# pierrepaleo/PDWT

Hardware: AMD Instinct MI355X
Metric: Mpixels/s fwd+inv DWT (4096² db4 L3) (higher is better)
Workload: dtype f32; 1 GPU; 4096x4096 float32, db4, 3 levels, separable DWT fwd+inv (BASELINE.json configs[1]); levels=3, parallelism=batch-split x1 (no data-path collective)

## Files before the change

pdwt_amd/csrc/casc_dev.hpp:

```cpp
#pragma once
#include "common.hpp"

#ifndef PDWT_CASC_DIAG
#define PDWT_CASC_DIAG 0
#endif
#define CASC_DIAG_ST(row) ((PDWT_CASC_DIAG & 1) ? ((row) & 31) : (row))
#define CASC_DIAG_LD(row) ((PDWT_CASC_DIAG & 2) ? ((row) & 31) : (row))

namespace pdwt {

template <int HLEN>
struct CascGeom {
    static constexpr int C = HLEN / 2 - 1;
    static constexpr int NB1 = C > 0 ? (C + 3) / 4 : 0;
    static constexpr int NB2 = C > 0 ? (C + 1) / 2 : 0;
    static constexpr int NBT = NB1 + NB2;
    static constexpr int WIN1 = 4 * (2 * NB1 + 1);
    static constexpr int WIN2 = 2 * (2 * NB2 + 1);
    static constexpr int MAXVL = 64 - 2 * NBT;
};

struct CascMap {
    int cpx;
    int strips;
    int gy;
    int flags;
    const void* tbl;
};
__host__ __device__ inline int casc_chunk_start(int g, int strip, int units, int gy, int strips, int cpx, int d)
{
    if (g >= gy) return units;
    int b = (int)(((long long)g * units) / gy);
    if (d != 0) {
        int bal = 0;
        for (int q = 0; q < g; q++) bal += (((q * strips + strip) / cpx) & 1) ? -1 : 1;
        b += d * bal;
    }
    return b;
}

struct CascBands {
    float *H1, *V1, *D1, *A2, *H2, *V2, *D2;
};
struct CascBatchF {
    const float* in;
    CascBands b;
};

template <int HLEN>
struct CascInvGeom {
    static constexpr int H2 = HLEN / 2;
    static constexpr int C = H2 / 2;
    static constexpr int SHIFT = (H2 & 1) ? 0 : 1;
    static constexpr int NB1 = C > 0 ? (C + 1) / 2 : 0;
    static constexpr int NB2 = C;
    static constexpr int NBT = NB1 + NB2;
    static constexpr int WIN1 = 2 * (2 * NB1 + 1);
    static constexpr int WIN2 = 2 * NB2 + 1;
    static constexpr int MAXVL = 64 - 2 * NBT;
    static constexpr int BASE = (C - SHIFT) & 1;
    static constexpr int VM_SB = H2 * (4 + 2 * (3 + 2));
};
struct CascInvBands {
    const float *A2, *H2, *V2, *D2, *H1, *V1, *D1;
};
struct CascInv3B {
    const float *A3, *H3, *V3, *D3;
};
struct CascBatchI {
    CascInvBands b;
    CascInv3B b3;
    float* out;
};


constexpr size_t kCascTraceOff = 1u << 20;
#ifdef PDWT_CASC_TRACE
#define CASC_TRACE_DECL unsigned long long casc_tr_[8] = {0, 0, 0, 0, 0, 0, 0, 0}
#define CASC_TRACE(i) casc_tr_[i] = wall_clock64()
#define CASC_TRACE_STORE(trash, wave_id, aux)                                                             \
    do {                                                                                                   \
        if ((threadIdx.x & 63) == 0) {                                                                     \
            unsigned long long* p_ = reinterpret_cast<unsigned long long*>((trash) + kCascTraceOff) + (size_t)(wave_id) * 8; \
            for (int i_ = 0; i_ < 7; i_++) p_[i_] = casc_tr_[i_];                                          \
            p_[7] = (unsigned long long)(aux);                                                             \
        }                                                                                                  \
    } while (0)
#else
#define CASC_TRACE_DECL
#define CASC_TRACE(i)
#define CASC_TRACE_STORE(trash, wave_id, aux)
#endif

int inv2d_casc3_f32(const float* A2, const float* H2, const float* V2, const float* D2, const float* H1, const float* V1, const float* D1,
                    const float* A3, const float* H3, const float* V3, const float* D3, float* out, float* trash, int nr, int nc, int hlen,
                    const Taps2<float>& f, const CascBatchI* d_tbl = nullptr, int nimg = 1);

int inv2d_cascw_f32(const float* A2, const float* H2, const float* V2, const float* D2, const float* H1, const float* V1, const float* D1,
                    const float* A3, const float* H3, const float* V3, const float* D3, float* out, float* trash, int nr, int nc, int hlen,
                    const Taps2<float>& f);

}
```

pdwt_amd/csrc/common.hpp:

```cpp
#pragma once
#include <atomic>
#include <hip/hip_runtime.h>
#include <hip/hip_ext.h>
#include <stddef.h>
#include <stdint.h>

#include "../../include/pdwt_hip.h"

namespace pdwt {

void set_last_error(hipError_t e, const char* what, const char* file, int line);

#define PDWT_HIP_TRY(expr)                                              \
    do {                                                                \
        hipError_t _e = (expr);                                         \
        if (_e != hipSuccess) {                                         \
            ::pdwt::set_last_error(_e, #expr, __FILE__, __LINE__);      \
            return PDWT_EHIP;                                           \
        }                                                               \
    } while (0)

hipStream_t stream();

enum KernelId {
    K_FWD2D_FUSED = 0,
    K_INV2D_FUSED,
    K_ANA_ROWS,
    K_ANA_COLS,
    K_SYN_COLS,
    K_SYN_ROWS,
    K_SWT_ANA_ROWS,
    K_SWT_ANA_COLS,
    K_SWT_SYN_COLS,
    K_SWT_SYN_ROWS,
    K_HAAR2D_FWD,
    K_HAAR2D_INV,
    K_HAAR1D_FWD,
    K_HAAR1D_INV,
    K_SOFT_THRESH,
    K_ABS_SUM,
    K_ABS_SUM_FINAL,
    K_FWD2D_CASC,
    K_INV2D_CASC,
    K_FWD2D_STREAM,
    K_INV2D_STREAM,
    K_FWD2D_SMALL,
    K_INV2D_SMALL,
    K_FWD2D_F64,
    K_INV2D_F64,
    K_THRESH_SUM,
    K_COUNT
};

struct KTimer {
    int id;
    hipEvent_t e0 = nullptr, e1 = nullptr;
    bool ext = false;
    explicit KTimer(int kernel_id, bool attach_to_launch = false);
    ~KTimer();
};
#define PDWT_LAUNCH_KT(kt, kernel, grid, block, lds, ...)                                                                  \
    do {                                                                                                                   \
        if ((kt).e0 && (kt).e1) hipExtLaunchKernelGGL(kernel, grid, block, lds, pdwt::stream(), (kt).e0, (kt).e1, 0, __VA_ARGS__); \
        else hipLaunchKernelGGL(kernel, grid, block, lds, pdwt::stream(), __VA_ARGS__);                                    \
    } while (0)

template <auto Kernel>
inline int lds_opt_in()
{
    static std::atomic<unsigned long long> done{0};
    int dev = 0;
    PDWT_HIP_TRY(hipGetDevice(&dev));
    const unsigned long long bit = 1ull << (dev & 63);
    if (!(done.load(std::memory_order_relaxed) & bit)) {
        PDWT_HIP_TRY(hipFuncSetAttribute((const void*)Kernel, hipFuncAttributeMaxDynamicSharedMemorySize, 160 * 1024));
        done.fetch_or(bit, std::memory_order_relaxed);
    }
    return PDWT_OK;
}

int lds_opt_in_ptr(const void* kernel);

unsigned long long* clock_probe_slot(int slot);
inline int clock_probe_size_class(int rows) { int c = 0; while ((rows << c) < 16384 && c < 7) c++; return c; }
constexpr int kClockProbeAllBlocks = 16384;
unsigned long long* clock_probe_all(int* all);
__device__ __forceinline__ void clock_probe_stamp(unsigned long long* probe, int second, int all = 0)
{
    if (probe && (all || (blockIdx.x == 0 && blockIdx.y == 0))) {
        unsigned long long* const p = probe + (all ? 4 * (size_t)blockIdx.x : (size_t)0);
        const unsigned long long c = clock64(), t = wall_clock64();
        if (threadIdx.x == 0) {
            p[2 * second] = c;
            p[2 * second + 1] = t;
        }
    }
}

enum KnobId {
    KN_FORCE_TWOPASS = 0,
    KN_TILED_COLS,
    KN_CASC,
    KN_CASC_WAVES,
    KN_CASC_NV,
    KN_CASC_MIN,
    KN_CASC_IWAVES,
    KN_CASC_IPFD,
    KN_CASC_WG,
    KN_CASC_IWG,
    KN_CASC_L3,
    KN_CASC_SPEC,
    KN_CASC_XCDW,
    KN_DWT1D_LDS_KB,
    KN_STREAM,
    KN_STREAM_R,
    KN_STREAM_WAVES,
    KN_STREAM_NARROW,
    KN_SMALL,
    KN_ROWS_TR,
    KN_RING_R,
    KN_RING_WAVES,
    KN_SWTF,
    KN_SWTF_M,
    KN_SWTF_MI,
    KN_SWTF_XCD,
    KN_SWTF_ALT,
    KN_SWTF_PERM,
    KN_SWTF_F64,
    KN_F64_LDS,
    KN_F64_LDS_MIN,
    KN_F64_LDS_WGS,
    KN_F64_LDS_MINGROUPS,
    KN_F64_LDS_SKEW,
    KN_NORM2SQ_REF1D,
    KN_NORM_IN_THRESHOLD,
    KN_SELFCHECK,
    KN_DWT1D_F64,
    KN_SWTF_LONG,
    KN_F64_TAIL,
    KN_EXP0,
    KN_EXP1,
    KN_EXP2,
    KN_EXP3,
    KN_NONSEP_TILED,
    KN_F64_LAT,
    KN_F64_LAT_MIN,
    KN_DWT1D_NT_MB,
    KN_COUNT
};
int knob(KnobId id);
bool counted_waits_ok();
void stat_casc_spec(int inverse);
int knob_set(const char* name, int value);
int knob_get(const char* name, int* value);

__host__ __device__ inline int div2(int n) { return (n + 1) >> 1; }
inline int idiv_up(int a, int b) { return (a + b - 1) / b; }

__device__ __forceinline__ int wrap_ext(int s, int n)
{
    const int np = n + (n & 1);
    if ((unsigned)s >= (unsigned)np) {
        s %= np;
        if (s < 0) s += np;
    }
    return (s == n) ? n - 1 : s;
}
__device__ __forceinline__ int wrap_per(int s, int n)
{
    if ((unsigned)s >= (unsigned)n) {
        s %= n;
        if (s < 0) s += n;
    }
    return s;
}

template <typename T>
struct Taps2 {
    T a[PDWT_MAX_FILTER_WIDTH];
    T b[PDWT_MAX_FILTER_WIDTH];
};

template <typename T> struct FiltersOf;
template <> struct FiltersOf<float> { using type = pdwt_filters_f32; };
template <> struct FiltersOf<double> { using type = pdwt_filters_f64; };

template <typename T>
inline Taps2<T> taps_fwd(const typename FiltersOf<T>::type* f)
{
    Taps2<T> t;
    for (int i = 0; i < PDWT_MAX_FILTER_WIDTH; i++) { t.a[i] = f->L[i]; t.b[i] = f->H[i]; }
    return t;
}
template <typename T>
inline Taps2<T> taps_inv(const typename FiltersOf<T>::type* f, T scale = T(1))
{
    Taps2<T> t;
    for (int i = 0; i < PDWT_MAX_FILTER_WIDTH; i++) { t.a[i] = f->IL[i] * scale; t.b[i] = f->IH[i] * scale; }
    return t;
}

template <typename T> __device__ __forceinline__ T fma_t(T a, T b, T c);
template <> __device__ __forceinline__ float fma_t<float>(float a, float b, float c) { return __builtin_fmaf(a, b, c); }
template <> __device__ __forceinline__ double fma_t<double>(double a, double b, double c) { return __builtin_fma(a, b, c); }

struct BandGeom {
    int nbands;
    int Nr[3 * 32 + 1], Nc[3 * 32 + 1];
    size_t alloc_elems[3 * 32 + 1];
};
int band_geometry(const pdwt_info& w, BandGeom* g);

}
```

pdwt_amd/csrc/dwt_casc.hip:

```cpp
#include "dwt_casc.hpp"

#include <algorithm>

#include "dwt_stream.hpp"
#include "stream_dev.hpp"
#include "casc_dev.hpp"

namespace pdwt {

constexpr int casc_fwd_stores(int p) { return 3 + 4 * (p & 1); }
template <int DIST>
constexpr int casc_fwd_after(int p)
{
    int n = casc_fwd_stores(p);
    for (int k = 1; k < DIST; k++) n += 2 + casc_fwd_stores(p + k);
    return n;
}

template <int HLEN>
constexpr int casc_fwd_region_bytes() { return (HLEN - 2) * 64 * (16 + 8); }

#define PDWT_VB_F0 " op_sel_hi:[0,1,0]"
#define PDWT_VB_N0 " op_sel_hi:[0,1,1]"
#define PDWT_VB_F1 " op_sel:[1,0,0] op_sel_hi:[1,1,0]"
#define PDWT_VB_N1 " op_sel:[1,0,0]"
template <bool WITH_VD>
__device__ __forceinline__ void col_pass8x2(v2f& ah0, v2f& ah1, v2f& vd0, v2f& vd1, v2f a0, v2f a1, v2f a2, v2f a3, v2f a4, v2f a5, v2f a6, v2f a7, v2f b0, v2f b1,
                                            v2f b2, v2f b3, v2f b4, v2f b5, v2f b6, v2f b7, v2f t0, v2f t1, v2f t2, v2f t3, v2f t4, v2f t5, v2f t6, v2f t7)
{
#define PDWT_CP_ROW(A, B, T, AC)                                                                                              \
    "v_pk_fma_f32 %0, " A ", " T ", " AC "0\n\tv_pk_fma_f32 %1, " B ", " T ", " AC "1\n\t"
    if constexpr (WITH_VD) {
        asm("v_pk_fma_f32 %0, %4, %20, 0" PDWT_VB_F0 "\n\tv_pk_fma_f32 %1, %12, %20, 0" PDWT_VB_F0 "\n\tv_pk_fma_f32 %2, %4, %20, 0" PDWT_VB_F1 "\n\tv_pk_fma_f32 %3, %12, %20, 0" PDWT_VB_F1
            "\n\tv_pk_fma_f32 %0, %5, %21, %0" PDWT_VB_N0 "\n\tv_pk_fma_f32 %1, %13, %21, %1" PDWT_VB_N0 "\n\tv_pk_fma_f32 %2, %5, %21, %2" PDWT_VB_N1 "\n\tv_pk_fma_f32 %3, %13, %21, %3" PDWT_VB_N1
            "\n\tv_pk_fma_f32 %0, %6, %22, %0" PDWT_VB_N0 "\n\tv_pk_fma_f32 %1, %14, %22, %1" PDWT_VB_N0 "\n\tv_pk_fma_f32 %2, %6, %22, %2" PDWT_VB_N1 "\n\tv_pk_fma_f32 %3, %14, %22, %3" PDWT_VB_N1
            "\n\tv_pk_fma_f32 %0, %7, %23, %0" PDWT_VB_N0 "\n\tv_pk_fma_f32 %1, %15, %23, %1" PDWT_VB_N0 "\n\tv_pk_fma_f32 %2, %7, %23, %2" PDWT_VB_N1 "\n\tv_pk_fma_f32 %3, %15, %23, %3" PDWT_VB_N1
            "\n\tv_pk_fma_f32 %0, %8, %24, %0" PDWT_VB_N0 "\n\tv_pk_fma_f32 %1, %16, %24, %1" PDWT_VB_N0 "\n\tv_pk_fma_f32 %2, %8, %24, %2" PDWT_VB_N1 "\n\tv_pk_fma_f32 %3, %16, %24, %3" PDWT_VB_N1
            "\n\tv_pk_fma_f32 %0, %9, %25, %0" PDWT_VB_N0 "\n\tv_pk_fma_f32 %1, %17, %25, %1" PDWT_VB_N0 "\n\tv_pk_fma_f32 %2, %9, %25, %2" PDWT_VB_N1 "\n\tv_pk_fma_f32 %3, %17, %25, %3" PDWT_VB_N1
            "\n\tv_pk_fma_f32 %0, %10, %26, %0" PDWT_VB_N0 "\n\tv_pk_fma_f32 %1, %18, %26, %1" PDWT_VB_N0 "\n\tv_pk_fma_f32 %2, %10, %26, %2" PDWT_VB_N1 "\n\tv_pk_fma_f32 %3, %18, %26, %3" PDWT_VB_N1
            "\n\tv_pk_fma_f32 %0, %11, %27, %0" PDWT_VB_N0 "\n\tv_pk_fma_f32 %1, %19, %27, %1" PDWT_VB_N0 "\n\tv_pk_fma_f32 %2, %11, %27, %2" PDWT_VB_N1 "\n\tv_pk_fma_f32 %3, %19, %27, %3" PDWT_VB_N1
            : "=&v"(ah0), "=&v"(ah1), "=&v"(vd0), "=&v"(vd1)
            : "v"(a0), "v"(a1), "v"(a2), "v"(a3), "v"(a4), "v"(a5), "v"(a6), "v"(a7), "v"(b0), "v"(b1), "v"(b2), "v"(b3), "v"(b4), "v"(b5), "v"(b6), "v"(b7),
              "s"(t0), "s"(t1), "s"(t2), "s"(t3), "s"(t4), "s"(t5), "s"(t6), "s"(t7));
    } else {
        asm("v_pk_fma_f32 %0, %2, %18, 0" PDWT_VB_F0 "\n\tv_pk_fma_f32 %1, %10, %18, 0" PDWT_VB_F0
            "\n\tv_pk_fma_f32 %0, %3, %19, %0" PDWT_VB_N0 "\n\tv_pk_fma_f32 %1, %11, %19, %1" PDWT_VB_N0
            "\n\tv_pk_fma_f32 %0, %4, %20, %0" PDWT_VB_N0 "\n\tv_pk_fma_f32 %1, %12, %20, %1" PDWT_VB_N0
            "\n\tv_pk_fma_f32 %0, %5, %21, %0" PDWT_VB_N0 "\n\tv_pk_fma_f32 %1, %13, %21, %1" PDWT_VB_N0
            "\n\tv_pk_fma_f32 %0, %6, %22, %0" PDWT_VB_N0 "\n\tv_pk_fma_f32 %1, %14, %22, %1" PDWT_VB_N0
            "\n\tv_pk_fma_f32 %0, %7, %23, %0" PDWT_VB_N0 "\n\tv_pk_fma_f32 %1, %15, %23, %1" PDWT_VB_N0
            "\n\tv_pk_fma_f32 %0, %8, %24, %0" PDWT_VB_N0 "\n\tv_pk_fma_f32 %1, %16, %24, %1" PDWT_VB_N0
            "\n\tv_pk_fma_f32 %0, %9, %25, %0" PDWT_VB_N0 "\n\tv_pk_fma_f32 %1, %17, %25, %1" PDWT_VB_N0
            : "=&v"(ah0), "=&v"(ah1)
            : "v"(a0), "v"(a1), "v"(a2), "v"(a3), "v"(a4), "v"(a5), "v"(a6), "v"(a7), "v"(b0), "v"(b1), "v"(b2), "v"(b3), "v"(b4), "v"(b5), "v"(b6), "v"(b7),
              "s"(t0), "s"(t1), "s"(t2), "s"(t3), "s"(t4), "s"(t5), "s"(t6), "s"(t7));
    }
#undef PDWT_CP_ROW
}
__device__ __forceinline__ void col_pass8x1(v2f& ah, v2f& vd, v2f a0, v2f a1, v2f a2, v2f a3, v2f a4, v2f a5, v2f a6, v2f a7, v2f t0, v2f t1, v2f t2, v2f t3, v2f t4,
                                            v2f t5, v2f t6, v2f t7)
{
    asm("v_pk_fma_f32 %0, %2, %10, 0" PDWT_VB_F0 "\n\tv_pk_fma_f32 %1, %2, %10, 0" PDWT_VB_F1
        "\n\tv_pk_fma_f32 %0, %3, %11, %0" PDWT_VB_N0 "\n\tv_pk_fma_f32 %1, %3, %11, %1" PDWT_VB_N1
        "\n\tv_pk_fma_f32 %0, %4, %12, %0" PDWT_VB_N0 "\n\tv_pk_fma_f32 %1, %4, %12, %1" PDWT_VB_N1
        "\n\tv_pk_fma_f32 %0, %5, %13, %0" PDWT_VB_N0 "\n\tv_pk_fma_f32 %1, %5, %13, %1" PDWT_VB_N1
        "\n\tv_pk_fma_f32 %0, %6, %14, %0" PDWT_VB_N0 "\n\tv_pk_fma_f32 %1, %6, %14, %1" PDWT_VB_N1
        "\n\tv_pk_fma_f32 %0, %7, %15, %0" PDWT_VB_N0 "\n\tv_pk_fma_f32 %1, %7, %15, %1" PDWT_VB_N1
        "\n\tv_pk_fma_f32 %0, %8, %16, %0" PDWT_VB_N0 "\n\tv_pk_fma_f32 %1, %8, %16, %1" PDWT_VB_N1
        "\n\tv_pk_fma_f32 %0, %9, %17, %0" PDWT_VB_N0 "\n\tv_pk_fma_f32 %1, %9, %17, %1" PDWT_VB_N1
        : "=&v"(ah), "=&v"(vd)
        : "v"(a0), "v"(a1), "v"(a2), "v"(a3), "v"(a4), "v"(a5), "v"(a6), "v"(a7), "s"(t0), "s"(t1), "s"(t2), "s"(t3), "s"(t4), "s"(t5), "s"(t6), "s"(t7));
}

template <int HLEN, int R2, bool LV, int DIST>
struct CascSpec {
    static constexpr int NA = 2 * R2, NA1 = NA + HLEN - 2, NL1 = NA - HLEN / 2 + 1;
    static constexpr int LIM = LV ? NA1 : NL1;
    static constexpr int stores_at(int q) { return ((q < NA) ? 3 : 0) + (((q & 1) && q >= HLEN - 1) ? 4 : 0); }
    static constexpr int loads_at(int q) { return (q < LIM && q + DIST < LIM) ? 2 : 0; }
    static constexpr int wait_cnt(int n)
    {
        const int m = n - DIST;
        int c = stores_at(m);
        for (int k = 1; k < DIST; k++) c += loads_at(m + k) + stores_at(m + k);
        return c;
    }
};

template <int HLEN, int NV, int W, bool SPEC = false>
__global__ __launch_bounds__(W == 1 ? 256 : 64 * W) void k_fwd2d_casc(const float* in, CascBands b, int Nr, int Nc, int VL,
                                                                       float* __restrict__ trash, CascMap cm, TapsLH f)
{
    using G = CascGeom<HLEN>;
    constexpr int C = G::C, NB1 = G::NB1, NB2 = G::NB2, NBT = G::NBT, WIN1 = G::WIN1, WIN2 = G::WIN2;
    extern __shared__ __attribute__((aligned(16))) unsigned char lds_raw[];
    CASC_TRACE_DECL;
    CASC_TRACE(0);
    if constexpr (W > 1) {
        if (cm.tbl) {
            static_assert(sizeof(CascBatchF) == 8 * sizeof(void*), "eight pointers per image");
            typedef const unsigned long long __attribute__((address_space(4))) * tbl_t;
            const tbl_t q = (tbl_t)(const unsigned long long*)cm.tbl + 8 * (size_t)blockIdx.y;
            in = (const float*)q[0];
            b = CascBands{(float*)q[1], (float*)q[2], (float*)q[3], (float*)q[4], (float*)q[5], (float*)q[6], (float*)q[7]};
        }
    }
    const int lane = threadIdx.x & 63;
    const int Nc2 = Nc >> 1, Nr2 = Nr >> 1, Nr4 = Nr >> 2, Nc4 = Nc >> 2;
    const int kw = __builtin_amdgcn_readfirstlane(threadIdx.x >> 6);
    int j0, rows2, strip;
    bool last;
    if constexpr (W == 1) {
        const int xcd = blockIdx.x & 7;
        const int wi = (blockIdx.x >> 3) * 4 + kw;
        if (wi >= cm.cpx * cm.strips) return;
        const int cy = xcd * cm.cpx + wi / cm.strips;
        strip = wi % cm.strips;
        const int nchunks = 8 * cm.cpx;
        j0 = (int)(((long long)cy * Nr4) / nchunks);
        rows2 = (int)(((long long)(cy + 1) * Nr4) / nchunks) - j0;
        if (rows2 <= 0) return;
        last = true;
    } else {
        const int xcd = blockIdx.x & 7, slot = blockIdx.x >> 3;
        const int wg = xcd * cm.cpx + slot;
        if (slot >= cm.cpx || wg >= cm.gy * cm.strips) return;
        const int gy = wg / cm.strips;
        strip = wg % cm.strips;
        const int J0 = casc_chunk_start(gy, strip, Nr4, cm.gy, cm.strips, cm.cpx, cm.flags);
        const int R = casc_chunk_start(gy + 1, strip, Nr4, cm.gy, cm.strips, cm.cpx, cm.flags) - J0;
        const int E = min((3 * (HLEN - 2) + 3) / 4, R / W - 1);
        const int base = (R + E) / W, rem = (R + E) % W;
        const int start = kw * base + min(kw, rem);
        rows2 = (kw < W - 1) ? base + (kw < rem ? 1 : 0) : R - start;
        j0 = J0 + start;
        last = (kw == W - 1);
    }
    const int xs = strip * VL * 4;
    const int x = xs + 4 * (lane - NBT);
    const bool valid = (lane >= NBT) && (lane < NBT + VL) && (x < Nc);
    const int xo = wrapi(x, Nc);
    const int yb = 4 * j0 - 3 * C;
    const int NA = 2 * rows2;
    const int NA1 = NA + HLEN - 2;
    const int NL1 = NA - HLEN / 2 + 1;
    const int rlast = last ? 2 * NA1 + HLEN - 3 : 2 * NA - 1;

    v2f ring[HLEN][2];
    v2f ring2[HLEN];
#pragma unroll
    for (int k = 0; k < HLEN; k++) ring2[k] = v2f{0.f, 0.f};

    const float* const lbase = in + xo;
    auto rowptr = [&](int r) { return lbase + (size_t)wrap1(yb + r, Nr) * Nc; };
    const unsigned xoff = (unsigned)xo * 4u;

    constexpr int REG = casc_fwd_region_bytes<HLEN>();
    unsigned char* const lds_rd = lds_raw + (size_t)(W > 1 ? kw : 0) * REG;
    unsigned char* const lds_wr = lds_raw + (size_t)(W > 1 && kw > 0 ? kw - 1 : 0) * REG;
    auto lds_ring = [&](unsigned char* reg, int r) { return reinterpret_cast<v4f*>(reg + ((size_t)r * 64 + lane) * 16); };
    auto lds_ring2 = [&](unsigned char* reg, int r) { return reinterpret_cast<v2f*>(reg + (size_t)(HLEN - 2) * 64 * 16 + ((size_t)r * 64 + lane) * 8); };
    auto row_pass1 = [&](const v4f& v, v2f (&lh)[2]) {
        float w[WIN1];
#pragma unroll
        for (int q = 0; q < 4; q++) w[NB1 * 4 + q] = v[q];
#pragma unroll
        for (int k = 0; k < NB1; k++) {
            const int dl = (NB1 - 1 - k) * 4, sl = (NB1 - k) * 4, dr = (NB1 + 1 + k) * 4, sr = (NB1 + k) * 4;
#pragma unroll
            for (int q = 0; q < 4; q++) {
                w[dl + q] = dpp_shr1(w[sl + q]);
                w[dr + q] = dpp_shl1(w[sr + q]);
            }
        }
#pragma unroll
        for (int p = 0; p < 2; p++) {
            v2f acc = {0.f, 0.f};
#pragma unroll
            for (int j = 0; j < HLEN; j++) acc = pk_fma(splat(w[NB1 * 4 - C + 2 * p + j]), f.t[HLEN - 1 - j], acc);
            lh[p] = acc;
        }
    };
    auto row_pass2 = [&](float a0, float a1, v2f& lh) {
        float w[WIN2];
        w[NB2 * 2] = a0;
        w[NB2 * 2 + 1] = a1;
#pragma unroll
        for (int k = 0; k < NB2; k++) {
            const int dl = (NB2 - 1 - k) * 2, sl = (NB2 - k) * 2, dr = (NB2 + 1 + k) * 2, sr = (NB2 + k) * 2;
#pragma unroll
            for (int q = 0; q < 2; q++) {
                w[dl + q] = dpp_shr1(w[sl + q]);
                w[dr + q] = dpp_shl1(w[sr + q]);
            }
        }
        v2f acc = {0.f, 0.f};
#pragma unroll
        for (int j = 0; j < HLEN; j++) acc = pk_fma(splat(w[NB2 * 2 - C + j]), f.t[HLEN - 1 - j], acc);
        lh = acc;
    };

    constexpr int DIST = NV / 2;
    static_assert(casc_fwd_after<DIST>(1) <= 63, "vmcnt is a 6-bit counter");
    v4f v[NV];
    {
        v4f pv[HLEN > 2 ? HLEN - 2 : 1];
#pragma unroll
        for (int r = 0; r < HLEN - 2; r++) pv[r] = *reinterpret_cast<const v4f*>(rowptr(r));
#pragma unroll
        for (int u = 0; u < NV; u++) v[u] = *reinterpret_cast<const v4f*>(rowptr(min(HLEN - 2 + u, rlast)));
        static_for<HLEN - 2>([&](auto Rr) {
            constexpr int r = decltype(Rr)::value;
            row_pass1(pv[r], ring[r]);
        });
    }
    if constexpr (W > 1) {
        if (kw > 0) {
#pragma unroll
            for (int r = 0; r < HLEN - 2; r++) *lds_ring(lds_wr, r) = v4f{ring[r][0].x, ring[r][0].y, ring[r][1].x, ring[r][1].y};
        }
    }

    const unsigned off1 = (unsigned)(valid ? x >> 1 : 0) * 4u, off2 = (unsigned)(valid ? x >> 2 : 0) * 4u;
    const lanemask_t vmask = __ballot(valid);
    const int lim1 = ((W == 1) || last) ? 0x7fffffff : NL1;
    const int lim2 = ((W == 1) || last) ? 0x7fffffff : NA;
    int lr = HLEN - 2 + NV;
    int lgr = wrap1(yb + min(lr, rlast), Nr);
    const size_t strideB = (size_t)Nc * 4;
    const char* const inB = reinterpret_cast<const char*>(in);
    const char* lp = inB + (size_t)lgr * strideB;
    const char* lplast = lp;
    auto next_rows = [&](const char*& p0, const char*& p1) {
        int lrq = lr;
        asm("" : "+s"(lrq));
        if (lrq < rlast) {
            p0 = lp;
            if (lgr + 2 < Nr) {
                p1 = lp + strideB;
                lp = p1 + strideB;
                lgr += 2;
            } else {
                p1 = (lgr + 1 == Nr) ? inB : lp + strideB;
                lgr = lgr + 2 - Nr;
                lp = inB + (size_t)lgr * strideB;
            }
            lplast = p1;
        } else {
            p0 = p1 = lplast;
        }
        lr += 2;
    };
    unsigned s1off = (unsigned)wrap1(2 * j0 - C, Nr2) * (unsigned)Nc2 * 4u;
    const unsigned s1end = (unsigned)Nr2 * (unsigned)Nc2 * 4u;
    unsigned s2off = (unsigned)j0 * (unsigned)Nc4 * 4u;
    (void)trash;
    const int hand_sb = __builtin_amdgcn_readfirstlane((W > 1 && kw > 0) ? 0 : -1);
    CASC_TRACE(1);
    static_for<NV>([&](auto K) { asm_drain1(v[decltype(K)::value]); });
    CASC_TRACE(2);
    auto a1_row = [&](auto A, int sb) {
            constexpr int a = decltype(A)::value;
            constexpr int u = a % (HLEN / 2);
            constexpr int s0 = (2 * u + HLEN - 2) % HLEN, s1 = (2 * u + HLEN - 1) % HLEN;
            const int n = sb * HLEN + a;
            constexpr int r0 = (2 * a) % NV, r1 = r0 + 1;
            int nq1 = n, nq2 = n;
            asm("" : "+s"(nq1));
            asm("" : "+s"(nq2));
            if (nq2 < lim2) {
                if (nq1 < lim1) {
                    asm_wait2<casc_fwd_after<DIST>((a + HLEN - DIST) % HLEN)>(v[r0], v[r1]);
                    row_pass1(v[r0], ring[s0]);
                    row_pass1(v[r1], ring[s1]);
                } else {
                    if constexpr (W > 1) {
                        const int i0 = 2 * (n - NL1);
                        const v4f q0 = *lds_ring(lds_rd, i0), q1 = *lds_ring(lds_rd, i0 + 1);
                        ring[s0][0] = v2f{q0.x, q0.y};
                        ring[s0][1] = v2f{q0.z, q0.w};
                        ring[s1][0] = v2f{q1.x, q1.y};
                        ring[s1][1] = v2f{q1.z, q1.w};
                    }
                }
                {
                    const char *p0, *p1;
                    next_rows(p0, p1);
                    asm_load_s(v[r0], reinterpret_cast<const float*>(p0), xoff);
                    asm_load_s(v[r1], reinterpret_cast<const float*>(p1), xoff);
                }
                v2f ah[2], vd[2];
#pragma unroll
                for (int p = 0; p < 2; p++) ah[p] = vd[p] = v2f{0.f, 0.f};
                static_for<HLEN>([&](auto J) {
                    constexpr int j = decltype(J)::value;
                    constexpr int s = (2 * u + j) % HLEN;
                    const v2f t = f.t[HLEN - 1 - j];
#pragma unroll
                    for (int p = 0; p < 2; p++) {
                        ah[p] = pk_fma(splat(ring[s][p].x), t, ah[p]);
                        vd[p] = pk_fma(splat(ring[s][p].y), t, vd[p]);
                    }
                });
                {
                    asm_store3_sm(b.H1, b.V1, b.D1, off1 + s1off, v2f{ah[0].y, ah[1].y}, v2f{vd[0].x, vd[1].x}, v2f{vd[0].y, vd[1].y},
                                  n < NA ? vmask : 0ull);
                    s1off += (unsigned)Nc2 * 4u;
                    if (s1off == s1end) s1off = 0;
                }
                row_pass2(ah[0].x, ah[1].x, ring2[a]);
                if constexpr (W > 1 && a < HLEN - 2) {
                    if (sb == hand_sb) *lds_ring2(lds_wr, a) = ring2[a];
                }
            } else {
                if constexpr (W > 1) ring2[a] = *lds_ring2(lds_rd, min(n - NA, HLEN - 3));
            }
            if constexpr (a & 1) {
                v2f ah2 = {0.f, 0.f}, vd2 = {0.f, 0.f};
                static_for<HLEN>([&](auto J) {
                    constexpr int j = decltype(J)::value;
                    constexpr int s = (a + 1 + j) % HLEN;
                    const v2f t = f.t[HLEN - 1 - j];
                    ah2 = pk_fma(splat(ring2[s].x), t, ah2);
                    vd2 = pk_fma(splat(ring2[s].y), t, vd2);
                });
                const bool own = (unsigned)(n - (HLEN - 1)) < (unsigned)(2 * rows2);
                asm_store4_sm(b.A2, b.H2, b.V2, b.D2, off2 + s2off, ah2.x, ah2.y, vd2.x, vd2.y, own ? vmask : 0ull);
                s2off += own ? (unsigned)Nc4 * 4u : 0u;
            }
    };
    auto epilogue = [&]() __attribute__((always_inline)) {
        CASC_TRACE(5);
#ifdef PDWT_CASC_TRACE
        asm volatile("s_waitcnt vmcnt(0)" ::: "memory");
#endif
        CASC_TRACE(6);
        CASC_TRACE_STORE(trash, blockIdx.x * W + kw, ((unsigned long long)NA1 << 32) | (unsigned)rows2);
    };
    if constexpr (SPEC) {
        static_assert(W == 16 && (NV == 2 || NV == 4), "wave programs exist for the 16-wave workgroups");
        const unsigned xoff_odd = xoff + (unsigned)strideB;
        auto spec = [&](auto R2c, auto LASTc) __attribute__((always_inline)) {
            constexpr int R2 = decltype(R2c)::value;
            constexpr bool LV = decltype(LASTc)::value;
            using S = CascSpec<HLEN, R2, LV, DIST>;
            constexpr int sNA = S::NA, sNA1 = S::NA1, sNL1 = S::NL1;
            constexpr int WR = LV ? 4 * R2 + 3 * C : 3 * C;
            const bool wraps = LV ? (j0 + R2 == Nr4) : (j0 == 0);
            const size_t wrapB = wraps ? (size_t)Nr * strideB : (size_t)0;
            const unsigned s1wrap = (!LV && j0 == 0) ? s1end : 0u;
            const char* sp = lp;
            static_for<sNA1>([&](auto Nn) {
                constexpr int n = decltype(Nn)::value;
                constexpr int a = n % HLEN;
                constexpr bool from_mem = LV ? true : (n < sNL1);
                constexpr bool computed = LV ? true : (n < sNA);
                constexpr bool store1 = n < sNA;
                constexpr int s0 = (2 * n + HLEN - 2) % HLEN, s1 = (2 * n + HLEN - 1) % HLEN;
                if constexpr (computed) {
                    if constexpr (from_mem) {
                        constexpr int q0 = (2 * n) % NV, q1 = q0 + 1;
                        if constexpr (n >= DIST) asm_wait2<S::wait_cnt(n)>(v[q0], v[q1]);
                        row_pass1(v[q0], ring[s0]);
                        row_pass1(v[q1], ring[s1]);
                        if constexpr (n + DIST < S::LIM) {
                            constexpr int r0 = 2 * (n + DIST) + HLEN - 2;
                            asm volatile("" : "=v"(v[q0]));
                            asm volatile("" : "=v"(v[q1]));
                            asm_load_s(v[q0], reinterpret_cast<const float*>(sp), xoff);
                            if constexpr (r0 + 1 == WR) {
                                asm_load_s(v[q1], reinterpret_cast<const float*>(sp + strideB - wrapB), xoff);
                            } else {
                                asm_load_s(v[q1], reinterpret_cast<const float*>(sp), xoff_odd);
                            }
                            sp += 2 * strideB;
                            if constexpr (r0 + 1 == WR || r0 + 2 == WR) sp -= wrapB;
                        }
                    } else {
                        constexpr int i0 = 2 * (n - sNL1);
                        const v4f q0 = *lds_ring(lds_rd, i0), q1 = *lds_ring(lds_rd, i0 + 1);
                        ring[s0][0] = v2f{q0.x, q0.y};
                        ring[s0][1] = v2f{q0.z, q0.w};
                        ring[s1][0] = v2f{q1.x, q1.y};
                        ring[s1][1] = v2f{q1.z, q1.w};
                    }
                    v2f ah[2], vd[2];
#pragma unroll
                    for (int p = 0; p < 2; p++) ah[p] = vd[p] = v2f{0.f, 0.f};
                    if constexpr (HLEN == 8) {
                        constexpr int q = (2 * n) % 8;
#define PDWT_R(j, p) ring[(q + (j)) % 8][p]
                        col_pass8x2<store1>(ah[0], ah[1], vd[0], vd[1], PDWT_R(0, 0), PDWT_R(1, 0), PDWT_R(2, 0), PDWT_R(3, 0), PDWT_R(4, 0), PDWT_R(5, 0), PDWT_R(6, 0),
                                            PDWT_R(7, 0), PDWT_R(0, 1), PDWT_R(1, 1), PDWT_R(2, 1), PDWT_R(3, 1), PDWT_R(4, 1), PDWT_R(5, 1), PDWT_R(6, 1), PDWT_R(7, 1),
                                            f.t[7], f.t[6], f.t[5], f.t[4], f.t[3], f.t[2], f.t[1], f.t[0]);
#undef PDWT_R
                    } else {
                        static_for<HLEN>([&](auto J) {
                            constexpr int j = decltype(J)::value;
                            constexpr int s = (2 * n + j) % HLEN;
                            const v2f t = f.t[HLEN - 1 - j];
#pragma unroll
                            for (int p = 0; p < 2; p++) {
                                ah[p] = pk_fma_vbcast<0, j == 0>(ring[s][p], t, ah[p]);
                                if constexpr (store1) vd[p] = pk_fma_vbcast<1, j == 0>(ring[s][p], t, vd[p]);
                            }
                        });
                    }
                    if constexpr (store1) {
                        asm_store3_sm(b.H1, b.V1, b.D1, off1 + s1off, v2f{ah[0].y, ah[1].y}, v2f{vd[0].x, vd[1].x}, v2f{vd[0].y, vd[1].y}, vmask);
                        s1off += (unsigned)Nc2 * 4u;
                        if constexpr (n == C - 1) s1off -= s1wrap;
                    }
                    row_pass2(ah[0].x, ah[1].x, ring2[a]);
                    if constexpr (n < HLEN - 2) {
                        if (kw > 0) *lds_ring2(lds_wr, n) = ring2[a];
                    }
                } else {
                    ring2[a] = *lds_ring2(lds_rd, n - sNA);
                }
                if constexpr ((n & 1) && n >= HLEN - 1) {
                    v2f ah2 = {0.f, 0.f}, vd2 = {0.f, 0.f};
                    if constexpr (HLEN == 8) {
                        constexpr int q = (a + 1) % 8;
                        col_pass8x1(ah2, vd2, ring2[q], ring2[(q + 1) % 8], ring2[(q + 2) % 8], ring2[(q + 3) % 8], ring2[(q + 4) % 8], ring2[(q + 5) % 8],
                                    ring2[(q + 6) % 8], ring2[(q + 7) % 8], f.t[7], f.t[6], f.t[5], f.t[4], f.t[3], f.t[2], f.t[1], f.t[0]);
                    } else {
                        static_for<HLEN>([&](auto J) {
                            constexpr int j = decltype(J)::value;
                            constexpr int s = (a + 1 + j) % HLEN;
                            const v2f t = f.t[HLEN - 1 - j];
                            ah2 = pk_fma_vbcast<0, j == 0>(ring2[s], t, ah2);
                            vd2 = pk_fma_vbcast<1, j == 0>(ring2[s], t, vd2);
                        });
                    }
                    asm_store4_sm(b.A2, b.H2, b.V2, b.D2, off2 + s2off, ah2.x, ah2.y, vd2.x, vd2.y, vmask);
                    s2off += (unsigned)Nc4 * 4u;
                }
                if constexpr (n == HLEN / 2 - 1 || n == HLEN - 1) asm volatile("s_waitcnt lgkmcnt(0)\n\ts_barrier" ::: "memory");

#ifdef PDWT_CASC_TRACE
                if constexpr (n == HLEN / 2 - 1) CASC_TRACE(3);
                if constexpr (n == HLEN - 1) CASC_TRACE(4);
#endif
            });
        };
        const int variant = __builtin_amdgcn_readfirstlane(last ? 3 : (rows2 == 5 ? 2 : 1));
        if (variant == 1) {
            spec(std::integral_constant<int, 4>{}, std::false_type{});
            epilogue();
            __builtin_amdgcn_endpgm();
        }
        if (variant == 2) {
            spec(std::integral_constant<int, 5>{}, std::false_type{});
            epilogue();
            __builtin_amdgcn_endpgm();
        }
        spec(std::integral_constant<int, 1>{}, std::true_type{});
        epilogue();
    } else {
    for (int sb = 0;; sb++) {
        static_for<HLEN / 2>([&](auto U) { a1_row(std::integral_constant<int, decltype(U)::value>{}, sb); });
        if constexpr (W > 1) {
            if (sb == 0) asm volatile("s_waitcnt lgkmcnt(0)\n\ts_barrier" ::: "memory");
        }
#ifdef PDWT_CASC_TRACE
        if (sb == 0) CASC_TRACE(3);
#endif
        if (sb * HLEN + HLEN / 2 >= NA1) break;
        static_for<HLEN / 2>([&](auto U) { a1_row(std::integral_constant<int, decltype(U)::value + HLEN / 2>{}, sb); });
        if constexpr (W > 1) {
            if (sb == 0) asm volatile("s_waitcnt lgkmcnt(0)\n\ts_barrier" ::: "memory");
        }
#ifdef PDWT_CASC_TRACE
        if (sb == 0) CASC_TRACE(4);
#endif
        if (sb * HLEN + HLEN >= NA1) break;
    }
    static_for<NV>([&](auto K) { asm_drain1(v[decltype(K)::value]); });
    epilogue();
    }
}

template <int HLEN, int PFD>
__global__ __launch_bounds__(256) void k_inv2d_casc(CascInvBands b, float* __restrict__ out, int Nr, int Nc, int VL,
                                                     float* __restrict__ trash, CascMap cm, Taps2<float> f)
{
    using G = CascInvGeom<HLEN>;
    constexpr int H2 = G::H2, C = G::C, SHIFT = G::SHIFT, NB1 = G::NB1, NB2 = G::NB2, NBT = G::NBT, WIN1 = G::WIN1, WIN2 = G::WIN2;
    constexpr int VM_PF = PFD * (4 + 2 * (3 + 2));
    static_assert(VM_PF - 3 <= 63, "vmcnt is a 6-bit counter");
    static_assert(H2 % PFD == 0 || PFD % H2 == 0, "register slots must be compile-time constants");
    const int lane = threadIdx.x & 63;
    const int xcd = blockIdx.x & 7;
    const int wi = (blockIdx.x >> 3) * 4 + __builtin_amdgcn_readfirstlane(threadIdx.x >> 6);
    if (wi >= cm.cpx * cm.strips) return;
    const int cy = xcd * cm.cpx + wi / cm.strips;
    const int strip = wi % cm.strips;
    const int Nr1 = Nr >> 1, Nc1 = Nc >> 1, Nr2 = Nr >> 2, Nc2 = Nc >> 2;
    const int nchunks = 8 * cm.cpx;
    const int ya = G::BASE + 2 * (int)(((long long)cy * (Nr1 >> 1)) / nchunks);
    const int ye = G::BASE + 2 * (int)(((long long)(cy + 1) * (Nr1 >> 1)) / nchunks);
    const int rows1 = ye - ya;
    if (rows1 <= 0) return;
    const int cx1 = strip * VL * 2 + 2 * (lane - NBT);
    const bool valid = (lane >= NBT) && (lane < NBT + VL) && (cx1 < Nc1);
    const int cx1w = wrapi(cx1, Nc1);
    const int cx2w = cx1w >> 1;
    const int gA = ya - C;
    const int P0 = (gA + SHIFT) >> 1;
    const int r2base = P0 - C;
    const int nrows1 = rows1 + H2 - 1 + SHIFT;
    const int nsteps = (nrows1 + 1) >> 1;

    const float* const pA2 = b.A2 + cx2w;
    const float* const pH2 = b.H2 + cx2w;
    const float* const pV2 = b.V2 + cx2w;
    const float* const pD2 = b.D2 + cx2w;
    const float* const pH1 = b.H1 + cx1w;
    const float* const pV1 = b.V1 + cx1w;
    const float* const pD1 = b.D1 + cx1w;
    auto off2 = [&](int r2) { return (size_t)wrap1(r2base + r2, Nr2) * Nc2; };
    auto off1 = [&](int r1) { return (size_t)wrap1(gA + r1, Nr1) * Nc1; };
    const unsigned voff2 = (unsigned)cx2w * 4u, voff1 = (unsigned)cx1w * 4u, voffo = (unsigned)(valid ? cx1 : 0) * 8u;
    const lanemask_t vmask = __ballot(valid);

    v2f r2av[H2], r2hd[H2];
    v2f ra[H2], rh[H2], rv[H2], rd[H2];
#pragma unroll
    for (int k = 0; k < H2; k++) ra[k] = rh[k] = rv[k] = rd[k] = v2f{0.f, 0.f};
    float q2[PFD][4];
    v2f q1[2 * PFD][3];
    {
#pragma unroll
        for (int r = 0; r < H2 - 1; r++) {
            const size_t o = off2(r);
            r2av[r] = v2f{pA2[o], pV2[o]};
            r2hd[r] = v2f{pH2[o], pD2[o]};
        }
        r2av[H2 - 1] = r2hd[H2 - 1] = v2f{0.f, 0.f};
#pragma unroll
        for (int p = 0; p < PFD; p++) {
            const size_t o = off2(H2 - 1 + p);
            q2[p][0] = pA2[o];
            q2[p][1] = pH2[o];
            q2[p][2] = pV2[o];
            q2[p][3] = pD2[o];
        }
#pragma unroll
        for (int q = 0; q < 2 * PFD; q++) {
            const size_t o = off1(q);
            q1[q][0] = *reinterpret_cast<const v2f*>(pH1 + o);
            q1[q][1] = *reinterpret_cast<const v2f*>(pV1 + o);
            q1[q][2] = *reinterpret_cast<const v2f*>(pD1 + o);
        }
    }

    float* const tr = trash + (size_t)(blockIdx.x & 7) * Nc;

    auto emit = [&](auto S0, auto OFF, int g) {
        constexpr int s0 = decltype(S0)::value, off = decltype(OFF)::value;
        const bool own = (g >= 0) && (g < 2 * rows1);
        float o4[4] = {0.f, 0.f, 0.f, 0.f};
        if (own) {
            v2f sa = {0.f, 0.f}, sh = {0.f, 0.f}, sv = {0.f, 0.f}, sd = {0.f, 0.f};
            static_for<H2>([&](auto J) {
                constexpr int j = decltype(J)::value;
                constexpr int s = (s0 + j) % H2;
                constexpr int k = HLEN - 1 - (2 * j + off);
                constexpr int kp = k & ~1;
                const v2f pl2 = v2f{f.a[kp], f.a[kp + 1]}, ph2 = v2f{f.b[kp], f.b[kp + 1]};
                sa = pk_fma_sbcast<k & 1, false>(ra[s], pl2, sa);
                sh = pk_fma_sbcast<k & 1, false>(rh[s], ph2, sh);
                sv = pk_fma_sbcast<k & 1, false>(rv[s], pl2, sv);
                sd = pk_fma_sbcast<k & 1, false>(rd[s], ph2, sd);
            });
            const v2f t1o = sa + sh, t2o = sv + sd;
            float t1[WIN1], t2[WIN1];
            t1[NB1 * 2] = t1o.x;
            t1[NB1 * 2 + 1] = t1o.y;
            t2[NB1 * 2] = t2o.x;
            t2[NB1 * 2 + 1] = t2o.y;
    #pragma unroll
            for (int k = 0; k < NB1; k++) {
                const int dl = (NB1 - 1 - k) * 2, sl = (NB1 - k) * 2, dr = (NB1 + 1 + k) * 2, sr = (NB1 + k) * 2;
    #pragma unroll
                for (int cc = 0; cc < 2; cc++) {
                    t1[dl + cc] = dpp_shr1(t1[sl + cc]);
                    t2[dl + cc] = dpp_shr1(t2[sl + cc]);
                    t1[dr + cc] = dpp_shl1(t1[sr + cc]);
                    t2[dr + cc] = dpp_shl1(t2[sr + cc]);
                }
            }
            auto pair_out = [&](auto E0) {
                constexpr int e0 = decltype(E0)::value;
                constexpr int pl = (e0 + SHIFT) >> 1;
                v2f s1 = {0.f, 0.f}, s2 = {0.f, 0.f};
    #pragma unroll
                for (int j = 0; j < H2; j++) {
                    const int m = HLEN - 1 - 2 * j;
                    s1 = pk_fma(splat(t1[NB1 * 2 + pl - C + j]), v2f{f.a[m - 1], f.a[m]}, s1);
                    s2 = pk_fma(splat(t2[NB1 * 2 + pl - C + j]), v2f{f.b[m - 1], f.b[m]}, s2);
                }
                const v2f o = s1 + s2;
                o4[e0] = o.x;
                o4[e0 + 1] = o.y;
            };
            auto single_out = [&](auto E) {
                constexpr int eo = decltype(E)::value;
                constexpr int gp = eo + SHIFT;
                constexpr int pl = gp >> 1, offx = 1 - (gp & 1);
                float s1 = 0.f, s2 = 0.f;
    #pragma unroll
                for (int j = 0; j < H2; j++) {
                    const int k = HLEN - 1 - (2 * j + offx);
                    s1 = __builtin_fmaf(t1[NB1 * 2 + pl - C + j], f.a[k], s1);
                    s2 = __builtin_fmaf(t2[NB1 * 2 + pl - C + j], f.b[k], s2);
                }
                o4[eo] = s1 + s2;
            };
            if constexpr (SHIFT == 0) {
                pair_out(std::integral_constant<int, 0>{});
                pair_out(std::integral_constant<int, 2>{});
            } else {
                single_out(std::integral_constant<int, 0>{});
                pair_out(std::integral_constant<int, 1>{});
                single_out(std::integral_constant<int, 3>{});
            }
        }
        asm_store_sm(own ? out + (size_t)wrap1(2 * ya + g, Nr) * Nc : tr, voffo, v4f{o4[0], o4[1], o4[2], o4[3]}, vmask);
    };

    auto synth2 = [&](auto S0, auto OFF, float& a0, float& a1) {
        constexpr int s0 = decltype(S0)::value, off = decltype(OFF)::value;
        v2f sav = {0.f, 0.f}, shd = {0.f, 0.f};
        static_for<H2>([&](auto J) {
            constexpr int j = decltype(J)::value;
            constexpr int s = (s0 + j) % H2;
            constexpr int k = HLEN - 1 - (2 * j + off);
            constexpr int kp = k & ~1;
            sav = pk_fma_sbcast<k & 1, false>(r2av[s], v2f{f.a[kp], f.a[kp + 1]}, sav);
            shd = pk_fma_sbcast<k & 1, false>(r2hd[s], v2f{f.b[kp], f.b[kp + 1]}, shd);
        });
        const v2f t = sav + shd;
        float t1[WIN2], t2[WIN2];
        t1[NB2] = t.x;
        t2[NB2] = t.y;
#pragma unroll
        for (int k = 0; k < NB2; k++) {
            t1[NB2 - 1 - k] = dpp_shr1(t1[NB2 - k]);
            t2[NB2 - 1 - k] = dpp_shr1(t2[NB2 - k]);
            t1[NB2 + 1 + k] = dpp_shl1(t1[NB2 + k]);
            t2[NB2 + 1 + k] = dpp_shl1(t2[NB2 + k]);
        }
        float o2[2];
#pragma unroll
        for (int e = 0; e < 2; e++) {
            const int gp = e + SHIFT;
            const int pl = gp >> 1, offx = 1 - (gp & 1);
            float s1 = 0.f, s2 = 0.f;
#pragma unroll
            for (int j = 0; j < H2; j++) {
                const int k = HLEN - 1 - (2 * j + offx);
                s1 = __builtin_fmaf(t1[NB2 + pl - C + j], f.a[k], s1);
                s2 = __builtin_fmaf(t2[NB2 + pl - C + j], f.b[k], s2);
            }
            o2[e] = s1 + s2;
        }
        a0 = o2[0];
        a1 = o2[1];
    };

    constexpr int kWait2 = VM_PF - 4, kWait1 = VM_PF - 3;
    auto step = [&](auto Pp, int sb) {
        constexpr int p = decltype(Pp)::value;
        const int s = sb * H2 + p;
        constexpr int pr = p % PFD;
        asm_wait4<kWait2>(q2[pr][0], q2[pr][1], q2[pr][2], q2[pr][3]);
        r2av[(H2 - 1 + p) % H2] = v2f{asm_copy(q2[pr][0]), asm_copy(q2[pr][2])};
        r2hd[(H2 - 1 + p) % H2] = v2f{asm_copy(q2[pr][1]), asm_copy(q2[pr][3])};
        {
            const size_t o = off2(min(H2 - 1 + s + PFD, H2 - 2 + nsteps));
            asm_load_s(q2[pr][0], b.A2 + o, voff2);
            asm_load_s(q2[pr][1], b.H2 + o, voff2);
            asm_load_s(q2[pr][2], b.V2 + o, voff2);
            asm_load_s(q2[pr][3], b.D2 + o, voff2);
        }
        static_for<2>([&](auto I) {
            constexpr int idx = decltype(I)::value;
            constexpr int q = 2 * p + idx;
            float a0, a1;
            synth2(std::integral_constant<int, p % H2>{}, std::integral_constant<int, 1 - idx>{}, a0, a1);
            const int r1 = 2 * s + idx;
            constexpr int qr = q % (2 * PFD);
            asm_wait3<kWait1>(q1[qr][0], q1[qr][1], q1[qr][2]);
            ra[q % H2] = v2f{a0, a1};
            rh[q % H2] = asm_copy(q1[qr][0]);
            rv[q % H2] = asm_copy(q1[qr][1]);
            rd[q % H2] = asm_copy(q1[qr][2]);
            {
                const size_t o = off1(min(r1 + 2 * PFD, 2 * nsteps - 1));
                asm_load_s(q1[qr][0], b.H1 + o, voff1);
                asm_load_s(q1[qr][1], b.V1 + o, voff1);
                asm_load_s(q1[qr][2], b.D1 + o, voff1);
            }
            const int g1 = 2 * (r1 - (H2 - 1)) - SHIFT;
            emit(std::integral_constant<int, (q + 1) % H2>{}, std::integral_constant<int, 1>{}, g1);
            emit(std::integral_constant<int, (q + 1) % H2>{}, std::integral_constant<int, 0>{}, g1 + 1);
        });
    };

    static_for<PFD>([&](auto K) {
        constexpr int k = decltype(K)::value;
        asm_drain1(q2[k][0]);
        asm_drain1(q2[k][1]);
        asm_drain1(q2[k][2]);
        asm_drain1(q2[k][3]);
    });
    static_for<2 * PFD>([&](auto K) {
        constexpr int k = decltype(K)::value;
        asm_drain1(q1[k][0]);
        asm_drain1(q1[k][1]);
        asm_drain1(q1[k][2]);
    });
    for (int sb = 0;; sb++) {
        bool fin = false;
        static_for<H2>([&](auto Pp) {
            if (!fin) {
                step(Pp, sb);
                fin = (sb * H2 + decltype(Pp)::value + 1 >= nsteps);
            }
        });
        if (fin) break;
    }
    static_for<PFD>([&](auto K) {
        constexpr int k = decltype(K)::value;
        asm_drain1(q2[k][0]);
        asm_drain1(q2[k][1]);
        asm_drain1(q2[k][2]);
        asm_drain1(q2[k][3]);
    });
    static_for<2 * PFD>([&](auto K) {
        constexpr int k = decltype(K)::value;
        asm_drain1(q1[k][0]);
        asm_drain1(q1[k][1]);
        asm_drain1(q1[k][2]);
    });
}

#define PDWT_CHECK_LAUNCH() PDWT_HIP_TRY(hipGetLastError())

static bool casc_enabled() { return knob(KN_CASC) == 1; }

template <int HLEN>
static int launch_fwd_casc(const float* in, const CascBands& b, float* trash, int nr, int nc, const Taps2<float>& f2, const CascBatchF* d_tbl, int nimg)
{
    TapsLH f;
    for (int k = 0; k < PDWT_MAX_FILTER_WIDTH; k++) f.t[k] = v2f{f2.a[k], f2.b[k]};
    constexpr int MAXVL = CascGeom<HLEN>::MAXVL;
    const int strips = idiv_up(nc, MAXVL * 4);
    const int VL = idiv_up(nc / 4, strips);
    constexpr int NVD = HLEN > 16 ? 4 : (HLEN % 4 == 0 ? HLEN / 2 : HLEN);
    KTimer kt(K_FWD2D_CASC, true);
    int W = knob(KN_CASC_WG);
    if (W == 0) W = 16;
    if (W != 1 && W != 4 && W != 8 && W != 16) W = 16;
    constexpr size_t REG = casc_fwd_region_bytes<HLEN>();
    while (W > 1 && (size_t)(W - 1) * REG > 150 * 1024) W /= 2;
    if (W == 2) W = 1;
    if (W > 1) {
        const int nr4 = nr / 4;
        const int wgs = knob(KN_CASC_WAVES) > 0 ? idiv_up(knob(KN_CASC_WAVES), W) : 256;
        int gy = std::max(1, wgs / strips);
        while (W > 4 && (nr4 / gy) / W < HLEN / 2) W /= 2;
        while (gy > 1 && (nr4 / gy) / W < HLEN / 2) gy--;
        if (gy >= 1 && (nr4 / gy) / W >= HLEN / 2) {
            int nwg = gy * strips;
            const size_t lds = (size_t)(W - 1) * REG;
            void (*k)(const float*, CascBands, int, int, int, float*, CascMap, TapsLH);
            k = (W == 4) ? k_fwd2d_casc<HLEN, NVD, 4> : (W == 8) ? k_fwd2d_casc<HLEN, NVD, 8> : k_fwd2d_casc<HLEN, NVD, 16>;
            const bool nv2 = W == 16 && (knob(KN_CASC_NV) == 0 || knob(KN_CASC_NV) == 2);
            if (nv2) k = k_fwd2d_casc<HLEN, 2, 16>;
            bool spec = nv2 && (knob(KN_CASC_SPEC) & 1) && 2 * 4 >= HLEN;
            auto spec_ok = [&](int gyq, int xwq) {
                const int cpxq = idiv_up(gyq * strips, 8);
                for (int g = 0; g < gyq; g++)
                    for (int st = 0; st < strips; st++) {
                        const int R = casc_chunk_start(g + 1, st, nr4, gyq, strips, cpxq, xwq) - casc_chunk_start(g, st, nr4, gyq, strips, cpxq, xwq);
                        if (R < 16) return false;
                        const int E = std::min((3 * (HLEN - 2) + 3) / 4, R / 16 - 1);
                        const int base = (R + E) / 16, rem = (R + E) % 16;
                        if (base != 4 || R - (15 * base + std::min(15, rem)) != 1) return false;
                    }
                return true;
            };
            if (spec && (knob(KN_CASC_SPEC) & 4) && knob(KN_CASC_WAVES) <= 0 && !d_tbl && (nr4 / gy) / 16 >= 8) {
                const int gy2 = (nr4 + 36) / 73;
                if (gy2 >= 3 * gy && spec_ok(gy2, 0)) {
                    gy = gy2;
                    nwg = gy * strips;
                }
            }
            int xw = spec ? knob(KN_CASC_XCDW) : 0;
            if (spec && xw != 0 && !spec_ok(gy, xw)) xw = 0;
            spec = spec && spec_ok(gy, xw);
            if (!spec) xw = 0;
            if (spec) {
                k = k_fwd2d_casc<HLEN, 2, 16, true>;
                stat_casc_spec(0);
            }
            const CascMap cm = {idiv_up(nwg, 8), strips, gy, xw, d_tbl};
            const dim3 grid((unsigned)(8 * cm.cpx), (unsigned)(d_tbl ? nimg : 1));
            if (lds > 64 * 1024) {
                int rc = (W == 4) ? lds_opt_in<k_fwd2d_casc<HLEN, NVD, 4>>()
                         : (W == 8) ? lds_opt_in<k_fwd2d_casc<HLEN, NVD, 8>>() : lds_opt_in<k_fwd2d_casc<HLEN, NVD, 16>>();
                if (rc == PDWT_OK && nv2) rc = lds_opt_in<k_fwd2d_casc<HLEN, 2, 16>>();
                if (rc == PDWT_OK && spec) rc = lds_opt_in<k_fwd2d_casc<HLEN, 2, 16, true>>();
                if (rc != PDWT_OK) return rc;
            }
            PDWT_LAUNCH_KT(kt, k, grid, dim3(64 * W), lds, in, b, nr, nc, VL, trash, cm, f);
            PDWT_CHECK_LAUNCH();
            return PDWT_OK;
        }
    }
    if (d_tbl) return 1;
    int cpx = (knob(KN_CASC_WAVES) > 0 ? knob(KN_CASC_WAVES) : 1024) / (8 * strips);
    if (cpx > nr / 4 / 4 / 8) cpx = nr / 4 / 4 / 8;
    if (cpx < 1) cpx = 1;
    const CascMap cm = {cpx, strips, 0};
    const dim3 grid((unsigned)(8 * idiv_up(cpx * strips, 4)));
    const int nv = knob(KN_CASC_NV) > 0 ? knob(KN_CASC_NV) : NVD;
    if (nv == 2)
        PDWT_LAUNCH_KT(kt, (k_fwd2d_casc<HLEN, 2, 1>), grid, dim3(256), 0, in, b, nr, nc, VL, trash, cm, f);
    else if (nv < HLEN && HLEN % 4 == 0)
        PDWT_LAUNCH_KT(kt, (k_fwd2d_casc<HLEN, NVD, 1>), grid, dim3(256), 0, in, b, nr, nc, VL, trash, cm, f);
    else
        PDWT_LAUNCH_KT(kt, (k_fwd2d_casc<HLEN, (HLEN > 16 ? NVD : HLEN), 1>), grid, dim3(256), 0, in, b, nr, nc, VL, trash, cm, f);
    PDWT_CHECK_LAUNCH();
    return PDWT_OK;
}

#ifdef PDWT_CASC_ONLY8
#define PDWT_CASC_FWD_HLENS(X) X(8)
#else
#define PDWT_CASC_FWD_HLENS(X) X(4) X(6) X(8) X(10) X(12) X(14) X(16) X(18) X(20)
#endif

int fwd2d_casc_f32(const float* in, float* H1, float* V1, float* D1, float* A2, float* H2, float* V2, float* D2, float* trash, int nr,
                   int nc, int hlen, const Taps2<float>& f, const CascBatchF* d_tbl, int nimg)
{
    if (!casc_enabled() || !stream_enabled() || !trash) return 1;
    if ((nr & 3) || (nc & 3) || nc < 256 || nr < 16 * hlen) return 1;
    if ((long long)nr * nc < (long long)knob(KN_CASC_MIN)) return 1;
    if ((long long)nr * nc >= (1LL << 32)) return 1;
    if (!al16(in) || !al16(H1) || !al16(V1) || !al16(D1) || !al16(A2) || !al16(H2) || !al16(V2) || !al16(D2)) return 1;
    const CascBands b = {H1, V1, D1, A2, H2, V2, D2};
    switch (hlen) {
#define X(H) \
    case H: return launch_fwd_casc<H>(in, b, trash, nr, nc, f, d_tbl, nimg);
        PDWT_CASC_FWD_HLENS(X)
#undef X
        default: return 1;
    }
}

template <int HLEN>
static int launch_inv_casc(const CascInvBands& b, float* out, float* trash, int nr, int nc, const Taps2<float>& f)
{
    constexpr int MAXVL = CascInvGeom<HLEN>::MAXVL;
    const int nc1 = nc / 2;
    const int strips = idiv_up(nc1, MAXVL * 2);
    const int VL = idiv_up(nc1 / 2, strips);
    int cpx = (knob(KN_CASC_IWAVES) > 0 ? knob(KN_CASC_IWAVES) : 2048) / (8 * strips);
    if (cpx > nr / 2 / 8 / 8) cpx = nr / 2 / 8 / 8;
    if (cpx < 1) cpx = 1;
    const CascMap cm = {cpx, strips, 0};
    const dim3 grid((unsigned)(8 * idiv_up(cpx * strips, 4)));
    KTimer kt(K_INV2D_CASC, true);
    constexpr int H2 = HLEN / 2;
    const int pfd = knob(KN_CASC_IPFD);
    bool launched = false;
    if constexpr (H2 % 2 == 0) {
        if (pfd == 2) {
            PDWT_LAUNCH_KT(kt, (k_inv2d_casc<HLEN, 2>), grid, dim3(256), 0, b, out, nr, nc, VL, trash, cm, f);
            launched = true;
        }
    }
    if constexpr (H2 * 14 - 3 <= 63 && H2 > 2) {
        if (pfd >= H2 && !launched) {
            PDWT_LAUNCH_KT(kt, (k_inv2d_casc<HLEN, H2>), grid, dim3(256), 0, b, out, nr, nc, VL, trash, cm, f);
            launched = true;
        }
    }
    if (!launched) PDWT_LAUNCH_KT(kt, (k_inv2d_casc<HLEN, 1>), grid, dim3(256), 0, b, out, nr, nc, VL, trash, cm, f);
    PDWT_CHECK_LAUNCH();
    return PDWT_OK;
}

#ifdef PDWT_CASC_ONLY8
#define PDWT_CASC_INV_HLENS(X) X(8)
#else
#define PDWT_CASC_INV_HLENS(X) X(4) X(6) X(8) X(10)
#endif

int inv2d_casc_f32(const float* A2, const float* H2, const float* V2, const float* D2, const float* H1, const float* V1, const float* D1,
                   float* out, float* trash, int nr, int nc, int hlen, const Taps2<float>& f)
{
    if (!casc_enabled() || !stream_enabled() || !trash) return 1;
    if ((nr & 3) || (nc & 3) || nc < 256 || nr < 32 * hlen) return 1;
    if ((long long)nr * nc < (long long)knob(KN_CASC_MIN)) return 1;
    if (!al16(out) || !al16(H1) || !al16(V1) || !al16(D1) || !al16(A2) || !al16(H2) || !al16(V2) || !al16(D2) || !al16(trash)) return 1;
    const CascInvBands b = {A2, H2, V2, D2, H1, V1, D1};
    switch (hlen) {
#define X(H) \
    case H: return launch_inv_casc<H>(b, out, trash, nr, nc, f);
        PDWT_CASC_INV_HLENS(X)
#undef X
        default: return 1;
    }
}

}
```

pdwt_amd/csrc/dwt_casc_inv3.hip:

```cpp
#include <algorithm>

#include "casc_dev.hpp"
#include "dwt_stream.hpp"
#include "stream_dev.hpp"

namespace pdwt {

#define PDWT_AI __attribute__((always_inline))

template <int HLEN>
constexpr int casc_inv3_region_bytes() { return (HLEN / 2 - 1) * 64 * (16 + 32); }

#define PDWT_PKS_FIRST0 " op_sel_hi:[1,0,0]"
#define PDWT_PKS_NEXT0 " op_sel_hi:[1,0,1]"
#define PDWT_PKS_FIRST1 " op_sel:[0,1,0] op_sel_hi:[1,1,0]"
#define PDWT_PKS_NEXT1 " op_sel:[0,1,0] op_sel_hi:[1,1,1]"
template <int HALF>
__device__ __forceinline__ void col_synth4x4(v2f& sa, v2f& sh, v2f& sv, v2f& sd, v2f a0, v2f a1, v2f a2, v2f a3, v2f h0, v2f h1, v2f h2, v2f h3, v2f v0,
                                             v2f v1, v2f v2, v2f v3, v2f d0, v2f d1, v2f d2, v2f d3, v2f fa3, v2f fa2_, v2f fa1, v2f fa0, v2f fb3, v2f fb2_,
                                             v2f fb1, v2f fb0)
{
#define PDWT_CS4(F, N)                                                                                                                    \
    asm("v_pk_fma_f32 %0, %4, %20, 0" F "\n\tv_pk_fma_f32 %1, %8, %24, 0" F "\n\tv_pk_fma_f32 %2, %12, %20, 0" F "\n\tv_pk_fma_f32 %3, %16, %24, 0" F \
        "\n\tv_pk_fma_f32 %0, %5, %21, %0" N "\n\tv_pk_fma_f32 %1, %9, %25, %1" N "\n\tv_pk_fma_f32 %2, %13, %21, %2" N "\n\tv_pk_fma_f32 %3, %17, %25, %3" N \
        "\n\tv_pk_fma_f32 %0, %6, %22, %0" N "\n\tv_pk_fma_f32 %1, %10, %26, %1" N "\n\tv_pk_fma_f32 %2, %14, %22, %2" N "\n\tv_pk_fma_f32 %3, %18, %26, %3" N \
        "\n\tv_pk_fma_f32 %0, %7, %23, %0" N "\n\tv_pk_fma_f32 %1, %11, %27, %1" N "\n\tv_pk_fma_f32 %2, %15, %23, %2" N "\n\tv_pk_fma_f32 %3, %19, %27, %3" N \
        : "=&v"(sa), "=&v"(sh), "=&v"(sv), "=&v"(sd)                                                                                       \
        : "v"(a0), "v"(a1), "v"(a2), "v"(a3), "v"(h0), "v"(h1), "v"(h2), "v"(h3), "v"(v0), "v"(v1), "v"(v2), "v"(v3), "v"(d0), "v"(d1), "v"(d2),  \
          "v"(d3), "s"(fa3), "s"(fa2_), "s"(fa1), "s"(fa0), "s"(fb3), "s"(fb2_), "s"(fb1), "s"(fb0))
    if constexpr (HALF == 0) PDWT_CS4(PDWT_PKS_FIRST0, PDWT_PKS_NEXT0);
    else PDWT_CS4(PDWT_PKS_FIRST1, PDWT_PKS_NEXT1);
#undef PDWT_CS4
}
template <int HALF>
__device__ __forceinline__ void col_synth2x4(v2f& sav, v2f& shd, v2f a0, v2f a1, v2f a2, v2f a3, v2f h0, v2f h1, v2f h2, v2f h3, v2f fa3, v2f fa2_, v2f fa1,
                                             v2f fa0, v2f fb3, v2f fb2_, v2f fb1, v2f fb0)
{
#define PDWT_CS2(F, N)                                                                                                      \
    asm("v_pk_fma_f32 %0, %2, %10, 0" F "\n\tv_pk_fma_f32 %1, %6, %14, 0" F "\n\tv_pk_fma_f32 %0, %3, %11, %0" N "\n\tv_pk_fma_f32 %1, %7, %15, %1" N \
        "\n\tv_pk_fma_f32 %0, %4, %12, %0" N "\n\tv_pk_fma_f32 %1, %8, %16, %1" N "\n\tv_pk_fma_f32 %0, %5, %13, %0" N "\n\tv_pk_fma_f32 %1, %9, %17, %1" N \
        : "=&v"(sav), "=&v"(shd)                                                                                            \
        : "v"(a0), "v"(a1), "v"(a2), "v"(a3), "v"(h0), "v"(h1), "v"(h2), "v"(h3), "s"(fa3), "s"(fa2_), "s"(fa1), "s"(fa0), "s"(fb3), "s"(fb2_),  \
          "s"(fb1), "s"(fb0))
    if constexpr (HALF == 0) PDWT_CS2(PDWT_PKS_FIRST0, PDWT_PKS_NEXT0);
    else PDWT_CS2(PDWT_PKS_FIRST1, PDWT_PKS_NEXT1);
#undef PDWT_CS2
}

template <int HLEN, int NQ, bool LV, bool L3>
struct CascInvSpec {
    using G = CascInvGeom<HLEN>;
    static constexpr int H2 = G::H2, XS = H2 / 2, NSTEPS = NQ + XS, NP = 2 * NQ;
    static constexpr int NL2 = L3 ? 3 : 4;
    static constexpr bool l2act(int s) { return s >= 0 && s < NSTEPS && (LV || s < NQ); }
    static constexpr bool need2(int s) { return l2act(s) && (LV || s + H2 - 1 < NQ); }
    static constexpr bool adv3(int s) { return L3 && !(s & 1) && (need2(s) || need2(s + 1)); }
    static constexpr int n3(int s) { return (adv3(s) && adv3(s + 2)) ? 4 : 0;  }
    static constexpr int n2(int s) { return (l2act(s) && need2(s + 1)) ? NL2 : 0; }
    static constexpr int n1(int s) { return (l2act(s) && l2act(s + 1)) ? 3 : 0; }
    static constexpr bool own(int s, int idx) { return 2 * s + idx - (H2 - 1) >= 0 && 2 * s + idx - (H2 - 1) < NP; }
    static constexpr int st(int s, int idx) { return own(s, idx) ? 2 : 0; }
    static constexpr int total(int s) { return n3(s) + n2(s) + 2 * n1(s) + st(s, 0) + st(s, 1); }
    static constexpr int wait3(int s) { return n2(s - 2) + 2 * n1(s - 2) + st(s - 2, 0) + st(s - 2, 1) + total(s - 1); }
    static constexpr int wait2(int s) { return 2 * n1(s - 1) + st(s - 1, 0) + st(s - 1, 1) + n3(s); }
    static constexpr int wait1(int s, int idx)
    {
        return idx == 0 ? st(s - 1, 0) + n1(s - 1) + st(s - 1, 1) + n3(s) + n2(s) : st(s - 1, 1) + n3(s) + n2(s) + n1(s) + st(s, 0);
    }
};

template <int HLEN, int W, bool L3, bool SPEC = false>
__global__ __launch_bounds__(64 * W) void k_inv2d_casc3(CascInvBands b, CascInv3B b3, float* out, int Nr, int Nc, int VL,
                                                         float* __restrict__ trash, CascMap cm, Taps2<float> f)
{
    using G = CascInvGeom<HLEN>;
    constexpr int H2 = G::H2, C = G::C, SHIFT = G::SHIFT, NBT = G::NBT;
    static_assert(H2 % 2 == 0, "the parity of a step must be a compile-time constant of the unrolled super-body");
    constexpr int XS = H2 / 2;
    constexpr int PHI = SHIFT;
    constexpr int T0 = (H2 - 1 + PHI) >> 1;
    static_assert(((H2 - 1 + PHI) & 1) == 0, "loop step 0 starts a level-(l+2) window");
    constexpr int NW3 = H2 + T0 - 1;
    constexpr int NL2 = L3 ? 3 : 4;
    constexpr int kStep = NL2 + 2 * (3 + 2);
    extern __shared__ __attribute__((aligned(16))) unsigned char lds_raw[];
    CASC_TRACE_DECL;
    CASC_TRACE(0);
    if (cm.tbl) {
        static_assert(sizeof(CascBatchI) == 12 * sizeof(void*), "twelve pointers per image");
        typedef const unsigned long long __attribute__((address_space(4))) * tbl_t;
        const tbl_t q = (tbl_t)(const unsigned long long*)cm.tbl + 12 * (size_t)blockIdx.y;
        b = CascInvBands{(const float*)q[0], (const float*)q[1], (const float*)q[2], (const float*)q[3], (const float*)q[4], (const float*)q[5], (const float*)q[6]};
        b3 = CascInv3B{(const float*)q[7], (const float*)q[8], (const float*)q[9], (const float*)q[10]};
        out = (float*)q[11];
    }
    const int lane = threadIdx.x & 63;
    const int kw = __builtin_amdgcn_readfirstlane(threadIdx.x >> 6);
    const int Nr1 = Nr >> 1, Nc1 = Nc >> 1, Nr2 = Nr >> 2, Nc2 = Nc >> 2, Nr3 = Nr >> 3, Nc3 = Nc >> 3;
    const int xcd = blockIdx.x & 7, slot = blockIdx.x >> 3;
    const int wg = xcd * cm.cpx + slot;
    if (slot >= cm.cpx || wg >= cm.gy * cm.strips) return;
    const int gy = wg / cm.strips, strip = wg % cm.strips;
    const int Np = Nr2 >> 1;
    const int Jp = casc_chunk_start(gy, strip, Np, cm.gy, cm.strips, cm.cpx, cm.flags);
    const int Rp = casc_chunk_start(gy + 1, strip, Np, cm.gy, cm.strips, cm.cpx, cm.flags) - Jp;
    const int Ep = 0;
    const int basep = (Rp + Ep) / W, remp = (Rp + Ep) % W;
    const int startp = kw * basep + min(kw, remp);
    const bool last = (kw == W - 1);
    const int nQ = 2 * (last ? Rp - startp : basep + (kw < remp ? 1 : 0));
    const int Q0 = 2 * (Jp + startp);
    const int nsteps = nQ + XS;
    const int P0 = 2 * (Q0 + C) - SHIFT;
    const int O0 = 2 * (P0 + C) - SHIFT;
    const int nP = 2 * nQ;
    const int last2 = last ? H2 - 2 + nsteps : nQ - 1;
    const int last1 = last ? 2 * nsteps - 1 : nP - 1;
    const int P3_0 = (Q0 + SHIFT) >> 1;
    const int last3 = ((last2 + PHI) >> 1) + H2 - 1;

    const int X0 = strip * VL - NBT;
    const int cx1 = 2 * (X0 + lane);
    const bool valid = (lane >= NBT) && (lane < NBT + VL) && (cx1 < Nc1);
    const int cx1w = wrapi(cx1, Nc1);
    const int cx2w = cx1w >> 1;
    const int c3w = wrapi(((X0 + 1) >> 1) - C + lane, Nc3);
    const int bp_addr = 4 * (((X0 + lane + 1) >> 1) - ((X0 + 1) >> 1) + C);
    const bool bp_odd = ((X0 + lane) & 1) != 0;

    auto off3 = [&](int i) PDWT_AI { return (size_t)CASC_DIAG_LD(wrapi(P3_0 - C + i, Nr3)) * Nc3; };
    auto off2 = [&](int s2) PDWT_AI { return (size_t)CASC_DIAG_LD(wrap1(Q0 + s2, Nr2)) * Nc2; };
    auto off1 = [&](int r1) PDWT_AI { return (size_t)CASC_DIAG_LD(wrap1(P0 + r1, Nr1)) * Nc1; };
    const unsigned voff3 = (unsigned)c3w * 4u, voff2 = (unsigned)cx2w * 4u, voff1 = (unsigned)cx1w * 4u, voffo = (unsigned)(valid ? cx1 : 0) * 8u;
    const lanemask_t vmask = __ballot(valid);
    constexpr int kFold = (PDWT_CASC_DIAG & 2) ? 32 : 0;
    const unsigned str3 = (unsigned)Nc3 * 4u, str2 = (unsigned)Nc2 * 4u, str1 = (unsigned)Nc1 * 4u;
    const unsigned end3 = (unsigned)(kFold ? min(kFold, Nr3) : Nr3) * str3, end2 = (unsigned)(kFold ? min(kFold, Nr2) : Nr2) * str2,
                   end1 = (unsigned)(kFold ? min(kFold, Nr1) : Nr1) * str1;
    int c3 = min(T0 + H2, last3), c2 = min(H2, last2), c1 = min(2, last1);
    unsigned o3 = (unsigned)CASC_DIAG_LD(wrapi(P3_0 - C + c3, Nr3)) * str3, o2 = (unsigned)CASC_DIAG_LD(wrap1(Q0 + c2, Nr2)) * str2,
             o1 = (unsigned)CASC_DIAG_LD(wrap1(P0 + c1, Nr1)) * str1;
    auto advance = [&](int& c, unsigned& o, int lastc, unsigned str, unsigned end) {
        int cq = c;
        asm("" : "+s"(cq));
        if (cq < lastc) {
            c++;
            o += str;
            if (o == end) o = 0;
        }
    };
    int orow = CASC_DIAG_ST(wrap1(O0, Nr));
    float* op = out + (size_t)orow * Nc;
    const int oend = (PDWT_CASC_DIAG & 1) ? min(32, Nr) : Nr;
    (void)trash;

    constexpr int REG = casc_inv3_region_bytes<HLEN>();
    unsigned char* const lds_rd = lds_raw + (size_t)kw * REG;
    unsigned char* const lds_wr = lds_raw + (size_t)(kw > 0 ? kw - 1 : 0) * REG;
    auto lds_l2 = [&](unsigned char* reg, int r) PDWT_AI { return reinterpret_cast<v4f*>(reg + ((size_t)r * 64 + lane) * 16); };
    auto lds_l1 = [&](unsigned char* reg, int r, int h) PDWT_AI {
        return reinterpret_cast<v4f*>(reg + (size_t)(H2 - 1) * 64 * 16 + (((size_t)r * 2 + h) * 64 + lane) * 16);
    };

    v2f r3av[H2], r3hd[H2];
    v2f r2av[H2], r2hd[H2];
    v2f ra[H2], rh[H2], rv[H2], rd[H2];
#pragma unroll
    for (int k = 0; k < H2; k++) ra[k] = rh[k] = rv[k] = rd[k] = v2f{0.f, 0.f};

    static_assert(SHIFT == 1, "even H2");
    v2f fa2[H2], fb2[H2];
#pragma unroll
    for (int i = 0; i < H2; i++) {
        fa2[i] = v2f{f.a[2 * i], f.a[2 * i + 1]};
        fb2[i] = v2f{f.b[2 * i], f.b[2 * i + 1]};
    }
    auto nat_pair = [&](const float* t1w, const float* t2w) PDWT_AI {
        v2f s1 = {0.f, 0.f}, s2 = {0.f, 0.f};
#pragma unroll
        for (int j = 0; j < H2; j++) {
            const int m = HLEN - 1 - 2 * j;
            s1 = pk_fma(splat(t1w[j]), fa2[(m - 1) / 2], s1);
            s2 = pk_fma(splat(t2w[j]), fb2[(m - 1) / 2], s2);
        }
        return s1 + s2;
    };
    auto synth_col = [&](const v2f (&av)[H2], const v2f (&hd)[H2], auto S0, auto OFF) {
        constexpr int s0 = decltype(S0)::value, off = decltype(OFF)::value;
        v2f sav = {0.f, 0.f}, shd = {0.f, 0.f};
        if constexpr (H2 == 4) {
            constexpr int half = (HLEN - 1 - off) & 1;
            col_synth2x4<half>(sav, shd, av[s0 % 4], av[(s0 + 1) % 4], av[(s0 + 2) % 4], av[(s0 + 3) % 4], hd[s0 % 4], hd[(s0 + 1) % 4], hd[(s0 + 2) % 4],
                               hd[(s0 + 3) % 4], fa2[3], fa2[2], fa2[1], fa2[0], fb2[3], fb2[2], fb2[1], fb2[0]);
        } else {
            static_for<H2>([&](auto J) {
                constexpr int j = decltype(J)::value;
                constexpr int sl = (s0 + j) % H2;
                constexpr int k = HLEN - 1 - (2 * j + off);
                sav = pk_fma_sbcast<k & 1, j == 0>(av[sl], fa2[k >> 1], sav);
                shd = pk_fma_sbcast<k & 1, j == 0>(hd[sl], fb2[k >> 1], shd);
            });
        }
        const v2f t = sav + shd;
        float t1w[H2], t2w[H2];
        t1w[C] = t.x;
        t2w[C] = t.y;
#pragma unroll
        for (int k = 1; k <= C; k++) {
            t1w[C - k] = dpp_shr1(t1w[C - k + 1]);
            t2w[C - k] = dpp_shr1(t2w[C - k + 1]);
        }
#pragma unroll
        for (int k = 1; k <= H2 - 1 - C; k++) {
            t1w[C + k] = dpp_shl1(t1w[C + k - 1]);
            t2w[C + k] = dpp_shl1(t2w[C + k - 1]);
        }
        return nat_pair(t1w, t2w);
    };
    auto own_pair = [&](v2f p0) PDWT_AI { return v2f{p0.y, dpp_shl1(p0.x)}; };
    auto a2_from = [&](const v2f (&av)[H2], const v2f (&hd)[H2], auto OFF) {
        const v2f p0 = synth_col(av, hd, std::integral_constant<int, 0>{}, OFF);
        const int glo = __builtin_amdgcn_ds_bpermute(bp_addr, __float_as_int(p0.x));
        const int ghi = __builtin_amdgcn_ds_bpermute(bp_addr, __float_as_int(p0.y));
        return __int_as_float(bp_odd ? glo : ghi);
    };

    float q3[4];
    float q2[4];
    v2f q1[2][3];
    {
        v2f w3av[NW3], w3hd[NW3];
        if constexpr (L3) {
#pragma unroll
            for (int i = 0; i < NW3; i++) {
                const size_t o = off3(min(i, last3)) + c3w;
                w3av[i] = v2f{b3.A3[o], b3.V3[o]};
                w3hd[i] = v2f{b3.H3[o], b3.D3[o]};
            }
            const size_t o = off3(min(NW3, last3)) + c3w;
            q3[0] = b3.A3[o];
            q3[1] = b3.H3[o];
            q3[2] = b3.V3[o];
            q3[3] = b3.D3[o];
        } else {
            q3[0] = q3[1] = q3[2] = q3[3] = 0.f;
        }
#pragma unroll
        for (int r = 0; r < H2 - 1; r++) {
            const size_t o = off2(r) + cx2w;
            r2av[r] = v2f{L3 ? 0.f : b.A2[o], b.V2[o]};
            r2hd[r] = v2f{b.H2[o], b.D2[o]};
        }
        r2av[H2 - 1] = r2hd[H2 - 1] = v2f{0.f, 0.f};
        {
            const size_t o = off2(H2 - 1) + cx2w;
            q2[0] = L3 ? 0.f : b.A2[o];
            q2[1] = b.H2[o];
            q2[2] = b.V2[o];
            q2[3] = b.D2[o];
        }
#pragma unroll
        for (int q = 0; q < 2; q++) {
            const size_t o = off1(q) + cx1w;
            q1[q][0] = *reinterpret_cast<const v2f*>(b.H1 + o);
            q1[q][1] = *reinterpret_cast<const v2f*>(b.V1 + o);
            q1[q][2] = *reinterpret_cast<const v2f*>(b.D1 + o);
        }
        if constexpr (L3) static_for<H2 - 1>([&](auto S2) {
            constexpr int s2 = decltype(S2)::value;
            constexpr int t = (s2 + PHI) >> 1, idx3 = (s2 + PHI) & 1;
            v2f av[H2], hd[H2];
#pragma unroll
            for (int j = 0; j < H2; j++) {
                av[j] = w3av[t + j];
                hd[j] = w3hd[t + j];
            }
            r2av[s2].x = a2_from(av, hd, std::integral_constant<int, 1 - idx3>{});
        });
        if constexpr (L3) {
#pragma unroll
            for (int j = 0; j < H2; j++) {
                r3av[j] = w3av[T0 - 1 + j];
                r3hd[j] = w3hd[T0 - 1 + j];
            }
        }
    }
    CASC_TRACE(1);
    if (kw > 0) {
#pragma unroll
        for (int r = 0; r < H2 - 1; r++) *lds_l2(lds_wr, r) = v4f{r2av[r].x, r2av[r].y, r2hd[r].x, r2hd[r].y};
    }


    auto emit = [&](auto S0, auto OFF, auto own_, int g) PDWT_AI {
        constexpr int s0 = decltype(S0)::value, off = decltype(OFF)::value;
        constexpr bool kOwnStatic = std::is_same<decltype(own_), std::true_type>::value;
        const bool own = own_;
        v4f o4;
        asm("" : "=v"(o4));
        if (own) {
            v2f sa = {0.f, 0.f}, sh = {0.f, 0.f}, sv = {0.f, 0.f}, sd = {0.f, 0.f};
            if constexpr (H2 == 4) {
                constexpr int half = (HLEN - 1 - off) & 1;
                constexpr int j0 = s0 % 4, j1 = (s0 + 1) % 4, j2 = (s0 + 2) % 4, j3 = (s0 + 3) % 4;
                col_synth4x4<half>(sa, sh, sv, sd, ra[j0], ra[j1], ra[j2], ra[j3], rh[j0], rh[j1], rh[j2], rh[j3], rv[j0], rv[j1], rv[j2], rv[j3], rd[j0],
                                   rd[j1], rd[j2], rd[j3], fa2[3], fa2[2], fa2[1], fa2[0], fb2[3], fb2[2], fb2[1], fb2[0]);
            } else {
                static_for<H2>([&](auto J) {
                    constexpr int j = decltype(J)::value;
                    constexpr int sl = (s0 + j) % H2;
                    constexpr int k = HLEN - 1 - (2 * j + off);
                    sa = pk_fma_sbcast<k & 1, j == 0>(ra[sl], fa2[k >> 1], sa);
                    sh = pk_fma_sbcast<k & 1, j == 0>(rh[sl], fb2[k >> 1], sh);
                    sv = pk_fma_sbcast<k & 1, j == 0>(rv[sl], fa2[k >> 1], sv);
                    sd = pk_fma_sbcast<k & 1, j == 0>(rd[sl], fb2[k >> 1], sd);
                });
            }
            const v2f t1o = sa + sh, t2o = sv + sd;
            constexpr int NT = H2 + 1;
            float t1w[NT], t2w[NT];
            t1w[C - 1] = t1o.x;
            t1w[C] = t1o.y;
            t2w[C - 1] = t2o.x;
            t2w[C] = t2o.y;
#pragma unroll
            for (int i = C - 2; i >= 0; i--) {
                t1w[i] = dpp_shr1(t1w[i + 2]);
                t2w[i] = dpp_shr1(t2w[i + 2]);
            }
#pragma unroll
            for (int i = C + 1; i < NT; i++) {
                t1w[i] = dpp_shl1(t1w[i - 2]);
                t2w[i] = dpp_shl1(t2w[i - 2]);
            }
            const v2f pa = nat_pair(t1w, t2w);
            const v2f pb = nat_pair(t1w + 1, t2w + 1);
            o4 = v4f{dpp_shr1(pb.y), pa.x, pa.y, pb.x};
        }
        (void)g;
        if constexpr (kOwnStatic) {
            asm_store_sm(op, voffo, o4, vmask);
            op += Nc;
        } else {
            asm_store_sm(op, voffo, o4, own ? vmask : 0ull);
            if (own) {
                op += Nc;
                if (++orow == oend) {
                    orow = 0;
                    op = out;
                }
            }
        }
    };

    auto step = [&](auto Pp, int sb) {
        constexpr int p = decltype(Pp)::value;
        constexpr bool even = L3 && (p & 1) == 0;
        constexpr int EX = even ? 4 : 0;
        const int s = sb * H2 + p;
        const bool l2act = last || (s < nQ);
        if (l2act) {
            const int s2 = H2 - 1 + s;
            if constexpr (even) {
                asm_wait4<2 * kStep>(q3[0], q3[1], q3[2], q3[3]);
#pragma unroll
                for (int j = 0; j < H2 - 1; j++) {
                    r3av[j] = r3av[j + 1];
                    r3hd[j] = r3hd[j + 1];
                }
                r3av[H2 - 1] = v2f{asm_copy(q3[0]), asm_copy(q3[2])};
                r3hd[H2 - 1] = v2f{asm_copy(q3[1]), asm_copy(q3[3])};
                {
                    const unsigned vo = voff3 + o3;
                    asm_load_s(q3[0], b3.A3, vo);
                    asm_load_s(q3[1], b3.H3, vo);
                    asm_load_s(q3[2], b3.V3, vo);
                    asm_load_s(q3[3], b3.D3, vo);
                    advance(c3, o3, last3, str3, end3);
                }
            }
            float a2 = 0.f;
            if constexpr (L3) a2 = a2_from(r3av, r3hd, std::integral_constant<int, even ? 1 : 0>{});
            constexpr int sl = (H2 - 1 + p) % H2;
            if constexpr (L3) {
                asm_wait3<2 * (3 + 2) + EX>(q2[1], q2[2], q2[3]);
            } else {
                asm_wait4<2 * (3 + 2)>(q2[0], q2[1], q2[2], q2[3]);
                a2 = asm_copy(q2[0]);
            }
            v4f e = v4f{a2, asm_copy(q2[2]), asm_copy(q2[1]), asm_copy(q2[3])};
            if (!(last || s2 < nQ)) e = *lds_l2(lds_rd, s2 - nQ);
            r2av[sl] = v2f{e.x, e.y};
            r2hd[sl] = v2f{e.z, e.w};
            {
                const unsigned vo = voff2 + o2;
                if constexpr (!L3) asm_load_s(q2[0], b.A2, vo);
                asm_load_s(q2[1], b.H2, vo);
                asm_load_s(q2[2], b.V2, vo);
                asm_load_s(q2[3], b.D2, vo);
                advance(c2, o2, last2, str2, end2);
            }
        }
        static_for<2>([&](auto I) {
            constexpr int idx = decltype(I)::value;
            constexpr int q = 2 * p + idx;
            const int r1 = 2 * s + idx;
            constexpr int sl = q % H2;
            if (l2act) {
                const v2f a01 = own_pair(synth_col(r2av, r2hd, std::integral_constant<int, p % H2>{}, std::integral_constant<int, 1 - idx>{}));
                asm_wait3<2 + (3 + 2) + NL2 + EX>(q1[idx][0], q1[idx][1], q1[idx][2]);
                ra[sl] = a01;
                rh[sl] = asm_copy(q1[idx][0]);
                rv[sl] = asm_copy(q1[idx][1]);
                rd[sl] = asm_copy(q1[idx][2]);
                {
                    const unsigned vo = voff1 + o1;
                    asm_load_s(q1[idx][0], b.H1, vo);
                    asm_load_s(q1[idx][1], b.V1, vo);
                    asm_load_s(q1[idx][2], b.D1, vo);
                    advance(c1, o1, last1, str1, end1);
                }
                if constexpr (q < H2 - 1) {
                    if (sb == 0 && kw > 0) {
                        *lds_l1(lds_wr, q, 0) = v4f{ra[sl].x, ra[sl].y, rh[sl].x, rh[sl].y};
                        *lds_l1(lds_wr, q, 1) = v4f{rv[sl].x, rv[sl].y, rd[sl].x, rd[sl].y};
                    }
                }
            } else if (r1 - nP < H2 - 1) {
                const v4f e0 = *lds_l1(lds_rd, r1 - nP, 0), e1 = *lds_l1(lds_rd, r1 - nP, 1);
                ra[sl] = v2f{e0.x, e0.y};
                rh[sl] = v2f{e0.z, e0.w};
                rv[sl] = v2f{e1.x, e1.y};
                rd[sl] = v2f{e1.z, e1.w};
            }
            const int ws = r1 - (H2 - 1);
            const bool own = (ws >= 0) && (ws < nP);
            emit(std::integral_constant<int, (q + 1) % H2>{}, std::integral_constant<int, 1>{}, own, 2 * ws);
            emit(std::integral_constant<int, (q + 1) % H2>{}, std::integral_constant<int, 0>{}, own, 2 * ws + 1);
        });
    };

    asm_drain1(q3[0]);
    asm_drain1(q3[1]);
    asm_drain1(q3[2]);
    asm_drain1(q3[3]);
    asm_drain1(q2[0]);
    asm_drain1(q2[1]);
    asm_drain1(q2[2]);
    asm_drain1(q2[3]);
    static_for<2>([&](auto K) {
        constexpr int k = decltype(K)::value;
        asm_drain1(q1[k][0]);
        asm_drain1(q1[k][1]);
        asm_drain1(q1[k][2]);
    });
    CASC_TRACE(2);

    auto spec = [&](auto NQc, auto LASTc) PDWT_AI {
        {
            constexpr int NQ = decltype(NQc)::value;
            constexpr bool LV = decltype(LASTc)::value;
            using S = CascInvSpec<HLEN, NQ, LV, L3>;
            constexpr int WR3 = NQ / 2 + C, WR2 = NQ, WR1 = 2 * NQ - 2 * C + SHIFT, WRO = 4 * NQ - 6 * C + 3 * SHIFT;
            const bool bottom = LV && (Q0 + NQ == Nr2);
            const unsigned w3 = bottom ? end3 : 0u, w2 = bottom ? end2 : 0u, w1 = bottom ? end1 : 0u;
            const size_t wo = bottom ? (size_t)Nr * Nc : (size_t)0;
            static_for<S::NSTEPS>([&](auto Ss) {
                constexpr int st = decltype(Ss)::value;
                constexpr int p = st % H2;
                constexpr bool even = L3 && (st & 1) == 0;
                if constexpr (S::l2act(st)) {
                    constexpr int s2 = H2 - 1 + st;
                    constexpr int sl = s2 % H2;
                    if constexpr (S::adv3(st)) {
                        if constexpr (st >= 2) asm_wait4<S::wait3(st)>(q3[0], q3[1], q3[2], q3[3]);
#pragma unroll
                        for (int j = 0; j < H2 - 1; j++) {
                            r3av[j] = r3av[j + 1];
                            r3hd[j] = r3hd[j + 1];
                        }
                        r3av[H2 - 1] = v2f{asm_copy(q3[0]), asm_copy(q3[2])};
                        r3hd[H2 - 1] = v2f{asm_copy(q3[1]), asm_copy(q3[3])};
                        if constexpr (S::n3(st) != 0) {
                            constexpr int row = T0 + H2 + st / 2;
                            const unsigned vo = voff3 + o3;
                            asm volatile("" : "=v"(q3[0]));
                            asm volatile("" : "=v"(q3[1]));
                            asm volatile("" : "=v"(q3[2]));
                            asm volatile("" : "=v"(q3[3]));
                            asm_load_s(q3[0], b3.A3, vo);
                            asm_load_s(q3[1], b3.H3, vo);
                            asm_load_s(q3[2], b3.V3, vo);
                            asm_load_s(q3[3], b3.D3, vo);
                            o3 += str3;
                            if constexpr (row + 1 == WR3) o3 -= w3;
                        }
                    }
                    if constexpr (S::need2(st)) {
                        float a2 = 0.f;
                        if constexpr (L3) a2 = a2_from(r3av, r3hd, std::integral_constant<int, even ? 1 : 0>{});
                        if constexpr (L3) {
                            if constexpr (st >= 1) asm_wait3<S::wait2(st)>(q2[1], q2[2], q2[3]);
                        } else {
                            if constexpr (st >= 1) asm_wait4<S::wait2(st)>(q2[0], q2[1], q2[2], q2[3]);
                            a2 = asm_copy(q2[0]);
                        }
                        r2av[sl] = v2f{a2, asm_copy(q2[2])};
                        r2hd[sl] = v2f{asm_copy(q2[1]), asm_copy(q2[3])};
                    } else {
                        const v4f e = *lds_l2(lds_rd, s2 - NQ);
                        r2av[sl] = v2f{e.x, e.y};
                        r2hd[sl] = v2f{e.z, e.w};
                    }
                    if constexpr (S::n2(st) != 0) {
                        const unsigned vo = voff2 + o2;
                        if constexpr (!L3) {
                            asm volatile("" : "=v"(q2[0]));
                            asm_load_s(q2[0], b.A2, vo);
                        }
                        asm volatile("" : "=v"(q2[1]));
                        asm volatile("" : "=v"(q2[2]));
                        asm volatile("" : "=v"(q2[3]));
                        asm_load_s(q2[1], b.H2, vo);
                        asm_load_s(q2[2], b.V2, vo);
                        asm_load_s(q2[3], b.D2, vo);
                        o2 += str2;
                        if constexpr (s2 + 2 == WR2) o2 -= w2;
                    }
                }
                static_for<2>([&](auto I) {
                    constexpr int idx = decltype(I)::value;
                    constexpr int r1 = 2 * st + idx;
                    constexpr int sl = r1 % H2;
                    if constexpr (S::l2act(st)) {
                        const v2f a01 = own_pair(synth_col(r2av, r2hd, std::integral_constant<int, p % H2>{}, std::integral_constant<int, 1 - idx>{}));
                        if constexpr (st >= 1) asm_wait3<S::wait1(st, idx)>(q1[idx][0], q1[idx][1], q1[idx][2]);
                        ra[sl] = a01;
                        rh[sl] = asm_copy(q1[idx][0]);
                        rv[sl] = asm_copy(q1[idx][1]);
                        rd[sl] = asm_copy(q1[idx][2]);
                        if constexpr (S::n1(st) != 0) {
                            const unsigned vo = voff1 + o1;
                            asm volatile("" : "=v"(q1[idx][0]));
                            asm volatile("" : "=v"(q1[idx][1]));
                            asm volatile("" : "=v"(q1[idx][2]));
                            asm_load_s(q1[idx][0], b.H1, vo);
                            asm_load_s(q1[idx][1], b.V1, vo);
                            asm_load_s(q1[idx][2], b.D1, vo);
                            o1 += str1;
                            if constexpr (r1 + 3 == WR1) o1 -= w1;
                        }
                        if constexpr (r1 < H2 - 1) {
                            if (kw > 0) {
                                *lds_l1(lds_wr, r1, 0) = v4f{ra[sl].x, ra[sl].y, rh[sl].x, rh[sl].y};
                                *lds_l1(lds_wr, r1, 1) = v4f{rv[sl].x, rv[sl].y, rd[sl].x, rd[sl].y};
                            }
                        }
                    } else if constexpr (r1 - S::NP < H2 - 1) {
                        const v4f e0 = *lds_l1(lds_rd, r1 - S::NP, 0), e1 = *lds_l1(lds_rd, r1 - S::NP, 1);
                        ra[sl] = v2f{e0.x, e0.y};
                        rh[sl] = v2f{e0.z, e0.w};
                        rv[sl] = v2f{e1.x, e1.y};
                        rd[sl] = v2f{e1.z, e1.w};
                    }
                    if constexpr (S::own(st, idx)) {
                        constexpr int ws = r1 - (H2 - 1);
                        static_for<2>([&](auto Pq) {
                            constexpr int par = decltype(Pq)::value;
                            constexpr int g = 2 * ws + par;
                            __builtin_amdgcn_sched_barrier(0);
                            emit(std::integral_constant<int, (r1 + 1) % H2>{}, std::integral_constant<int, 1 - par>{}, std::true_type{}, g);
                            if constexpr (g + 1 == WRO) op -= wo;
                            __builtin_amdgcn_sched_barrier(0);
                        });
                    }
                });
                if constexpr (st < XS) asm volatile("s_waitcnt lgkmcnt(0)\n\ts_barrier" ::: "memory");
#ifdef PDWT_CASC_TRACE
                if constexpr (st == H2 - 1) CASC_TRACE(3);
                if constexpr (st == 2 * H2 - 1) CASC_TRACE(4);
#endif
            });
        }
    };
    auto epilogue = [&]() PDWT_AI {
        CASC_TRACE(5);
#ifdef PDWT_CASC_TRACE
        asm volatile("s_waitcnt vmcnt(0)" ::: "memory");
#endif
        CASC_TRACE(6);
        CASC_TRACE_STORE(trash + kCascTraceOff, blockIdx.x * W + kw, ((unsigned long long)nsteps << 32) | (unsigned)nQ);
    };
    if constexpr (SPEC) {
        static_assert(W == 16, "wave programs exist for the 16-wave workgroups");
        const int variant = __builtin_amdgcn_readfirstlane(last ? 3 : (nQ == 6 ? 2 : 1));
        if (variant == 1) {
            spec(std::integral_constant<int, 4>{}, std::false_type{});
            epilogue();
            __builtin_amdgcn_endpgm();
        }
        if (variant == 2) {
            spec(std::integral_constant<int, 6>{}, std::false_type{});
            epilogue();
            __builtin_amdgcn_endpgm();
        }
        spec(std::integral_constant<int, 4>{}, std::true_type{});
        epilogue();
    } else {
    for (int sb = 0;; sb++) {
        bool fin = false;
        static_for<H2>([&](auto Pp) {
            constexpr int p = decltype(Pp)::value;
            if (!fin) {
                step(Pp, sb);
                if constexpr (p < XS || p == 0) {
                    if (sb == 0) asm volatile("s_waitcnt lgkmcnt(0)\n\ts_barrier" ::: "memory");
                }
                fin = (sb * H2 + p + 1 >= nsteps);
            }
        });
#ifdef PDWT_CASC_TRACE
        if (sb == 0) CASC_TRACE(3);
        if (sb == 1) CASC_TRACE(4);
#endif
        if (fin) break;
    }
    {
        asm_drain1(q3[0]);
        asm_drain1(q3[1]);
        asm_drain1(q3[2]);
        asm_drain1(q3[3]);
        asm_drain1(q2[0]);
        asm_drain1(q2[1]);
        asm_drain1(q2[2]);
        asm_drain1(q2[3]);
        static_for<2>([&](auto K) {
            constexpr int k = decltype(K)::value;
            asm_drain1(q1[k][0]);
            asm_drain1(q1[k][1]);
            asm_drain1(q1[k][2]);
        });
    }
        epilogue();
    }
}

#define PDWT_CHECK_LAUNCH() PDWT_HIP_TRY(hipGetLastError())

template <int HLEN, bool L3>
static int launch_inv_casc3(const CascInvBands& b, const CascInv3B& b3, float* out, float* trash, int nr, int nc, const Taps2<float>& f,
                            const CascBatchI* d_tbl, int nimg)
{
    using G = CascInvGeom<HLEN>;
    constexpr int H2 = G::H2;
    const int nc1 = nc / 2, np = nr / 8;
    const int strips = idiv_up(nc1, G::MAXVL * 2);
    const int VL = idiv_up(nc1 / 2, strips);
    int Wk = knob(KN_CASC_IWG);
    if (Wk != 4 && Wk != 8 && Wk != 12 && Wk != 16) Wk = 16;
    constexpr size_t REG = casc_inv3_region_bytes<HLEN>();
    auto lds_bytes = [&](int w) { return (size_t)(w - 1) * REG; };
    const int wgs = knob(KN_CASC_IWAVES) > 0 ? idiv_up(knob(KN_CASC_IWAVES), Wk) : 256;
    auto fits = [&](int w, int g) {
        if (lds_bytes(w) > 150 * 1024) return false;
        for (int Rp : {np / g, idiv_up(np, g)}) {
            const int Ep = 0;
            const int basep = (Rp + Ep) / w, remp = (Rp + Ep) % w;
            if (2 * basep < H2) return false;
            const int lastp = Rp - ((w - 1) * basep + std::min(w - 1, remp));
            if (lastp < 1) return false;
        }
        return true;
    };
    int W = 0, gy = 0;
    for (int w : {Wk, 16, 12, 8, 4}) {
        for (int g = std::max(1, wgs / strips); g >= std::max(1, wgs / strips / 2) && !W; g--)
            if (fits(w, g)) {
                W = w;
                gy = g;
            }
        if (W) break;
    }
    if (!W) return 1;
    const int nwg = gy * strips;
    
    const size_t lds = lds_bytes(W);
    void (*k)(CascInvBands, CascInv3B, float*, int, int, int, float*, CascMap, Taps2<float>);
    k = (W == 4) ? k_inv2d_casc3<HLEN, 4, L3> : (W == 8) ? k_inv2d_casc3<HLEN, 8, L3> : (W == 12) ? k_inv2d_casc3<HLEN, 12, L3> : k_inv2d_casc3<HLEN, 16, L3>;
    bool spec = W == 16 && ((knob(KN_CASC_SPEC) >> 1) & 1) && H2 <= 4;
    int xw = spec ? knob(KN_CASC_XCDW) : 0;
    for (int pass = 0; pass < 2; pass++) {
        bool ok = spec;
        for (int g = 0; g < gy && ok; g++)
            for (int st = 0; st < strips && ok; st++) {
                const int Rp = casc_chunk_start(g + 1, st, np, gy, strips, idiv_up(nwg, 8), xw) - casc_chunk_start(g, st, np, gy, strips, idiv_up(nwg, 8), xw);
                ok = Rp / 16 == 2;
            }
        if (ok || xw == 0) {
            spec = ok;
            break;
        }
        xw = 0;
    }
    if (!spec) xw = 0;
    if (spec) {
        k = k_inv2d_casc3<HLEN, 16, L3, true>;
        stat_casc_spec(1);
    }
    const CascMap cm = {idiv_up(nwg, 8), strips, gy, xw, d_tbl};
    const dim3 grid((unsigned)(8 * cm.cpx), (unsigned)(d_tbl ? nimg : 1));
    if (lds > 64 * 1024) {
        const int rc = spec ? lds_opt_in<k_inv2d_casc3<HLEN, 16, L3, true>>()
                       : (W == 4) ? lds_opt_in<k_inv2d_casc3<HLEN, 4, L3>>() : (W == 8) ? lds_opt_in<k_inv2d_casc3<HLEN, 8, L3>>() : (W == 12) ? lds_opt_in<k_inv2d_casc3<HLEN, 12, L3>>() : lds_opt_in<k_inv2d_casc3<HLEN, 16, L3>>();
        if (rc != PDWT_OK) return rc;
    }
    KTimer kt(K_INV2D_CASC, true);
    PDWT_LAUNCH_KT(kt, k, grid, dim3(64 * W), lds, b, b3, out, nr, nc, VL, trash, cm, f);
    PDWT_CHECK_LAUNCH();
    return PDWT_OK;
}

int inv2d_casc3_f32(const float* A2, const float* H2, const float* V2, const float* D2, const float* H1, const float* V1, const float* D1,
                    const float* A3, const float* H3, const float* V3, const float* D3, float* out, float* trash, int nr, int nc, int hlen,
                    const Taps2<float>& f, const CascBatchI* d_tbl, int nimg)
{
    const bool l3 = A3 != nullptr;
    if ((nr & 7) || (nc & 7) || nc < 256 || nr < 32 * hlen) return 1;
    if ((long long)nr * nc >= (1LL << 32)) return 1;
    if (!al16(out) || !al16(H1) || !al16(V1) || !al16(D1) || !al16(H2) || !al16(V2) || !al16(D2) || !al16(trash)) return 1;
    if (!l3 && !al16(A2)) return 1;
    const CascInvBands b = {A2, H2, V2, D2, H1, V1, D1};
    const CascInv3B b3 = {A3, H3, V3, D3};
    switch (hlen) {
        case 4: return l3 ? launch_inv_casc3<4, true>(b, b3, out, trash, nr, nc, f, d_tbl, nimg) : launch_inv_casc3<4, false>(b, b3, out, trash, nr, nc, f, d_tbl, nimg);
        case 8: return l3 ? launch_inv_casc3<8, true>(b, b3, out, trash, nr, nc, f, d_tbl, nimg) : launch_inv_casc3<8, false>(b, b3, out, trash, nr, nc, f, d_tbl, nimg);
        case 12: return l3 ? launch_inv_casc3<12, true>(b, b3, out, trash, nr, nc, f, d_tbl, nimg) : launch_inv_casc3<12, false>(b, b3, out, trash, nr, nc, f, d_tbl, nimg);
        case 20: return l3 ? launch_inv_casc3<20, true>(b, b3, out, trash, nr, nc, f, d_tbl, nimg) : launch_inv_casc3<20, false>(b, b3, out, trash, nr, nc, f, d_tbl, nimg);
        case 16: return l3 ? launch_inv_casc3<16, true>(b, b3, out, trash, nr, nc, f, d_tbl, nimg) : launch_inv_casc3<16, false>(b, b3, out, trash, nr, nc, f, d_tbl, nimg);
        default: return 1;
    }
}

}
```

pdwt_amd/csrc/dwt_stream.hip:

```cpp
#include "dwt_stream.hpp"

#include <algorithm>
#include "stream_dev.hpp"

namespace pdwt {

template <int HLEN, int NIN_>
struct FwdGeom {
    static constexpr int NIN = NIN_;
    static constexpr int C = HLEN / 2 - 1;
    static constexpr int NB = C > 0 ? (C + NIN - 1) / NIN : 0;
    static constexpr int WIN = NIN * (2 * NB + 1);
    static constexpr int MAXVL = 64 - 2 * NB;
};

template <int HLEN, int NIN>
__global__ __launch_bounds__(256) void k_fwd2d_stream(const float* __restrict__ in, float* __restrict__ cA, float* __restrict__ cH,
                                                       float* __restrict__ cV, float* __restrict__ cD, int Nr, int Nc, int R, int VL,
                                                       float* __restrict__ trash, int trash_mask, ChunkMap cm, TapsLH f,
                                                       const StreamBatchF* __restrict__ batch)
{
    if (batch) {
        const StreamBatchF e = batch[blockIdx.y];
        in = e.in;
        cA = e.cA;
        cH = e.cH;
        cV = e.cV;
        cD = e.cD;
        trash = e.trash;
    }
    using G = FwdGeom<HLEN, NIN>;
    using VIN = typename VecOf<NIN>::type;
    constexpr int NB = G::NB, C = G::C, WIN = G::WIN, P = NIN / 2;
    int cy, bx;
    if (!chunk_of_block(cm, cy, bx)) return;
    const int lane = threadIdx.x & 63;
    const int strip = bx * 4 + (threadIdx.x >> 6);
    const int xs = strip * VL * NIN;
    if (xs >= Nc) return;
    const int Nr2 = Nr >> 1, Nc2 = Nc >> 1;
    const int y0 = cy * R;
    const int rows = min(R, Nr2 - y0);
    if (rows <= 0) return;
    const int x = xs + NIN * (lane - NB);
    const bool valid = (lane >= NB) && (lane < NB + VL) && (x < Nc);
    const int xo = wrapi(x, Nc);
    const int yb = 2 * y0 - C;
    const int nin = 2 * rows + HLEN - 2;

    v2f ring[HLEN][P];

    auto load_row = [&](int r, VIN& v) { v = *reinterpret_cast<const VIN*>(in + (size_t)wrap1(yb + r, Nr) * Nc + xo); };

    auto row_pass = [&](const VIN& v, v2f (&lh)[P]) {
        float w[WIN];
#pragma unroll
        for (int q = 0; q < NIN; q++) w[NB * NIN + q] = v[q];
#pragma unroll
        for (int k = 0; k < NB; k++) {
            const int dl = (NB - 1 - k) * NIN, sl = (NB - k) * NIN, dr = (NB + 1 + k) * NIN, sr = (NB + k) * NIN;
#pragma unroll
            for (int q = 0; q < NIN; q++) {
                w[dl + q] = dpp_shr1(w[sl + q]);
                w[dr + q] = dpp_shl1(w[sr + q]);
            }
        }
#pragma unroll
        for (int p = 0; p < P; p++) {
            v2f acc = {0.f, 0.f};
#pragma unroll
            for (int j = 0; j < HLEN; j++) acc = pk_fma(splat(w[NB * NIN - C + 2 * p + j]), f.t[HLEN - 1 - j], acc);
            lh[p] = acc;
        }
    };

    VIN v[HLEN];
    {
        VIN pv[HLEN > 2 ? HLEN - 2 : 1];
#pragma unroll
        for (int r = 0; r < HLEN - 2; r++) load_row(r, pv[r]);
#pragma unroll
        for (int u = 0; u < HLEN; u++)
            if (HLEN - 2 + u < nin) load_row(HLEN - 2 + u, v[u]);
        static_for<HLEN - 2>([&](auto Rr) {
            constexpr int r = decltype(Rr)::value;
            row_pass(pv[r], ring[r]);
        });
    }

    const size_t ocol = (size_t)(x >> 1);
    auto body = [&](auto FAST, int q0) {
        constexpr bool fast = decltype(FAST)::value;
        const int rnext = 2 * q0 + 2 * HLEN - 2;
        static_for<HLEN / 2>([&](auto U) {
            constexpr int u = decltype(U)::value;
            if (fast || q0 + u < rows) {
                constexpr int s0 = (2 * u + HLEN - 2) % HLEN, s1 = (2 * u + HLEN - 1) % HLEN;
                row_pass(v[2 * u], ring[s0]);
                row_pass(v[2 * u + 1], ring[s1]);
                if (fast || rnext + 2 * u + 1 < nin) {
                    load_row(rnext + 2 * u, v[2 * u]);
                    load_row(rnext + 2 * u + 1, v[2 * u + 1]);
                }
                v2f ah[P], vd[P];
#pragma unroll
                for (int p = 0; p < P; p++) ah[p] = vd[p] = v2f{0.f, 0.f};
                static_for<HLEN>([&](auto J) {
                    constexpr int j = decltype(J)::value;
                    constexpr int s = (2 * u + j) % HLEN;
                    const v2f t = f.t[HLEN - 1 - j];
#pragma unroll
                    for (int p = 0; p < P; p++) {
                        ah[p] = pk_fma(splat(ring[s][p].x), t, ah[p]);
                        vd[p] = pk_fma(splat(ring[s][p].y), t, vd[p]);
                    }
                });
                float a[P], hh[P], vv[P], dd[P];
#pragma unroll
                for (int p = 0; p < P; p++) {
                    a[p] = ah[p].x;
                    hh[p] = ah[p].y;
                    vv[p] = vd[p].x;
                    dd[p] = vd[p].y;
                }
                if (valid) {
                    const size_t o = (size_t)(y0 + q0 + u) * Nc2 + ocol;
                    vstore(cA + o, a);
                    vstore(cH + o, hh);
                    vstore(cV + o, vv);
                    vstore(cD + o, dd);
                }
            }
        });
    };
    int q0 = 0;
    if (q0 + HLEN <= rows) {
        constexpr int kAfter = 4 + 6 * (HLEN / 2 - 1);
        using VOUT = typename std::conditional<P == 2, v2f, float>::type;
        float* const tr = trash + (size_t)(blockIdx.x & trash_mask) * 1024 + (threadIdx.x >> 6) * 256 + lane * P;
        const size_t ostep = valid ? (size_t)Nc2 : 0;
        float* pA = valid ? cA + (size_t)y0 * Nc2 + ocol : tr;
        float* pH = valid ? cH + (size_t)y0 * Nc2 + ocol : tr + 64 * P;
        float* pV = valid ? cV + (size_t)y0 * Nc2 + ocol : tr;
        float* pD = valid ? cD + (size_t)y0 * Nc2 + ocol : tr + 64 * P;
        const float* const lbase = in + xo;
        static_for<HLEN>([&](auto K) { asm_drain1(v[decltype(K)::value]); });
        for (; q0 + HLEN <= rows; q0 += HLEN / 2) {
            const int rnext = 2 * q0 + 2 * HLEN - 2;
            static_for<HLEN / 2>([&](auto U) {
                constexpr int u = decltype(U)::value;
                constexpr int s0 = (2 * u + HLEN - 2) % HLEN, s1 = (2 * u + HLEN - 1) % HLEN;
                asm_wait2<kAfter>(v[2 * u], v[2 * u + 1]);
                row_pass(v[2 * u], ring[s0]);
                row_pass(v[2 * u + 1], ring[s1]);
                asm_load(v[2 * u], lbase + (size_t)wrap1(yb + rnext + 2 * u, Nr) * Nc);
                asm_load(v[2 * u + 1], lbase + (size_t)wrap1(yb + rnext + 2 * u + 1, Nr) * Nc);
                v2f ah[P], vd[P];
#pragma unroll
                for (int p = 0; p < P; p++) ah[p] = vd[p] = v2f{0.f, 0.f};
                static_for<HLEN>([&](auto J) {
                    constexpr int j = decltype(J)::value;
                    constexpr int s = (2 * u + j) % HLEN;
                    const v2f t = f.t[HLEN - 1 - j];
#pragma unroll
                    for (int p = 0; p < P; p++) {
                        ah[p] = pk_fma(splat(ring[s][p].x), t, ah[p]);
                        vd[p] = pk_fma(splat(ring[s][p].y), t, vd[p]);
                    }
                });
                const size_t ro = (size_t)(q0 + u) * ostep;
                if constexpr (P == 2) {
                    asm_store(pA + ro, VOUT{ah[0].x, ah[1].x});
                    asm_store(pH + ro, VOUT{ah[0].y, ah[1].y});
                    asm_store(pV + ro, VOUT{vd[0].x, vd[1].x});
                    asm_store(pD + ro, VOUT{vd[0].y, vd[1].y});
                } else {
                    asm_store(pA + ro, ah[0].x);
                    asm_store(pH + ro, ah[0].y);
                    asm_store(pV + ro, vd[0].x);
                    asm_store(pD + ro, vd[0].y);
                }
            });
        }
        static_for<HLEN>([&](auto K) { asm_drain1(v[decltype(K)::value]); });
    }
    for (; q0 < rows; q0 += HLEN / 2) body(std::false_type{}, q0);
}

template <int HLEN>
struct InvGeom {
    static constexpr int H2 = HLEN / 2;
    static constexpr int C = H2 / 2;
    static constexpr int SHIFT = (H2 & 1) ? 0 : 1;
    static constexpr int PC = 2;
    static constexpr int NB = C > 0 ? (C + PC - 1) / PC : 0;
    static constexpr int WIN = PC * (2 * NB + 1);
    static constexpr int NROWS_EXTRA = H2 - 1 + SHIFT;
    static constexpr int MAXVL = 64 - 2 * NB;
};

template <int HLEN>
__global__ __launch_bounds__(256) void k_inv2d_stream(const float* __restrict__ cA, const float* __restrict__ cH,
                                                       const float* __restrict__ cV, const float* __restrict__ cD, float* __restrict__ out,
                                                       int Nri, int Nci, int RQ, int VL, ChunkMap cm, Taps2<float> f,
                                                       const StreamBatchI* __restrict__ batch)
{
    if (batch) {
        const StreamBatchI e = batch[blockIdx.y];
        cA = e.cA;
        cH = e.cH;
        cV = e.cV;
        cD = e.cD;
        out = e.out;
    }
    using G = InvGeom<HLEN>;
    constexpr int H2 = G::H2, C = G::C, SHIFT = G::SHIFT, NB = G::NB, WIN = G::WIN;
    int cy, bx;
    if (!chunk_of_block(cm, cy, bx)) return;
    const int lane = threadIdx.x & 63;
    const int strip = bx * 4 + (threadIdx.x >> 6);
    const int col0 = strip * VL * 2;
    if (col0 >= Nci) return;
    const int cx = col0 + (lane - NB) * 2;
    const int cxw = wrapi(cx, Nci);
    const bool valid = (lane >= NB) && (lane < NB + VL) && (cx < Nci);
    const int Nco = 2 * Nci;
    const int y0 = cy * RQ;
    const int rowsq = min(RQ, Nri - y0);
    if (rowsq <= 0) return;
    const int yb = y0 - C;
    const int nrows = rowsq + G::NROWS_EXTRA;

    v2f ra[H2], rhh[H2], rv[H2], rd[H2];

    auto load_row = [&](int r, float2& a, float2& h, float2& v, float2& d) {
        const size_t o = (size_t)wrap1(yb + r, Nri) * Nci + cxw;
        a = *reinterpret_cast<const float2*>(cA + o);
        h = *reinterpret_cast<const float2*>(cH + o);
        v = *reinterpret_cast<const float2*>(cV + o);
        d = *reinterpret_cast<const float2*>(cD + o);
    };
    auto put = [&](auto S, const float2& a, const float2& h, const float2& v, const float2& d) {
        constexpr int s = decltype(S)::value;
        ra[s] = v2f{a.x, a.y};
        rhh[s] = v2f{h.x, h.y};
        rv[s] = v2f{v.x, v.y};
        rd[s] = v2f{d.x, d.y};
    };

    auto emit = [&](auto S0, auto OFF, int gy) {
        constexpr int s0 = decltype(S0)::value, off = decltype(OFF)::value;
        v2f sa = {0.f, 0.f}, sh = {0.f, 0.f}, sv = {0.f, 0.f}, sd = {0.f, 0.f};
        static_for<H2>([&](auto J) {
            constexpr int j = decltype(J)::value;
            constexpr int s = (s0 + j) % H2;
            constexpr int k = HLEN - 1 - (2 * j + off);
            constexpr int kp = k & ~1;
            const v2f pl2 = v2f{f.a[kp], f.a[kp + 1]}, ph2 = v2f{f.b[kp], f.b[kp + 1]};
            sa = pk_fma_sbcast<k & 1, false>(ra[s], pl2, sa);
            sh = pk_fma_sbcast<k & 1, false>(rhh[s], ph2, sh);
            sv = pk_fma_sbcast<k & 1, false>(rv[s], pl2, sv);
            sd = pk_fma_sbcast<k & 1, false>(rd[s], ph2, sd);
        });
        const v2f t1o = sa + sh, t2o = sv + sd;
        float t1[WIN], t2[WIN];
        t1[NB * 2] = t1o.x;
        t1[NB * 2 + 1] = t1o.y;
        t2[NB * 2] = t2o.x;
        t2[NB * 2 + 1] = t2o.y;
#pragma unroll
        for (int k = 0; k < NB; k++) {
            const int dl = (NB - 1 - k) * 2, sl = (NB - k) * 2, dr = (NB + 1 + k) * 2, sr = (NB + k) * 2;
#pragma unroll
            for (int cc = 0; cc < 2; cc++) {
                t1[dl + cc] = dpp_shr1(t1[sl + cc]);
                t2[dl + cc] = dpp_shr1(t2[sl + cc]);
                t1[dr + cc] = dpp_shl1(t1[sr + cc]);
                t2[dr + cc] = dpp_shl1(t2[sr + cc]);
            }
        }
        float o4[4];
        auto pair_out = [&](auto E0) {
            constexpr int e0 = decltype(E0)::value;
            constexpr int pl = (e0 + SHIFT) >> 1;
            v2f s1 = {0.f, 0.f}, s2 = {0.f, 0.f};
#pragma unroll
            for (int j = 0; j < H2; j++) {
                const int m = HLEN - 1 - 2 * j;
                s1 = pk_fma(splat(t1[NB * 2 + pl - C + j]), v2f{f.a[m - 1], f.a[m]}, s1);
                s2 = pk_fma(splat(t2[NB * 2 + pl - C + j]), v2f{f.b[m - 1], f.b[m]}, s2);
            }
            const v2f o = s1 + s2;
            o4[e0] = o.x;
            o4[e0 + 1] = o.y;
        };
        auto single_out = [&](auto E) {
            constexpr int eo = decltype(E)::value;
            constexpr int gp = eo + SHIFT;
            constexpr int pl = gp >> 1, offx = 1 - (gp & 1);
            float s1 = 0.f, s2 = 0.f;
#pragma unroll
            for (int j = 0; j < H2; j++) {
                const int k = HLEN - 1 - (2 * j + offx);
                s1 = __builtin_fmaf(t1[NB * 2 + pl - C + j], f.a[k], s1);
                s2 = __builtin_fmaf(t2[NB * 2 + pl - C + j], f.b[k], s2);
            }
            o4[eo] = s1 + s2;
        };
        if constexpr (SHIFT == 0) {
            pair_out(std::integral_constant<int, 0>{});
            pair_out(std::integral_constant<int, 2>{});
        } else {
            single_out(std::integral_constant<int, 0>{});
            pair_out(std::integral_constant<int, 1>{});
            single_out(std::integral_constant<int, 3>{});
        }
        if (valid) *reinterpret_cast<float4*>(out + (size_t)gy * Nco + 2 * cx) = make_float4(o4[0], o4[1], o4[2], o4[3]);
    };

    float2 a[H2], h[H2], v[H2], d[H2];
    {
        float2 pa[H2 > 1 ? H2 - 1 : 1], ph[H2 > 1 ? H2 - 1 : 1], pv[H2 > 1 ? H2 - 1 : 1], pd[H2 > 1 ? H2 - 1 : 1];
#pragma unroll
        for (int r = 0; r < H2 - 1; r++) load_row(r, pa[r], ph[r], pv[r], pd[r]);
#pragma unroll
        for (int u = 0; u < H2; u++)
            if (H2 - 1 + u < nrows) load_row(H2 - 1 + u, a[u], h[u], v[u], d[u]);
        static_for<H2 - 1>([&](auto Rr) {
            constexpr int r = decltype(Rr)::value;
            put(Rr, pa[r], ph[r], pv[r], pd[r]);
        });
    }

    const int nsteady = nrows - (H2 - 1);
    auto body = [&](auto FAST, int t0) {
        constexpr bool fast = decltype(FAST)::value;
        static_for<H2>([&](auto U) {
            constexpr int u = decltype(U)::value;
            const int t = t0 + u;
            if (fast || t < nsteady) {
                put(std::integral_constant<int, (H2 - 1 + u) % H2>{}, a[u], h[u], v[u], d[u]);
                if (fast || H2 - 1 + t + H2 < nrows) load_row(H2 - 1 + t + H2, a[u], h[u], v[u], d[u]);
                const int g1 = 2 * t - SHIFT, g0 = g1 + 1;
                if (fast) {
                    emit(std::integral_constant<int, u % H2>{}, std::integral_constant<int, 1>{}, 2 * y0 + g1);
                    emit(std::integral_constant<int, u % H2>{}, std::integral_constant<int, 0>{}, 2 * y0 + g0);
                } else {
                    if (g1 >= 0 && g1 < 2 * rowsq) emit(std::integral_constant<int, u % H2>{}, std::integral_constant<int, 1>{}, 2 * y0 + g1);
                    if (g0 < 2 * rowsq) emit(std::integral_constant<int, u % H2>{}, std::integral_constant<int, 0>{}, 2 * y0 + g0);
                }
            }
        });
    };
    int t0 = 0;
    body(std::false_type{}, t0);
    t0 += H2;
    if (t0 + 2 * H2 <= nsteady - 1) {
        body(std::true_type{}, t0);
        t0 += H2;
        for (; t0 + 2 * H2 <= nsteady - 1; t0 += H2) body(std::true_type{}, t0);
    }
    for (; t0 < nsteady; t0 += H2) body(std::false_type{}, t0);
}

bool stream_enabled() { return knob(KN_STREAM) == 1 && counted_waits_ok(); }

static int pick_rows(long long nrows_total, int strips, int unit)
{
    int R = knob(KN_STREAM_R);
    if (R <= 0) {
        const long long target_waves = knob(KN_STREAM_WAVES);
        R = (int)(((long long)nrows_total * strips) / target_waves);
        if (R > 64) R = 64;
        if (R < 2) R = 2;
    }
    (void)unit;
    return R;
}

#define PDWT_CHECK_LAUNCH() PDWT_HIP_TRY(hipGetLastError())

template <int HLEN, int NIN>
static int launch_fwd_n(const float* in, float* cA, float* cH, float* cV, float* cD, float* trash, int trash_mask, int nr, int nc,
                        const Taps2<float>& f2, const StreamBatchF* batch = nullptr, int nimg = 1)
{
    TapsLH f;
    for (int k = 0; k < PDWT_MAX_FILTER_WIDTH; k++) f.t[k] = v2f{f2.a[k], f2.b[k]};
    constexpr int MAXVL = FwdGeom<HLEN, NIN>::MAXVL;
    const int strips = idiv_up(nc, MAXVL * NIN);
    const int VL = idiv_up(nc / NIN, strips);
    const int R = std::min(pick_rows((long long)(nr / 2) * nimg, strips, HLEN / 2), std::max(2, nr / 2));
    dim3 grid;
    const ChunkMap cm = make_map(idiv_up(strips, 4), idiv_up(nr / 2, R), &grid);
    grid.y = (unsigned)nimg;
    KTimer kt(K_FWD2D_STREAM, true);
    PDWT_LAUNCH_KT(kt, (k_fwd2d_stream<HLEN, NIN>), grid, dim3(256), 0, in, cA, cH, cV, cD, nr, nc, R, VL, trash, trash_mask, cm, f, batch);
    PDWT_CHECK_LAUNCH();
    return PDWT_OK;
}
template <int HLEN>
static int launch_fwd(const float* in, float* cA, float* cH, float* cV, float* cD, float* trash, int trash_mask, int nr, int nc,
                      const Taps2<float>& f, const StreamBatchF* batch = nullptr, int nimg = 1)
{
    const long long narrow_below = knob(KN_STREAM_NARROW);
    if constexpr (HLEN > 10) {
        return launch_fwd_n<HLEN, 2>(in, cA, cH, cV, cD, trash, trash_mask, nr, nc, f, batch, nimg);
    } else {
        if ((long long)nr * nc * nimg <= narrow_below) return launch_fwd_n<HLEN, 2>(in, cA, cH, cV, cD, trash, trash_mask, nr, nc, f, batch, nimg);
        return launch_fwd_n<HLEN, 4>(in, cA, cH, cV, cD, trash, trash_mask, nr, nc, f, batch, nimg);
    }
}

template <int HLEN>
static int launch_inv(const float* cA, const float* cH, const float* cV, const float* cD, float* out, int nri, int nci, const Taps2<float>& f,
                      const StreamBatchI* batch = nullptr, int nimg = 1)
{
    constexpr int MAXVL = InvGeom<HLEN>::MAXVL;
    const int strips = idiv_up(nci, MAXVL * 2);
    const int VL = idiv_up(nci / 2, strips);
    const int RQ = std::min(pick_rows((long long)nri * nimg, strips, InvGeom<HLEN>::H2), std::max(2, nri));
    dim3 grid;
    const ChunkMap cm = make_map(idiv_up(strips, 4), idiv_up(nri, RQ), &grid);
    grid.y = (unsigned)nimg;
    KTimer kt(K_INV2D_STREAM, true);
    PDWT_LAUNCH_KT(kt, k_inv2d_stream<HLEN>, grid, dim3(256), 0, cA, cH, cV, cD, out, nri, nci, RQ, VL, cm, f, batch);
    PDWT_CHECK_LAUNCH();
    return PDWT_OK;
}

#define PDWT_STREAM_FWD_HLENS(X) X(4) X(6) X(8) X(10) X(12) X(14) X(16)
#define PDWT_STREAM_INV_HLENS(X) X(4) X(6) X(8) X(10) X(12) X(14) X(16)

int fwd2d_stream_f32(const float* in, float* cA, float* cH, float* cV, float* cD, float* trash, size_t trash_floats, int nr, int nc, int hlen,
                     const Taps2<float>& f)
{
    if (!stream_enabled() || !trash || trash_floats < 1024) return 1;
    int slots = 1;
    while (slots < 256 && (size_t)slots * 2 * 1024 <= trash_floats) slots *= 2;
    const int trash_mask = slots - 1;
    if ((nr & 1) || (nc & 3) || nc < 64 || nr < 2 * hlen) return 1;
    if (!al16(in) || !al16(cA) || !al16(cH) || !al16(cV) || !al16(cD)) return 1;
    switch (hlen) {
#define X(H) \
    case H: return launch_fwd<H>(in, cA, cH, cV, cD, trash, trash_mask, nr, nc, f);
        PDWT_STREAM_FWD_HLENS(X)
#undef X
        default: return 1;
    }
}

int inv2d_stream_f32(const float* cA, const float* cH, const float* cV, const float* cD, float* out, int nri, int nci, int nro, int nco,
                     int hlen, const Taps2<float>& f)
{
    if (!stream_enabled()) return 1;
    if ((nci & 1) || nco != 2 * nci || nro != 2 * nri || nci < 32 || nri < 2 * hlen) return 1;
    if (!al16(out) || !al16(cA) || !al16(cH) || !al16(cV) || !al16(cD)) return 1;
    switch (hlen) {
#define X(H) \
    case H: return launch_inv<H>(cA, cH, cV, cD, out, nri, nci, f);
        PDWT_STREAM_INV_HLENS(X)
#undef X
        default: return 1;
    }
}


bool fwd2d_stream_takes(int nr, int nc, int hlen)
{
    if (!stream_enabled() || (nr & 1) || (nc & 3) || nc < 64 || nr < 2 * hlen) return false;
    switch (hlen) {
#define X(H) case H:
        PDWT_STREAM_FWD_HLENS(X)
#undef X
        return true;
        default: return false;
    }
}
bool inv2d_stream_takes(int nri, int nci, int hlen)
{
    if (!stream_enabled() || (nci & 1) || nci < 32 || nri < 2 * hlen) return false;
    switch (hlen) {
#define X(H) case H:
        PDWT_STREAM_INV_HLENS(X)
#undef X
        return true;
        default: return false;
    }
}

int fwd2d_stream_batch_f32(const StreamBatchF* d_tab, int nimg, size_t trash_floats, int nr, int nc, int hlen, const Taps2<float>& f)
{
    if (!d_tab || nimg < 1 || nimg > 65535 || trash_floats < 1024 || !fwd2d_stream_takes(nr, nc, hlen)) return 1;
    int slots = 1;
    while (slots < 256 && (size_t)slots * 2 * 1024 <= trash_floats) slots *= 2;
    switch (hlen) {
#define X(H) \
    case H: return launch_fwd<H>(nullptr, nullptr, nullptr, nullptr, nullptr, nullptr, slots - 1, nr, nc, f, d_tab, nimg);
        PDWT_STREAM_FWD_HLENS(X)
#undef X
        default: return 1;
    }
}

int inv2d_stream_batch_f32(const StreamBatchI* d_tab, int nimg, int nri, int nci, int hlen, const Taps2<float>& f)
{
    if (!d_tab || nimg < 1 || nimg > 65535 || !inv2d_stream_takes(nri, nci, hlen)) return 1;
    switch (hlen) {
#define X(H) \
    case H: return launch_inv<H>(nullptr, nullptr, nullptr, nullptr, nullptr, nri, nci, f, d_tab, nimg);
        PDWT_STREAM_INV_HLENS(X)
#undef X
        default: return 1;
    }
}

}
```

pdwt_amd/csrc/runtime.hip:

```cpp
#include <set>
#include <utility>
#include <stdio.h>
#include <stdlib.h>
#include <string.h>

#include <mutex>
#include <vector>

#include "common.hpp"

namespace pdwt {

static thread_local char g_err[512] = "";

void set_last_error(hipError_t e, const char* what, const char* file, int line)
{
    snprintf(g_err, sizeof(g_err), "%s: %s (%s:%d)", hipGetErrorString(e), what, file, line);
    (void)hipGetLastError();
}

static std::mutex g_mu;
static hipStream_t g_streams[64] = {};
static hipStream_t g_user_streams[64] = {};
static bool g_user_set[64] = {};

hipStream_t stream()
{
    int dev = 0;
    if (hipGetDevice(&dev) != hipSuccess || dev < 0 || dev >= 64) return nullptr;
    std::lock_guard<std::mutex> lk(g_mu);
    if (g_user_set[dev]) return g_user_streams[dev];
    if (!g_streams[dev]) {
        static const bool nonblocking = getenv("PDWT_STREAM_NONBLOCKING") && atoi(getenv("PDWT_STREAM_NONBLOCKING")) == 1;
        if (hipStreamCreateWithFlags(&g_streams[dev], nonblocking ? hipStreamNonBlocking : hipStreamDefault) != hipSuccess) {
            g_streams[dev] = nullptr;
        }
    }
    return g_streams[dev];
}

int lds_opt_in_ptr(const void* kernel)
{
    static std::mutex mu;
    static std::set<std::pair<const void*, int>> done;
    int dev = 0;
    PDWT_HIP_TRY(hipGetDevice(&dev));
    std::lock_guard<std::mutex> lk(mu);
    if (done.count({kernel, dev})) return PDWT_OK;
    PDWT_HIP_TRY(hipFuncSetAttribute(kernel, hipFuncAttributeMaxDynamicSharedMemorySize, 160 * 1024));
    done.insert({kernel, dev});
    return PDWT_OK;
}

struct KnobDef { const char* name; const char* env; int dflt; };
static const KnobDef g_knob_defs[KN_COUNT] = {
    {"force_twopass", "PDWT_FORCE_TWOPASS", 0}, {"tiled_cols", "PDWT_TILED_COLS", 0},
    {"casc", "PDWT_CASC", 1}, {"casc_waves", "PDWT_CASC_WAVES", 0}, {"casc_nv", "PDWT_CASC_NV", 0},
    {"casc_min", "PDWT_CASC_MIN", 2048 * 2048}, {"casc_iwaves", "PDWT_CASC_IWAVES", 0}, {"casc_ipfd", "PDWT_CASC_IPFD", 1},
    {"casc_wg", "PDWT_CASC_WG", 0}, {"casc_iwg", "PDWT_CASC_IWG", 0}, {"casc_l3", "PDWT_CASC_L3", 1}, {"casc_spec", "PDWT_CASC_SPEC", 7}, {"casc_xcdw", "PDWT_CASC_XCDW", 0}, {"dwt1d_lds_kb", "PDWT_DWT1D_LDS_KB", 80},
    {"stream", "PDWT_STREAM", 1}, {"stream_r", "PDWT_STREAM_R", 0}, {"stream_waves", "PDWT_STREAM_WAVES", 8192},
    {"stream_narrow", "PDWT_STREAM_NARROW", 2048 * 2048}, {"small", "PDWT_SMALL", 1},
    {"rows_tr", "PDWT_ROWS_TR", 1}, {"ring_r", "PDWT_RING_R", 0}, {"ring_waves", "PDWT_RING_WAVES", 4096},
    {"swtf", "PDWT_SWTF", 1}, {"swtf_m", "PDWT_SWTF_M", 0}, {"swtf_mi", "PDWT_SWTF_MI", 0},
    {"swtf_xcd", "PDWT_SWTF_XCD", 1}, {"swtf_alt", "PDWT_SWTF_ALT", 1}, {"swtf_perm", "PDWT_SWTF_PERM", 1}, {"swtf_f64", "PDWT_SWTF_F64", 1},
    {"f64_lds", "PDWT_F64_LDS", 1}, {"f64_lds_min", "PDWT_F64_LDS_MIN", 256}, {"f64_lds_wgs", "PDWT_F64_LDS_WGS", 512}, {"f64_lds_mingroups", "PDWT_F64_LDS_MINGROUPS", 1}, {"f64_lds_skew", "PDWT_F64_LDS_SKEW", 64}, {"norm2sq_ref1d", "PDWT_NORM2SQ_REF1D", 0},
    {"norm_in_threshold", "PDWT_NORM_IN_THRESHOLD", -1},
    {"selfcheck", "PDWT_SELFCHECK", 1}, {"dwt1d_f64", "PDWT_DWT1D_F64", 1}, {"swtf_long", "PDWT_SWTF_LONG", 1}, {"f64_tail", "PDWT_F64_TAIL", 0},
    {"exp0", "PDWT_EXP0", 0}, {"exp1", "PDWT_EXP1", 0}, {"exp2", "PDWT_EXP2", 0}, {"exp3", "PDWT_EXP3", 0}, {"nonsep_tiled", "PDWT_NONSEP_TILED", 1},
    {"f64_lat", "PDWT_F64_LAT", 1}, {"f64_lat_min", "PDWT_F64_LAT_MIN", 4096}, {"dwt1d_nt_mb", "PDWT_DWT1D_NT_MB", 192},
};
static int g_knob_vals[KN_COUNT];
static std::once_flag g_knob_once;
static void knob_init()
{
    for (int i = 0; i < KN_COUNT; i++) {
        const char* e = getenv(g_knob_defs[i].env);
        g_knob_vals[i] = (e && *e) ? atoi(e) : g_knob_defs[i].dflt;
    }
}
int knob(KnobId id)
{
    std::call_once(g_knob_once, knob_init);
    return g_knob_vals[id];
}
int knob_set(const char* name, int value)
{
    std::call_once(g_knob_once, knob_init);
    if (!name) return PDWT_EINVAL;
    for (int i = 0; i < KN_COUNT; i++) {
        if (!strcmp(name, g_knob_defs[i].name)) {
            g_knob_vals[i] = value;
            return PDWT_OK;
        }
    }
    return PDWT_EINVAL;
}

std::atomic<int> g_stat_spec_fwd{0}, g_stat_spec_inv{0};
void stat_casc_spec(int inverse) { (inverse ? g_stat_spec_inv : g_stat_spec_fwd).fetch_add(1, std::memory_order_relaxed); }
std::atomic<int> g_stat_lat_fwd{0}, g_stat_lat_inv{0};
void stat_lat(int inverse) { (inverse ? g_stat_lat_inv : g_stat_lat_fwd).fetch_add(1, std::memory_order_relaxed); }

int knob_get(const char* name, int* value)
{
    std::call_once(g_knob_once, knob_init);
    if (!name || !value) return PDWT_EINVAL;
    if (!strcmp(name, "stat_casc_spec_fwd") || !strcmp(name, "stat_casc_spec_inv")) {
        *value = (name[15] == 'f' ? g_stat_spec_fwd : g_stat_spec_inv).load(std::memory_order_relaxed);
        return PDWT_OK;
    }
    if (!strcmp(name, "stat_lat_fwd") || !strcmp(name, "stat_lat_inv")) {
        *value = (name[9] == 'f' ? g_stat_lat_fwd : g_stat_lat_inv).load(std::memory_order_relaxed);
        return PDWT_OK;
    }
    for (int i = 0; i < KN_COUNT; i++) {
        if (!strcmp(name, g_knob_defs[i].name)) {
            *value = g_knob_vals[i];
            return PDWT_OK;
        }
    }
    return PDWT_EINVAL;
}

static unsigned long long* g_probe[64] = {};
static unsigned long long* g_probe_allbuf[64] = {};
static bool g_probe_on = false;
static int g_probe_all = 0;
unsigned long long* clock_probe_all(int* all)
{
    *all = 0;
    if (!g_probe_all) return nullptr;
    int dev = 0;
    if (hipGetDevice(&dev) != hipSuccess || dev < 0 || dev >= 64) return nullptr;
    if (!g_probe_allbuf[dev] && hipMalloc(&g_probe_allbuf[dev], (size_t)kClockProbeAllBlocks * 4 * sizeof(unsigned long long)) != hipSuccess) return nullptr;
    *all = g_probe_all;
    return g_probe_allbuf[dev];
}
unsigned long long* clock_probe_slot(int slot)
{
    if (!g_probe_on || slot < 0 || slot >= 16) return nullptr;
    int dev = 0;
    if (hipGetDevice(&dev) != hipSuccess || dev < 0 || dev >= 64) return nullptr;
    if (!g_probe[dev]) {
        if (hipMalloc(&g_probe[dev], 16 * 4 * sizeof(unsigned long long)) != hipSuccess) return nullptr;
        (void)hipMemsetAsync(g_probe[dev], 0, 16 * 4 * sizeof(unsigned long long), stream());
    }
    return g_probe[dev] + 4 * slot;
}

static const char* const g_knames[K_COUNT] = {
    "fwd2d_fused", "inv2d_fused", "ana_rows", "ana_cols", "syn_cols", "syn_rows",
    "swt_ana_rows", "swt_ana_cols", "swt_syn_cols", "swt_syn_rows",
    "haar2d_fwd", "haar2d_inv", "haar1d_fwd", "haar1d_inv", "soft_thresh", "abs_sum", "abs_sum_final",
    "fwd2d_casc", "inv2d_casc", "fwd2d_stream", "inv2d_stream", "fwd2d_small", "inv2d_small", "fwd2d_f64", "inv2d_f64", "thresh_sum",
};
struct KRec { int id; hipEvent_t e0, e1; };
static thread_local bool g_kt_on = false;
static thread_local std::vector<KRec>* g_kt = nullptr;
static thread_local std::vector<hipEvent_t>* g_evpool = nullptr;

static hipEvent_t ev_get()
{
    if (g_evpool && !g_evpool->empty()) {
        hipEvent_t e = g_evpool->back();
        g_evpool->pop_back();
        return e;
    }
    hipEvent_t e = nullptr;
    if (hipEventCreate(&e) != hipSuccess) return nullptr;
    return e;
}

KTimer::KTimer(int kernel_id, bool attach_to_launch) : id(kernel_id), ext(attach_to_launch)
{
    if (!g_kt_on) return;
    e0 = ev_get();
    e1 = ev_get();
    if (e0 && !ext) (void)hipEventRecord(e0, stream());
}
KTimer::~KTimer()
{
    if (!e0 || !e1) return;
    if (!ext) (void)hipEventRecord(e1, stream());
    if (!g_kt) g_kt = new std::vector<KRec>();
    g_kt->push_back(KRec{id, e0, e1});
}

}

using namespace pdwt;

extern "C" {

int pdwt_device_count(void)
{
    int n = 0;
    if (hipGetDeviceCount(&n) != hipSuccess) {
        (void)hipGetLastError();
        return 0;
    }
    return n;
}
int pdwt_set_device(int dev)
{
    PDWT_HIP_TRY(hipSetDevice(dev));
    return PDWT_OK;
}
int pdwt_get_device(void)
{
    int dev = -1;
    if (hipGetDevice(&dev) != hipSuccess) return PDWT_EHIP;
    return dev;
}
int pdwt_device_name(char* buf, int buflen)
{
    if (!buf || buflen <= 0) return PDWT_EINVAL;
    int dev = 0;
    PDWT_HIP_TRY(hipGetDevice(&dev));
    hipDeviceProp_t p;
    PDWT_HIP_TRY(hipGetDeviceProperties(&p, dev));
    snprintf(buf, (size_t)buflen, "%s (%s, %d CUs)", p.name, p.gcnArchName, p.multiProcessorCount);
    return PDWT_OK;
}
void* pdwt_malloc(size_t nbytes)
{
    void* p = nullptr;
    hipError_t e = hipMalloc(&p, nbytes ? nbytes : 1);
    if (e != hipSuccess) {
        set_last_error(e, "hipMalloc", __FILE__, __LINE__);
        return nullptr;
    }
    return p;
}
int pdwt_free(void* dptr)
{
    if (!dptr) return PDWT_OK;
    PDWT_HIP_TRY(hipStreamSynchronize(stream()));
    PDWT_HIP_TRY(hipFree(dptr));
    return PDWT_OK;
}
int pdwt_memset(void* dptr, int byte, size_t nbytes)
{
    if (!nbytes) return PDWT_OK;
    PDWT_HIP_TRY(hipMemsetAsync(dptr, byte, nbytes, stream()));
    return PDWT_OK;
}
int pdwt_memcpy_h2d(void* dst, const void* src, size_t nbytes)
{
    if (!nbytes) return PDWT_OK;
    PDWT_HIP_TRY(hipMemcpyAsync(dst, src, nbytes, hipMemcpyHostToDevice, stream()));
    PDWT_HIP_TRY(hipStreamSynchronize(stream()));
    return PDWT_OK;
}
int pdwt_memcpy_d2h(void* dst, const void* src, size_t nbytes)
{
    if (!nbytes) return PDWT_OK;
    PDWT_HIP_TRY(hipMemcpyAsync(dst, src, nbytes, hipMemcpyDeviceToHost, stream()));
    PDWT_HIP_TRY(hipStreamSynchronize(stream()));
    return PDWT_OK;
}
int pdwt_memcpy_d2d(void* dst, const void* src, size_t nbytes)
{
    if (!nbytes) return PDWT_OK;
    PDWT_HIP_TRY(hipMemcpyAsync(dst, src, nbytes, hipMemcpyDeviceToDevice, stream()));
    return PDWT_OK;
}
int pdwt_memcpy_d2d_foreign(void* dst, const void* src, size_t nbytes)
{
    if (!nbytes) return PDWT_OK;
    PDWT_HIP_TRY(hipStreamSynchronize(nullptr));
    PDWT_HIP_TRY(hipMemcpyAsync(dst, src, nbytes, hipMemcpyDeviceToDevice, stream()));
    PDWT_HIP_TRY(hipStreamSynchronize(stream()));
    return PDWT_OK;
}
int pdwt_sync(void)
{
    PDWT_HIP_TRY(hipStreamSynchronize(stream()));
    return PDWT_OK;
}
void* pdwt_get_stream(void) { return (void*)stream(); }
int pdwt_set_stream(void* user_stream, int use_it)
{
    int dev = 0;
    PDWT_HIP_TRY(hipGetDevice(&dev));
    if (dev < 0 || dev >= 64) return PDWT_EINVAL;
    PDWT_HIP_TRY(hipStreamSynchronize(stream()));
    std::lock_guard<std::mutex> lk(g_mu);
    g_user_set[dev] = use_it != 0;
    g_user_streams[dev] = use_it ? (hipStream_t)user_stream : nullptr;
    return PDWT_OK;
}
const char* pdwt_last_error_string(void) { return g_err; }

void* pdwt_event_create(void)
{
    hipEvent_t e = nullptr;
    if (hipEventCreate(&e) != hipSuccess) return nullptr;
    return (void*)e;
}
int pdwt_event_record(void* ev)
{
    PDWT_HIP_TRY(hipEventRecord((hipEvent_t)ev, stream()));
    return PDWT_OK;
}
int pdwt_event_sync(void* ev)
{
    PDWT_HIP_TRY(hipEventSynchronize((hipEvent_t)ev));
    return PDWT_OK;
}
float pdwt_event_elapsed_ms(void* a, void* b)
{
    float ms = -1.f;
    if (hipEventElapsedTime(&ms, (hipEvent_t)a, (hipEvent_t)b) != hipSuccess) return -1.f;
    return ms;
}
int pdwt_event_destroy(void* ev)
{
    PDWT_HIP_TRY(hipEventDestroy((hipEvent_t)ev));
    return PDWT_OK;
}

int pdwt_graph_allowed(void) { return (g_kt_on || g_probe_on) ? 0 : 1; }
int pdwt_graph_capture_begin(void)
{
    (void)pdwt::counted_waits_ok();
    PDWT_HIP_TRY(hipStreamBeginCapture(pdwt::stream(), hipStreamCaptureModeThreadLocal));
    return PDWT_OK;
}
int pdwt_graph_capture_end(void** exec_out)
{
    if (!exec_out) return PDWT_EINVAL;
    *exec_out = nullptr;
    hipGraph_t g = nullptr;
    hipError_t e = hipStreamEndCapture(pdwt::stream(), &g);
    if (e != hipSuccess || !g) {
        (void)hipGetLastError();
        return PDWT_EHIP;
    }
    hipGraphExec_t x = nullptr;
    e = hipGraphInstantiate(&x, g, nullptr, nullptr, 0);
    (void)hipGraphDestroy(g);
    if (e != hipSuccess || !x) {
        (void)hipGetLastError();
        return PDWT_EHIP;
    }
    *exec_out = (void*)x;
    return PDWT_OK;
}
int pdwt_graph_launch(void* exec)
{
    if (!exec) return PDWT_EINVAL;
    PDWT_HIP_TRY(hipGraphLaunch((hipGraphExec_t)exec, pdwt::stream()));
    return PDWT_OK;
}
int pdwt_graph_destroy(void* exec)
{
    if (exec) PDWT_HIP_TRY(hipGraphExecDestroy((hipGraphExec_t)exec));
    return PDWT_OK;
}

namespace {
typedef float probe_v4f __attribute__((ext_vector_type(4)));
__global__ __launch_bounds__(256) void k_bw_probe(const probe_v4f* __restrict__ in, probe_v4f* __restrict__ out, size_t n4, int mode)
{
    const size_t G = gridDim.x, nblk = (n4 + 255) / 256, per = (nblk + G - 1) / G;
    probe_v4f acc = {0.f, 0.f, 0.f, 0.f};
    for (size_t k = 0; k < per; k += 8) {
        probe_v4f r[8];
        size_t idx[8];
        bool on[8];
#pragma unroll
        for (int u = 0; u < 8; u++) {
            idx[u] = (blockIdx.x * per + k + u) * 256 + threadIdx.x;
            on[u] = (k + u < per) && idx[u] < n4;
            if (mode != 2) r[u] = in[on[u] ? idx[u] : threadIdx.x];
            else r[u] = probe_v4f{1.f, 2.f, 3.f, (float)u};
        }
#pragma unroll
        for (int u = 0; u < 8; u++) {
            if (mode == 1) acc += r[u];
            else if (on[u]) out[idx[u]] = r[u];
        }
    }
    if (mode == 1 && acc.x + acc.y + acc.z + acc.w == 12345.678f) out[0] = acc;
}
}
int pdwt_probe_bandwidth(const void* src, void* dst, size_t bytes, int mode)
{
    if (mode < 0 || mode > 2 || bytes < 4096 || (mode != 2 && !src) || !dst) return PDWT_EINVAL;
    int dev = 0, ncu = 256;
    PDWT_HIP_TRY(hipGetDevice(&dev));
    PDWT_HIP_TRY(hipDeviceGetAttribute(&ncu, hipDeviceAttributeMultiprocessorCount, dev));
    hipLaunchKernelGGL(k_bw_probe, dim3((unsigned)(8 * ncu)), dim3(256), 0, pdwt::stream(), (const probe_v4f*)src, (probe_v4f*)dst, bytes / 16, mode);
    PDWT_HIP_TRY(hipGetLastError());
    return PDWT_OK;
}

int pdwt_clock_probe_enable(int on)
{
    g_probe_on = on == 1;
    g_probe_all = on >= 2 ? on - 1 : 0;
    return PDWT_OK;
}
int pdwt_clock_probe_dump(unsigned long long* out, int nblocks)
{
    int dev = 0;
    PDWT_HIP_TRY(hipGetDevice(&dev));
    if (!out || nblocks < 1 || nblocks > kClockProbeAllBlocks || dev < 0 || dev >= 64 || !g_probe_allbuf[dev]) return PDWT_EINVAL;
    return pdwt_memcpy_d2h(out, g_probe_allbuf[dev], (size_t)nblocks * 4 * sizeof(unsigned long long));
}
int pdwt_clock_probe_read(int slot, double* shader_mhz, double* span_us)
{
    if (slot < 0 || slot >= 16 || !shader_mhz || !span_us) return PDWT_EINVAL;
    int dev = 0;
    PDWT_HIP_TRY(hipGetDevice(&dev));
    *shader_mhz = *span_us = 0.0;
    if (dev < 0 || dev >= 64 || !g_probe[dev]) return PDWT_OK;
    unsigned long long h[4];
    const int rc = pdwt_memcpy_d2h(h, g_probe[dev] + 4 * slot, sizeof(h));
    if (rc != PDWT_OK) return rc;
    if (h[3] > h[1] && h[2] > h[0]) {
        const double ticks = (double)(h[3] - h[1]);
        *span_us = ticks / 100.0;
        *shader_mhz = (double)(h[2] - h[0]) / ticks * 100.0;
    }
    return PDWT_OK;
}
int pdwt_ktime_enable(int on)
{
    g_kt_on = on != 0;
    return PDWT_OK;
}
int pdwt_ktime_reset(void)
{
    if (g_kt) {
        if (!g_evpool) g_evpool = new std::vector<hipEvent_t>();
        (void)hipStreamSynchronize(stream());
        for (auto& r : *g_kt) {
            g_evpool->push_back(r.e0);
            g_evpool->push_back(r.e1);
        }
        g_kt->clear();
    }
    return PDWT_OK;
}
int pdwt_ktime_read(int kernel_id, int* n_launches, double* total_ms)
{
    if (kernel_id < 0 || kernel_id >= K_COUNT) return PDWT_EINVAL;
    PDWT_HIP_TRY(hipStreamSynchronize(stream()));
    int n = 0;
    double tot = 0;
    if (g_kt) {
        for (auto& r : *g_kt) {
            if (r.id != kernel_id) continue;
            float ms = 0;
            if (hipEventElapsedTime(&ms, r.e0, r.e1) == hipSuccess) {
                tot += ms;
                n++;
            }
        }
    }
    if (n_launches) *n_launches = n;
    if (total_ms) *total_ms = tot;
    return PDWT_OK;
}
const char* pdwt_kernel_name(int kernel_id) { return (kernel_id >= 0 && kernel_id < K_COUNT) ? g_knames[kernel_id] : nullptr; }
int pdwt_kernel_count(void) { return K_COUNT; }

}
```

pdwt_amd/csrc/stream_dev.hpp:

```cpp
#pragma once
#include <stdlib.h>

#include <type_traits>

#include "common.hpp"

#if defined(__HIP_DEVICE_COMPILE__) && !defined(__gfx950__)
#error "pdwt_amd streaming kernels: gfx950 (MI355X) only -- see stream_dev.hpp"
#endif

namespace pdwt {

__device__ __forceinline__ float dpp_shr1(float src)
{
    return __int_as_float(__builtin_amdgcn_mov_dpp(__float_as_int(src), 0x138, 0xf, 0xf, true));
}
__device__ __forceinline__ float dpp_shl1(float src)
{
    return __int_as_float(__builtin_amdgcn_mov_dpp(__float_as_int(src), 0x130, 0xf, 0xf, true));
}

__device__ __forceinline__ int wrapi(int s, int n)
{
    s %= n;
    return s < 0 ? s + n : s;
}
__device__ __forceinline__ int wrap1(int s, int n) { return s < 0 ? s + n : (s >= n ? s - n : s); }

template <int I, int N, typename F>
__device__ __forceinline__ void static_for_impl(F&& fn)
{
    if constexpr (I < N) {
        fn(std::integral_constant<int, I>{});
        static_for_impl<I + 1, N>(fn);
    }
}
template <int N, typename F>
__device__ __forceinline__ void static_for(F&& fn)
{
    static_for_impl<0, N>(fn);
}

typedef float v2f __attribute__((ext_vector_type(2)));
__device__ __forceinline__ v2f pk_fma(v2f a, v2f b, v2f c) { return __builtin_elementwise_fma(a, b, c); }
__device__ __forceinline__ v2f splat(float x) { return v2f{x, x}; }

template <int HALF, bool FIRST>
__device__ __forceinline__ v2f pk_fma_sbcast(v2f v, v2f spair, v2f acc)
{
    if constexpr (FIRST) {
        v2f r;
        if constexpr (HALF == 0) asm("v_pk_fma_f32 %0, %1, %2, 0 op_sel_hi:[1,0,0]" : "=v"(r) : "v"(v), "s"(spair));
        else asm("v_pk_fma_f32 %0, %1, %2, 0 op_sel:[0,1,0] op_sel_hi:[1,1,0]" : "=v"(r) : "v"(v), "s"(spair));
        return r;
    } else {
        if constexpr (HALF == 0) asm("v_pk_fma_f32 %0, %1, %2, %0 op_sel_hi:[1,0,1]" : "+v"(acc) : "v"(v), "s"(spair));
        else asm("v_pk_fma_f32 %0, %1, %2, %0 op_sel:[0,1,0] op_sel_hi:[1,1,1]" : "+v"(acc) : "v"(v), "s"(spair));
        return acc;
    }
}

template <int HALF, bool FIRST>
__device__ __forceinline__ v2f pk_fma_vbcast(v2f v, v2f spair, v2f acc)
{
    if constexpr (FIRST) {
        v2f r;
        if constexpr (HALF == 0) asm("v_pk_fma_f32 %0, %1, %2, 0 op_sel_hi:[0,1,0]" : "=v"(r) : "v"(v), "s"(spair));
        else asm("v_pk_fma_f32 %0, %1, %2, 0 op_sel:[1,0,0] op_sel_hi:[1,1,0]" : "=v"(r) : "v"(v), "s"(spair));
        return r;
    } else {
        if constexpr (HALF == 0) asm("v_pk_fma_f32 %0, %1, %2, %0 op_sel_hi:[0,1,1]" : "+v"(acc) : "v"(v), "s"(spair));
        else asm("v_pk_fma_f32 %0, %1, %2, %0 op_sel:[1,0,0]" : "+v"(acc) : "v"(v), "s"(spair));
        return acc;
    }
}

struct TapsLH {
    v2f t[PDWT_MAX_FILTER_WIDTH];
};

struct ChunkMap {
    int gx;
    int nchunks;
    int rpx;
};
__device__ __forceinline__ bool chunk_of_block(const ChunkMap& m, int& cy, int& bx)
{
    const int b = blockIdx.x;
    const int xcd = b & 7, slot = b >> 3;
    cy = xcd * m.rpx + slot / m.gx;
    bx = slot % m.gx;
    return cy < min(m.nchunks, (xcd + 1) * m.rpx);
}

typedef float v4f __attribute__((ext_vector_type(4)));
template <int N> struct VecOf;
template <> struct VecOf<4> { using type = v4f; };
template <> struct VecOf<2> { using type = v2f; };
__device__ __forceinline__ void vstore(float* p, const float (&a)[2]) { *reinterpret_cast<float2*>(p) = make_float2(a[0], a[1]); }
__device__ __forceinline__ void vstore(float* p, const float (&a)[1]) { *p = a[0]; }

__device__ __forceinline__ void asm_load(v4f& d, const float* p) { asm volatile("global_load_dwordx4 %0, %1, off" : "+v"(d) : "v"(p) : "memory"); }
__device__ __forceinline__ void asm_load(v2f& d, const float* p) { asm volatile("global_load_dwordx2 %0, %1, off" : "+v"(d) : "v"(p) : "memory"); }
__device__ __forceinline__ void asm_load(float& d, const float* p) { asm volatile("global_load_dword %0, %1, off" : "+v"(d) : "v"(p) : "memory"); }
__device__ __forceinline__ void asm_store(float* p, v2f d) { asm volatile("global_store_dwordx2 %0, %1, off" ::"v"(p), "v"(d) : "memory"); }
__device__ __forceinline__ void asm_store(float* p, float d) { asm volatile("global_store_dword %0, %1, off" ::"v"(p), "v"(d) : "memory"); }
__device__ __forceinline__ void asm_store(float* p, v4f d) { asm volatile("global_store_dwordx4 %0, %1, off\n\ts_nop 1" ::"v"(p), "v"(d) : "memory"); }
typedef unsigned long long lanemask_t;
#if defined(PDWT_LD_NT) && PDWT_LD_NT
#define PDWT_LD_POLICY " nt"
#else
#define PDWT_LD_POLICY ""
#endif
__device__ __forceinline__ void asm_load_s(v4f& d, const float* sbase, unsigned voff)
{
    asm volatile("global_load_dwordx4 %0, %1, %2" PDWT_LD_POLICY : "+v"(d) : "v"(voff), "s"(sbase) : "memory");
}
__device__ __forceinline__ void asm_load_s(v2f& d, const float* sbase, unsigned voff)
{
    asm volatile("global_load_dwordx2 %0, %1, %2" PDWT_LD_POLICY : "+v"(d) : "v"(voff), "s"(sbase) : "memory");
}
__device__ __forceinline__ void asm_load_s(float& d, const float* sbase, unsigned voff)
{
    asm volatile("global_load_dword %0, %1, %2" PDWT_LD_POLICY : "+v"(d) : "v"(voff), "s"(sbase) : "memory");
}
__device__ __forceinline__ void asm_store_sm(float* sbase, unsigned voff, v2f d, lanemask_t mask)
{
    lanemask_t saved;
    asm volatile("s_and_saveexec_b64 %0, %4\n\tglobal_store_dwordx2 %1, %2, %3\n\ts_mov_b64 exec, %0"
                 : "=&s"(saved) : "v"(voff), "v"(d), "s"(sbase), "s"(mask) : "memory", "scc");
}
__device__ __forceinline__ void asm_store_sm(float* sbase, unsigned voff, float d, lanemask_t mask)
{
    lanemask_t saved;
    asm volatile("s_and_saveexec_b64 %0, %4\n\tglobal_store_dword %1, %2, %3\n\ts_mov_b64 exec, %0"
                 : "=&s"(saved) : "v"(voff), "v"(d), "s"(sbase), "s"(mask) : "memory", "scc");
}
__device__ __forceinline__ void asm_store_sm(float* sbase, unsigned voff, v4f d, lanemask_t mask)
{
    lanemask_t saved;
    asm volatile("s_and_saveexec_b64 %0, %4\n\tglobal_store_dwordx4 %1, %2, %3\n\ts_nop 1\n\ts_mov_b64 exec, %0"
                 : "=&s"(saved) : "v"(voff), "v"(d), "s"(sbase), "s"(mask) : "memory", "scc");
}
__device__ __forceinline__ void asm_store3_sm(float* b0, float* b1, float* b2, unsigned voff, v2f d0, v2f d1, v2f d2, lanemask_t mask)
{
    lanemask_t saved;
    asm volatile("s_and_saveexec_b64 %0, %8\n\tglobal_store_dwordx2 %1, %2, %5\n\tglobal_store_dwordx2 %1, %3, %6\n\tglobal_store_dwordx2 %1, %4, %7\n\ts_mov_b64 exec, %0"
                 : "=&s"(saved) : "v"(voff), "v"(d0), "v"(d1), "v"(d2), "s"(b0), "s"(b1), "s"(b2), "s"(mask) : "memory", "scc");
}
__device__ __forceinline__ void asm_store4_sm(float* b0, float* b1, float* b2, float* b3, unsigned voff, float d0, float d1, float d2, float d3, lanemask_t mask)
{
    lanemask_t saved;
    asm volatile("s_and_saveexec_b64 %0, %10\n\tglobal_store_dword %1, %2, %6\n\tglobal_store_dword %1, %3, %7\n\tglobal_store_dword %1, %4, %8\n\tglobal_store_dword %1, %5, %9\n\ts_mov_b64 exec, %0"
                 : "=&s"(saved) : "v"(voff), "v"(d0), "v"(d1), "v"(d2), "v"(d3), "s"(b0), "s"(b1), "s"(b2), "s"(b3), "s"(mask) : "memory", "scc");
}
__device__ __forceinline__ void asm_store_sm_nt(float* sbase, unsigned voff, v4f d, lanemask_t mask)
{
    lanemask_t saved;
    asm volatile("s_and_saveexec_b64 %0, %4\n\tglobal_store_dwordx4 %1, %2, %3 nt\n\ts_nop 1\n\ts_mov_b64 exec, %0"
                 : "=&s"(saved) : "v"(voff), "v"(d), "s"(sbase), "s"(mask) : "memory", "scc");
}
__device__ __forceinline__ float asm_copy(const float& src)
{
    float d;
    asm volatile("v_mov_b32 %0, %1" : "=v"(d) : "v"(src));
    return d;
}
__device__ __forceinline__ v2f asm_copy(const v2f& src)
{
    v2f d;
    asm volatile("v_mov_b64 %0, %1" : "=v"(d) : "v"(src));
    return d;
}
template <int N, typename V>
__device__ __forceinline__ void asm_wait2(V& a, V& b) { asm volatile("s_waitcnt vmcnt(%2)" : "+v"(a), "+v"(b) : "n"(N) : "memory"); }
template <int N, typename V>
__device__ __forceinline__ void asm_wait4(V& a, V& b, V& c, V& d) { asm volatile("s_waitcnt vmcnt(%4)" : "+v"(a), "+v"(b), "+v"(c), "+v"(d) : "n"(N) : "memory"); }
template <int N, typename V>
__device__ __forceinline__ void asm_wait3(V& a, V& b, V& c) { asm volatile("s_waitcnt vmcnt(%3)" : "+v"(a), "+v"(b), "+v"(c) : "n"(N) : "memory"); }
template <int N, typename V>
__device__ __forceinline__ void asm_wait2_sel(bool counted, V& a, V& b)
{
    asm volatile("s_cmp_eq_u32 %2, 0\n\ts_cbranch_scc1 .Lws0_%=\n\ts_waitcnt vmcnt(%3)\n\ts_branch .Lws1_%=\n.Lws0_%=:\n\ts_waitcnt vmcnt(0)\n.Lws1_%=:"
                 : "+v"(a), "+v"(b) : "s"(__builtin_amdgcn_readfirstlane((int)counted)), "n"(N) : "memory", "scc");
}
template <int N, typename V>
__device__ __forceinline__ void asm_wait8_sel(bool counted, V& a, V& b, V& c, V& d, V& e, V& f, V& g, V& h)
{
    asm volatile("s_cmp_eq_u32 %8, 0\n\ts_cbranch_scc1 .Lws0_%=\n\ts_waitcnt vmcnt(%9)\n\ts_branch .Lws1_%=\n.Lws0_%=:\n\ts_waitcnt vmcnt(0)\n.Lws1_%=:"
                 : "+v"(a), "+v"(b), "+v"(c), "+v"(d), "+v"(e), "+v"(f), "+v"(g), "+v"(h) : "s"(__builtin_amdgcn_readfirstlane((int)counted)), "n"(N) : "memory", "scc");
}
template <typename V>
__device__ __forceinline__ void asm_drain1(V& a) { asm volatile("s_waitcnt vmcnt(0)" : "+v"(a) : : "memory"); }


static inline ChunkMap make_map(int gx, int nchunks, dim3* grid)
{
    ChunkMap m;
    m.gx = gx;
    m.nchunks = nchunks;
    m.rpx = idiv_up(nchunks, 8);
    *grid = dim3((unsigned)(8 * m.rpx * gx));
    return m;
}
static inline bool al16(const void* p) { return ((uintptr_t)p & 15) == 0; }

}
```

Measured before the change: 341,700 Mpixels/s.

## Use host-verified reciprocal division, single-wrap indexing and early prologue loads in cascade kernels

Replaces integer divisions in the work-group-to-chunk mapping with multiply-by-reciprocal, with the reciprocals checked on the host for all indices in use. Column wrapping uses a single conditional subtract when the geometry allows it. The forward cascade kernel issues its prologue row loads before the LDS setup and waits on them with counted vmcnt, and kernel arguments are reordered and touched early so scalar loads start sooner. The per-XCD balancing option (xcdw) is removed and replaced by the recip knob. New host-side guards fall back when the geometry is out of range, at the cost of a host verification loop whose result is cached per thread.

```diff
diff --git a/pdwt_amd/csrc/casc_dev.hpp b/pdwt_amd/csrc/casc_dev.hpp
--- a/pdwt_amd/csrc/casc_dev.hpp
+++ b/pdwt_amd/csrc/casc_dev.hpp
@@ -24,20 +24,42 @@
     int cpx;
     int strips;
     int gy;
-    int flags;
+    unsigned ms;
+    unsigned mg;
     const void* tbl;
 };
-__host__ __device__ inline int casc_chunk_start(int g, int strip, int units, int gy, int strips, int cpx, int d)
+__host__ __device__ inline int casc_chunk_start(int g, int units, int gy)
 {
     if (g >= gy) return units;
-    int b = (int)(((long long)g * units) / gy);
-    if (d != 0) {
-        int bal = 0;
-        for (int q = 0; q < g; q++) bal += (((q * strips + strip) / cpx) & 1) ? -1 : 1;
-        b += d * bal;
+    return (int)(((long long)g * units) / gy);
+}
+inline bool casc_map_recip(CascMap& cm, int units, bool enable)
+{
+    cm.ms = cm.mg = 0;
+    if (!enable || cm.strips < 1 || cm.gy < 1 || (long long)(cm.gy + 1) * units >= (1LL << 31) || (long long)cm.gy * cm.strips >= (1LL << 31)) return false;
+    const unsigned ms = recip31(cm.strips), mg = recip31(cm.gy);
+    static thread_local struct { int strips, gy, units; bool ok; } last = {0, 0, 0, false};
+    if (last.strips != cm.strips || last.gy != cm.gy || last.units != units) {
+        bool ok = true;
+        for (int wg = 0; wg < cm.gy * cm.strips && ok; wg++) ok = div_recip31((unsigned)wg, ms) == wg / cm.strips;
+        for (int g = 0; g <= cm.gy && ok; g++) ok = div_recip31((unsigned)g * (unsigned)units, mg) == casc_chunk_start(g, units, cm.gy);
+        last = {cm.strips, cm.gy, units, ok};
     }
-    return b;
+    if (!last.ok) return false;
+    cm.ms = ms;
+    cm.mg = mg;
+    return true;
 }
+#ifdef __HIPCC__
+__device__ __forceinline__ void casc_wg_chunk(const CascMap& cm, int wg, int units, int& strip, int& J0, int& R)
+{
+    const int gy = div_recip31((unsigned)wg, cm.ms);
+    strip = wg - gy * cm.strips;
+    const unsigned x0 = (unsigned)gy * (unsigned)units;
+    J0 = div_recip31(x0, cm.mg);
+    R = div_recip31(x0 + (unsigned)units, cm.mg) - J0;
+}
+#endif
 
 struct CascBands {
     float *H1, *V1, *D1, *A2, *H2, *V2, *D2;
diff --git a/pdwt_amd/csrc/common.hpp b/pdwt_amd/csrc/common.hpp
--- a/pdwt_amd/csrc/common.hpp
+++ b/pdwt_amd/csrc/common.hpp
@@ -110,7 +110,7 @@
     KN_CASC_IWG,
     KN_CASC_L3,
     KN_CASC_SPEC,
-    KN_CASC_XCDW,
+    KN_CASC_RECIP,
     KN_DWT1D_LDS_KB,
     KN_STREAM,
     KN_STREAM_R,
@@ -154,6 +154,9 @@
 int knob_set(const char* name, int value);
 int knob_get(const char* name, int* value);
 
+__host__ __device__ inline int div_recip31(unsigned x, unsigned m) { return (int)(((unsigned long long)(2u * x) * m) >> 32); }
+inline unsigned recip31(int d) { return (unsigned)(((1ULL << 31) + (unsigned)d - 1) / (unsigned)d); }
+
 __host__ __device__ inline int div2(int n) { return (n + 1) >> 1; }
 inline int idiv_up(int a, int b) { return (a + b - 1) / b; }
 
diff --git a/pdwt_amd/csrc/dwt_casc.hip b/pdwt_amd/csrc/dwt_casc.hip
--- a/pdwt_amd/csrc/dwt_casc.hip
+++ b/pdwt_amd/csrc/dwt_casc.hip
@@ -88,22 +88,22 @@
 };
 
 template <int HLEN, int NV, int W, bool SPEC = false>
-__global__ __launch_bounds__(W == 1 ? 256 : 64 * W) void k_fwd2d_casc(const float* in, CascBands b, int Nr, int Nc, int VL,
-                                                                       float* __restrict__ trash, CascMap cm, TapsLH f)
+__global__ __launch_bounds__(W == 1 ? 256 : 64 * W) void k_fwd2d_casc(const float* in, CascBands b, int Nr, int Nc, int VL, CascMap cm,
+                                                                       float* __restrict__ trash, TapsLH f)
 {
     using G = CascGeom<HLEN>;
     constexpr int C = G::C, NB1 = G::NB1, NB2 = G::NB2, NBT = G::NBT, WIN1 = G::WIN1, WIN2 = G::WIN2;
     extern __shared__ __attribute__((aligned(16))) unsigned char lds_raw[];
     CASC_TRACE_DECL;
     CASC_TRACE(0);
-    if constexpr (W > 1) {
-        if (cm.tbl) {
-            static_assert(sizeof(CascBatchF) == 8 * sizeof(void*), "eight pointers per image");
-            typedef const unsigned long long __attribute__((address_space(4))) * tbl_t;
-            const tbl_t q = (tbl_t)(const unsigned long long*)cm.tbl + 8 * (size_t)blockIdx.y;
-            in = (const float*)q[0];
-            b = CascBands{(float*)q[1], (float*)q[2], (float*)q[3], (float*)q[4], (float*)q[5], (float*)q[6], (float*)q[7]};
-        }
+    PDWT_FETCH_NOW(in, cm.tbl, Nr, Nc, VL, cm.cpx, cm.strips, cm.gy, cm.ms, cm.mg);
+    static_for<HLEN>([&](auto K) { PDWT_FETCH_NOW(f.t[decltype(K)::value]); });
+    if (W > 1 && cm.tbl) {
+        static_assert(sizeof(CascBatchF) == 8 * sizeof(void*), "eight pointers per image");
+        typedef const unsigned long long __attribute__((address_space(4))) * tbl_t;
+        const tbl_t q = (tbl_t)(const unsigned long long*)cm.tbl + 8 * (size_t)blockIdx.y;
+        in = (const float*)q[0];
+        b = CascBands{(float*)q[1], (float*)q[2], (float*)q[3], (float*)q[4], (float*)q[5], (float*)q[6], (float*)q[7]};
     }
     const int lane = threadIdx.x & 63;
     const int Nc2 = Nc >> 1, Nr2 = Nr >> 1, Nr4 = Nr >> 2, Nc4 = Nc >> 2;
@@ -125,12 +125,10 @@
         const int xcd = blockIdx.x & 7, slot = blockIdx.x >> 3;
         const int wg = xcd * cm.cpx + slot;
         if (slot >= cm.cpx || wg >= cm.gy * cm.strips) return;
-        const int gy = wg / cm.strips;
-        strip = wg % cm.strips;
-        const int J0 = casc_chunk_start(gy, strip, Nr4, cm.gy, cm.strips, cm.cpx, cm.flags);
-        const int R = casc_chunk_start(gy + 1, strip, Nr4, cm.gy, cm.strips, cm.cpx, cm.flags) - J0;
-        const int E = min((3 * (HLEN - 2) + 3) / 4, R / W - 1);
-        const int base = (R + E) / W, rem = (R + E) % W;
+        int J0, R;
+        casc_wg_chunk(cm, wg, Nr4, strip, J0, R);
+        const int E = min((3 * (HLEN - 2) + 3) / 4, (int)((unsigned)R / W) - 1);
+        const int base = (int)((unsigned)(R + E) / W), rem = (int)((unsigned)(R + E) % W);
         const int start = kw * base + min(kw, rem);
         rows2 = (kw < W - 1) ? base + (kw < rem ? 1 : 0) : R - start;
         j0 = J0 + start;
@@ -139,7 +137,7 @@
     const int xs = strip * VL * 4;
     const int x = xs + 4 * (lane - NBT);
     const bool valid = (lane >= NBT) && (lane < NBT + VL) && (x < Nc);
-    const int xo = wrapi(x, Nc);
+    const int xo = wrap1(x, Nc);
     const int yb = 4 * j0 - 3 * C;
     const int NA = 2 * rows2;
     const int NA1 = NA + HLEN - 2;
@@ -151,9 +149,27 @@
 #pragma unroll
     for (int k = 0; k < HLEN; k++) ring2[k] = v2f{0.f, 0.f};
 
-    const float* const lbase = in + xo;
-    auto rowptr = [&](int r) { return lbase + (size_t)wrap1(yb + r, Nr) * Nc; };
     const unsigned xoff = (unsigned)xo * 4u;
+    constexpr int DIST = NV / 2;
+    constexpr int NPRO = HLEN - 2 + NV;
+    static_assert(NV <= HLEN + 2, "the prologue rows must be rows every wave loads");
+    static_assert(casc_fwd_after<DIST>(1) <= 63 && NPRO <= 63, "vmcnt is a 6-bit counter");
+    const size_t strideB = (size_t)Nc * 4;
+    const char* const inB = reinterpret_cast<const char*>(in);
+    v4f pv[HLEN > 2 ? HLEN - 2 : 1];
+    v4f v[NV];
+    {
+        const int g0 = wrap1(yb, Nr);
+        const int nwrap = Nr - g0;
+        const char* const pA = inB + (size_t)g0 * strideB;
+        const char* const pB = pA - (size_t)Nr * strideB;
+        static_for<NPRO>([&](auto Rr) {
+            constexpr int r = decltype(Rr)::value;
+            v4f& d = r < HLEN - 2 ? pv[r < HLEN - 2 ? r : 0] : v[r >= HLEN - 2 ? r - (HLEN - 2) : 0];
+            asm volatile("" : "=v"(d));
+            asm_load_s(d, reinterpret_cast<const float*>(r < nwrap ? pA : pB), xoff + (unsigned)r * (unsigned)strideB);
+        });
+    }
 
     constexpr int REG = casc_fwd_region_bytes<HLEN>();
     unsigned char* const lds_rd = lds_raw + (size_t)(W > 1 ? kw : 0) * REG;
@@ -200,20 +216,11 @@
         lh = acc;
     };
 
-    constexpr int DIST = NV / 2;
-    static_assert(casc_fwd_after<DIST>(1) <= 63, "vmcnt is a 6-bit counter");
-    v4f v[NV];
-    {
-        v4f pv[HLEN > 2 ? HLEN - 2 : 1];
-#pragma unroll
-        for (int r = 0; r < HLEN - 2; r++) pv[r] = *reinterpret_cast<const v4f*>(rowptr(r));
-#pragma unroll
-        for (int u = 0; u < NV; u++) v[u] = *reinterpret_cast<const v4f*>(rowptr(min(HLEN - 2 + u, rlast)));
-        static_for<HLEN - 2>([&](auto Rr) {
-            constexpr int r = decltype(Rr)::value;
-            row_pass1(pv[r], ring[r]);
-        });
-    }
+    static_for<HLEN - 2>([&](auto Rr) {
+        constexpr int r = decltype(Rr)::value;
+        asm volatile("s_waitcnt vmcnt(%1)" : "+v"(pv[r]) : "n"(NPRO - 1 - r) : "memory");
+        row_pass1(pv[r], ring[r]);
+    });
     if constexpr (W > 1) {
         if (kw > 0) {
 #pragma unroll
@@ -227,8 +234,6 @@
     const int lim2 = ((W == 1) || last) ? 0x7fffffff : NA;
     int lr = HLEN - 2 + NV;
     int lgr = wrap1(yb + min(lr, rlast), Nr);
-    const size_t strideB = (size_t)Nc * 4;
-    const char* const inB = reinterpret_cast<const char*>(in);
     const char* lp = inB + (size_t)lgr * strideB;
     const char* lplast = lp;
     auto next_rows = [&](const char*& p0, const char*& p1) {
@@ -751,6 +756,25 @@
 
 static bool casc_enabled() { return knob(KN_CASC) == 1; }
 
+template <int HLEN, int NVD>
+static auto fwd_casc_kernel(int W, bool nv2, bool spec, bool want_optin, int* optin)
+{
+    void (*k)(const float*, CascBands, int, int, int, CascMap, float*, TapsLH);
+    *optin = PDWT_OK;
+#define PDWT_PICK(...)                                             \
+    do {                                                           \
+        k = __VA_ARGS__;                                           \
+        if (want_optin) *optin = lds_opt_in<__VA_ARGS__>();        \
+    } while (0)
+    if (spec) PDWT_PICK(k_fwd2d_casc<HLEN, 2, 16, true>);
+    else if (nv2) PDWT_PICK(k_fwd2d_casc<HLEN, 2, 16, false>);
+    else if (W == 4) PDWT_PICK(k_fwd2d_casc<HLEN, NVD, 4, false>);
+    else if (W == 8) PDWT_PICK(k_fwd2d_casc<HLEN, NVD, 8, false>);
+    else PDWT_PICK(k_fwd2d_casc<HLEN, NVD, 16, false>);
+#undef PDWT_PICK
+    return k;
+}
+
 template <int HLEN>
 static int launch_fwd_casc(const float* in, const CascBands& b, float* trash, int nr, int nc, const Taps2<float>& f2, const CascBatchF* d_tbl, int nimg)
 {
@@ -776,65 +800,55 @@
         if (gy >= 1 && (nr4 / gy) / W >= HLEN / 2) {
             int nwg = gy * strips;
             const size_t lds = (size_t)(W - 1) * REG;
-            void (*k)(const float*, CascBands, int, int, int, float*, CascMap, TapsLH);
-            k = (W == 4) ? k_fwd2d_casc<HLEN, NVD, 4> : (W == 8) ? k_fwd2d_casc<HLEN, NVD, 8> : k_fwd2d_casc<HLEN, NVD, 16>;
             const bool nv2 = W == 16 && (knob(KN_CASC_NV) == 0 || knob(KN_CASC_NV) == 2);
-            if (nv2) k = k_fwd2d_casc<HLEN, 2, 16>;
             bool spec = nv2 && (knob(KN_CASC_SPEC) & 1) && 2 * 4 >= HLEN;
-            auto spec_ok = [&](int gyq, int xwq) {
-                const int cpxq = idiv_up(gyq * strips, 8);
-                for (int g = 0; g < gyq; g++)
-                    for (int st = 0; st < strips; st++) {
-                        const int R = casc_chunk_start(g + 1, st, nr4, gyq, strips, cpxq, xwq) - casc_chunk_start(g, st, nr4, gyq, strips, cpxq, xwq);
-                        if (R < 16) return false;
-                        const int E = std::min((3 * (HLEN - 2) + 3) / 4, R / 16 - 1);
-                        const int base = (R + E) / 16, rem = (R + E) % 16;
-                        if (base != 4 || R - (15 * base + std::min(15, rem)) != 1) return false;
-                    }
+            auto spec_ok = [&](int gyq) {
+                for (int g = 0; g < gyq; g++) {
+                    const int R = casc_chunk_start(g + 1, nr4, gyq) - casc_chunk_start(g, nr4, gyq);
+                    if (R < 16) return false;
+                    const int E = std::min((3 * (HLEN - 2) + 3) / 4, R / 16 - 1);
+                    const int base = (R + E) / 16, rem = (R + E) % 16;
+                    if (base != 4 || R - (15 * base + std::min(15, rem)) != 1) return false;
+                }
                 return true;
             };
             if (spec && (knob(KN_CASC_SPEC) & 4) && knob(KN_CASC_WAVES) <= 0 && !d_tbl && (nr4 / gy) / 16 >= 8) {
                 const int gy2 = (nr4 + 36) / 73;
-                if (gy2 >= 3 * gy && spec_ok(gy2, 0)) {
+                if (gy2 >= 3 * gy && spec_ok(gy2)) {
                     gy = gy2;
                     nwg = gy * strips;
                 }
             }
-            int xw = spec ? knob(KN_CASC_XCDW) : 0;
-            if (spec && xw != 0 && !spec_ok(gy, xw)) xw = 0;
-            spec = spec && spec_ok(gy, xw);
-            if (!spec) xw = 0;
-            if (spec) {
-                k = k_fwd2d_casc<HLEN, 2, 16, true>;
-                stat_casc_spec(0);
-            }
-            const CascMap cm = {idiv_up(nwg, 8), strips, gy, xw, d_tbl};
+            spec = spec && spec_ok(gy);
+            CascMap cm = {idiv_up(nwg, 8), strips, gy, 0u, 0u, d_tbl};
+            if (casc_map_recip(cm, nr4, knob(KN_CASC_RECIP) != 0)) {
+            const long long xmax = (long long)(strips - 1) * VL * 4 + 4 * 63;
+            if (xmax >= 2LL * nc || 4 * CascGeom<HLEN>::NBT > nc || (long long)nc * 4 * (3 * HLEN) >= (1LL << 32)) return 1;
             const dim3 grid((unsigned)(8 * cm.cpx), (unsigned)(d_tbl ? nimg : 1));
-            if (lds > 64 * 1024) {
-                int rc = (W == 4) ? lds_opt_in<k_fwd2d_casc<HLEN, NVD, 4>>()
-                         : (W == 8) ? lds_opt_in<k_fwd2d_casc<HLEN, NVD, 8>>() : lds_opt_in<k_fwd2d_casc<HLEN, NVD, 16>>();
-                if (rc == PDWT_OK && nv2) rc = lds_opt_in<k_fwd2d_casc<HLEN, 2, 16>>();
-                if (rc == PDWT_OK && spec) rc = lds_opt_in<k_fwd2d_casc<HLEN, 2, 16, true>>();
-                if (rc != PDWT_OK) return rc;
-            }
-            PDWT_LAUNCH_KT(kt, k, grid, dim3(64 * W), lds, in, b, nr, nc, VL, trash, cm, f);
+            int rc = PDWT_OK;
+            const auto k = fwd_casc_kernel<HLEN, NVD>(W, nv2, spec, lds > 64 * 1024, &rc);
+            if (rc != PDWT_OK) return rc;
+            if (spec) stat_casc_spec(0);
+            PDWT_LAUNCH_KT(kt, k, grid, dim3(64 * W), lds, in, b, nr, nc, VL, cm, trash, f);
             PDWT_CHECK_LAUNCH();
             return PDWT_OK;
+            }
         }
     }
     if (d_tbl) return 1;
     int cpx = (knob(KN_CASC_WAVES) > 0 ? knob(KN_CASC_WAVES) : 1024) / (8 * strips);
     if (cpx > nr / 4 / 4 / 8) cpx = nr / 4 / 4 / 8;
     if (cpx < 1) cpx = 1;
-    const CascMap cm = {cpx, strips, 0};
+    const CascMap cm = {cpx, strips, 0, 0u, 0u, nullptr};
+    if ((long long)(strips - 1) * VL * 4 + 4 * 63 >= 2LL * nc || 4 * CascGeom<HLEN>::NBT > nc) return 1;
     const dim3 grid((unsigned)(8 * idiv_up(cpx * strips, 4)));
     const int nv = knob(KN_CASC_NV) > 0 ? knob(KN_CASC_NV) : NVD;
     if (nv == 2)
-        PDWT_LAUNCH_KT(kt, (k_fwd2d_casc<HLEN, 2, 1>), grid, dim3(256), 0, in, b, nr, nc, VL, trash, cm, f);
+        PDWT_LAUNCH_KT(kt, (k_fwd2d_casc<HLEN, 2, 1>), grid, dim3(256), 0, in, b, nr, nc, VL, cm, trash, f);
     else if (nv < HLEN && HLEN % 4 == 0)
-        PDWT_LAUNCH_KT(kt, (k_fwd2d_casc<HLEN, NVD, 1>), grid, dim3(256), 0, in, b, nr, nc, VL, trash, cm, f);
+        PDWT_LAUNCH_KT(kt, (k_fwd2d_casc<HLEN, NVD, 1>), grid, dim3(256), 0, in, b, nr, nc, VL, cm, trash, f);
     else
-        PDWT_LAUNCH_KT(kt, (k_fwd2d_casc<HLEN, (HLEN > 16 ? NVD : HLEN), 1>), grid, dim3(256), 0, in, b, nr, nc, VL, trash, cm, f);
+        PDWT_LAUNCH_KT(kt, (k_fwd2d_casc<HLEN, (HLEN > 16 ? NVD : HLEN), 1>), grid, dim3(256), 0, in, b, nr, nc, VL, cm, trash, f);
     PDWT_CHECK_LAUNCH();
     return PDWT_OK;
 }
diff --git a/pdwt_amd/csrc/dwt_casc_inv3.hip b/pdwt_amd/csrc/dwt_casc_inv3.hip
--- a/pdwt_amd/csrc/dwt_casc_inv3.hip
+++ b/pdwt_amd/csrc/dwt_casc_inv3.hip
@@ -70,8 +70,8 @@
 };
 
 template <int HLEN, int W, bool L3, bool SPEC = false>
-__global__ __launch_bounds__(64 * W) void k_inv2d_casc3(CascInvBands b, CascInv3B b3, float* out, int Nr, int Nc, int VL,
-                                                         float* __restrict__ trash, CascMap cm, Taps2<float> f)
+__global__ __launch_bounds__(64 * W) void k_inv2d_casc3(CascInvBands b, CascInv3B b3, float* out, int Nr, int Nc, int VL, CascMap cm,
+                                                         float* __restrict__ trash, Taps2<float> f)
 {
     using G = CascInvGeom<HLEN>;
     constexpr int H2 = G::H2, C = G::C, SHIFT = G::SHIFT, NBT = G::NBT;
@@ -86,6 +86,7 @@
     extern __shared__ __attribute__((aligned(16))) unsigned char lds_raw[];
     CASC_TRACE_DECL;
     CASC_TRACE(0);
+    PDWT_FETCH_NOW(cm.tbl, b.H1, b.V1, b.D1, b.H2, b.V2, b.D2, b3.A3, b3.H3, b3.V3, b3.D3, Nr, Nc, VL, cm.cpx, cm.strips, cm.gy, cm.ms, cm.mg);
     if (cm.tbl) {
         static_assert(sizeof(CascBatchI) == 12 * sizeof(void*), "twelve pointers per image");
         typedef const unsigned long long __attribute__((address_space(4))) * tbl_t;
@@ -100,12 +101,11 @@
     const int xcd = blockIdx.x & 7, slot = blockIdx.x >> 3;
     const int wg = xcd * cm.cpx + slot;
     if (slot >= cm.cpx || wg >= cm.gy * cm.strips) return;
-    const int gy = wg / cm.strips, strip = wg % cm.strips;
     const int Np = Nr2 >> 1;
-    const int Jp = casc_chunk_start(gy, strip, Np, cm.gy, cm.strips, cm.cpx, cm.flags);
-    const int Rp = casc_chunk_start(gy + 1, strip, Np, cm.gy, cm.strips, cm.cpx, cm.flags) - Jp;
+    int strip, Jp, Rp;
+    casc_wg_chunk(cm, wg, Np, strip, Jp, Rp);
     const int Ep = 0;
-    const int basep = (Rp + Ep) / W, remp = (Rp + Ep) % W;
+    const int basep = (int)((unsigned)(Rp + Ep) / W), remp = (int)((unsigned)(Rp + Ep) % W);
     const int startp = kw * basep + min(kw, remp);
     const bool last = (kw == W - 1);
     const int nQ = 2 * (last ? Rp - startp : basep + (kw < remp ? 1 : 0));
@@ -122,13 +122,13 @@
     const int X0 = strip * VL - NBT;
     const int cx1 = 2 * (X0 + lane);
     const bool valid = (lane >= NBT) && (lane < NBT + VL) && (cx1 < Nc1);
-    const int cx1w = wrapi(cx1, Nc1);
+    const int cx1w = wrap1(cx1, Nc1);
     const int cx2w = cx1w >> 1;
-    const int c3w = wrapi(((X0 + 1) >> 1) - C + lane, Nc3);
+    const int c3w = wrap2(((X0 + 1) >> 1) - C + lane, Nc3);
     const int bp_addr = 4 * (((X0 + lane + 1) >> 1) - ((X0 + 1) >> 1) + C);
     const bool bp_odd = ((X0 + lane) & 1) != 0;
 
-    auto off3 = [&](int i) PDWT_AI { return (size_t)CASC_DIAG_LD(wrapi(P3_0 - C + i, Nr3)) * Nc3; };
+    auto off3 = [&](int i) PDWT_AI { return (size_t)CASC_DIAG_LD(wrap1(P3_0 - C + i, Nr3)) * Nc3; };
     auto off2 = [&](int s2) PDWT_AI { return (size_t)CASC_DIAG_LD(wrap1(Q0 + s2, Nr2)) * Nc2; };
     auto off1 = [&](int r1) PDWT_AI { return (size_t)CASC_DIAG_LD(wrap1(P0 + r1, Nr1)) * Nc1; };
     const unsigned voff3 = (unsigned)c3w * 4u, voff2 = (unsigned)cx2w * 4u, voff1 = (unsigned)cx1w * 4u, voffo = (unsigned)(valid ? cx1 : 0) * 8u;
@@ -138,7 +138,7 @@
     const unsigned end3 = (unsigned)(kFold ? min(kFold, Nr3) : Nr3) * str3, end2 = (unsigned)(kFold ? min(kFold, Nr2) : Nr2) * str2,
                    end1 = (unsigned)(kFold ? min(kFold, Nr1) : Nr1) * str1;
     int c3 = min(T0 + H2, last3), c2 = min(H2, last2), c1 = min(2, last1);
-    unsigned o3 = (unsigned)CASC_DIAG_LD(wrapi(P3_0 - C + c3, Nr3)) * str3, o2 = (unsigned)CASC_DIAG_LD(wrap1(Q0 + c2, Nr2)) * str2,
+    unsigned o3 = (unsigned)CASC_DIAG_LD(wrap1(P3_0 - C + c3, Nr3)) * str3, o2 = (unsigned)CASC_DIAG_LD(wrap1(Q0 + c2, Nr2)) * str2,
              o1 = (unsigned)CASC_DIAG_LD(wrap1(P0 + c1, Nr1)) * str1;
     auto advance = [&](int& c, unsigned& o, int lastc, unsigned str, unsigned end) {
         int cq = c;
@@ -648,6 +648,25 @@
 #define PDWT_CHECK_LAUNCH() PDWT_HIP_TRY(hipGetLastError())
 
 template <int HLEN, bool L3>
+static auto inv_casc3_kernel(int W, bool spec, bool want_optin, int* optin)
+{
+    void (*k)(CascInvBands, CascInv3B, float*, int, int, int, CascMap, float*, Taps2<float>);
+    *optin = PDWT_OK;
+#define PDWT_PICK(...)                                             \
+    do {                                                           \
+        k = __VA_ARGS__;                                           \
+        if (want_optin) *optin = lds_opt_in<__VA_ARGS__>();        \
+    } while (0)
+    if (spec) PDWT_PICK(k_inv2d_casc3<HLEN, 16, L3, true>);
+    else if (W == 4) PDWT_PICK(k_inv2d_casc3<HLEN, 4, L3, false>);
+    else if (W == 8) PDWT_PICK(k_inv2d_casc3<HLEN, 8, L3, false>);
+    else if (W == 12) PDWT_PICK(k_inv2d_casc3<HLEN, 12, L3, false>);
+    else PDWT_PICK(k_inv2d_casc3<HLEN, 16, L3, false>);
+#undef PDWT_PICK
+    return k;
+}
+
+template <int HLEN, bool L3>
 static int launch_inv_casc3(const CascInvBands& b, const CascInv3B& b3, float* out, float* trash, int nr, int nc, const Taps2<float>& f,
                             const CascBatchI* d_tbl, int nimg)
 {
@@ -685,37 +704,24 @@
     const int nwg = gy * strips;
     
     const size_t lds = lds_bytes(W);
-    void (*k)(CascInvBands, CascInv3B, float*, int, int, int, float*, CascMap, Taps2<float>);
-    k = (W == 4) ? k_inv2d_casc3<HLEN, 4, L3> : (W == 8) ? k_inv2d_casc3<HLEN, 8, L3> : (W == 12) ? k_inv2d_casc3<HLEN, 12, L3> : k_inv2d_casc3<HLEN, 16, L3>;
     bool spec = W == 16 && ((knob(KN_CASC_SPEC) >> 1) & 1) && H2 <= 4;
-    int xw = spec ? knob(KN_CASC_XCDW) : 0;
-    for (int pass = 0; pass < 2; pass++) {
-        bool ok = spec;
-        for (int g = 0; g < gy && ok; g++)
-            for (int st = 0; st < strips && ok; st++) {
-                const int Rp = casc_chunk_start(g + 1, st, np, gy, strips, idiv_up(nwg, 8), xw) - casc_chunk_start(g, st, np, gy, strips, idiv_up(nwg, 8), xw);
-                ok = Rp / 16 == 2;
-            }
-        if (ok || xw == 0) {
-            spec = ok;
-            break;
-        }
-        xw = 0;
-    }
-    if (!spec) xw = 0;
-    if (spec) {
-        k = k_inv2d_casc3<HLEN, 16, L3, true>;
-        stat_casc_spec(1);
-    }
-    const CascMap cm = {idiv_up(nwg, 8), strips, gy, xw, d_tbl};
+    for (int g = 0; g < gy && spec; g++) spec = (casc_chunk_start(g + 1, np, gy) - casc_chunk_start(g, np, gy)) / 16 == 2;
+    CascMap cm = {idiv_up(nwg, 8), strips, gy, 0u, 0u, d_tbl};
+    if (!casc_map_recip(cm, np, knob(KN_CASC_RECIP) != 0)) return 1;
+    {
+        const long long x0max = (long long)(strips - 1) * VL - G::NBT;
+        const int nc3 = nc / 8;
+        if (2 * G::NBT > nc1 || 2 * (x0max + 63) >= 2LL * nc1) return 1;
+        if (G::NBT / 2 + G::C + 1 > nc3 || ((x0max + 1) >> 1) - G::C + 63 >= 3LL * nc3) return 1;
+        if (nr / 8 < 2 * HLEN) return 1;
+    }
     const dim3 grid((unsigned)(8 * cm.cpx), (unsigned)(d_tbl ? nimg : 1));
-    if (lds > 64 * 1024) {
-        const int rc = spec ? lds_opt_in<k_inv2d_casc3<HLEN, 16, L3, true>>()
-                       : (W == 4) ? lds_opt_in<k_inv2d_casc3<HLEN, 4, L3>>() : (W == 8) ? lds_opt_in<k_inv2d_casc3<HLEN, 8, L3>>() : (W == 12) ? lds_opt_in<k_inv2d_casc3<HLEN, 12, L3>>() : lds_opt_in<k_inv2d_casc3<HLEN, 16, L3>>();
-        if (rc != PDWT_OK) return rc;
-    }
+    int rc = PDWT_OK;
+    const auto k = inv_casc3_kernel<HLEN, L3>(W, spec, lds > 64 * 1024, &rc);
+    if (rc != PDWT_OK) return rc;
+    if (spec) stat_casc_spec(1);
     KTimer kt(K_INV2D_CASC, true);
-    PDWT_LAUNCH_KT(kt, k, grid, dim3(64 * W), lds, b, b3, out, nr, nc, VL, trash, cm, f);
+    PDWT_LAUNCH_KT(kt, k, grid, dim3(64 * W), lds, b, b3, out, nr, nc, VL, cm, trash, f);
     PDWT_CHECK_LAUNCH();
     return PDWT_OK;
 }
diff --git a/pdwt_amd/csrc/dwt_stream.hip b/pdwt_amd/csrc/dwt_stream.hip
--- a/pdwt_amd/csrc/dwt_stream.hip
+++ b/pdwt_amd/csrc/dwt_stream.hip
@@ -17,17 +17,20 @@
 template <int HLEN, int NIN>
 __global__ __launch_bounds__(256) void k_fwd2d_stream(const float* __restrict__ in, float* __restrict__ cA, float* __restrict__ cH,
                                                        float* __restrict__ cV, float* __restrict__ cD, int Nr, int Nc, int R, int VL,
-                                                       float* __restrict__ trash, int trash_mask, ChunkMap cm, TapsLH f,
-                                                       const StreamBatchF* __restrict__ batch)
-{
+                                                       ChunkMap cm, const StreamBatchF* __restrict__ batch, float* __restrict__ trash,
+                                                       int trash_mask, TapsLH f)
+{
+    PDWT_FETCH_NOW(batch, in, Nr, Nc, R, VL, cm.gx, cm.nchunks, cm.rpx, cm.mgx, cm.one_wrap);
     if (batch) {
-        const StreamBatchF e = batch[blockIdx.y];
-        in = e.in;
-        cA = e.cA;
-        cH = e.cH;
-        cV = e.cV;
-        cD = e.cD;
-        trash = e.trash;
+        static_assert(sizeof(StreamBatchF) == 6 * sizeof(void*), "six pointers per image");
+        typedef const unsigned long long __attribute__((address_space(4))) * tbl_t;
+        const tbl_t q = (tbl_t)(const unsigned long long*)batch + 6 * (size_t)blockIdx.y;
+        in = (const float*)q[0];
+        cA = (float*)q[1];
+        cH = (float*)q[2];
+        cV = (float*)q[3];
+        cD = (float*)q[4];
+        trash = (float*)q[5];
     }
     using G = FwdGeom<HLEN, NIN>;
     using VIN = typename VecOf<NIN>::type;
@@ -44,7 +47,7 @@
     if (rows <= 0) return;
     const int x = xs + NIN * (lane - NB);
     const bool valid = (lane >= NB) && (lane < NB + VL) && (x < Nc);
-    const int xo = wrapi(x, Nc);
+    const int xo = wrap_col(x, Nc, cm.one_wrap);
     const int yb = 2 * y0 - C;
     const int nin = 2 * rows + HLEN - 2;
 
@@ -202,16 +205,19 @@
 template <int HLEN>
 __global__ __launch_bounds__(256) void k_inv2d_stream(const float* __restrict__ cA, const float* __restrict__ cH,
                                                        const float* __restrict__ cV, const float* __restrict__ cD, float* __restrict__ out,
-                                                       int Nri, int Nci, int RQ, int VL, ChunkMap cm, Taps2<float> f,
-                                                       const StreamBatchI* __restrict__ batch)
-{
+                                                       int Nri, int Nci, int RQ, int VL, ChunkMap cm, const StreamBatchI* __restrict__ batch,
+                                                       Taps2<float> f)
+{
+    PDWT_FETCH_NOW(batch, cA, cH, cV, cD, Nri, Nci, RQ, VL, cm.gx, cm.nchunks, cm.rpx, cm.mgx, cm.one_wrap);
     if (batch) {
-        const StreamBatchI e = batch[blockIdx.y];
-        cA = e.cA;
-        cH = e.cH;
-        cV = e.cV;
-        cD = e.cD;
-        out = e.out;
+        static_assert(sizeof(StreamBatchI) == 5 * sizeof(void*), "five pointers per image");
+        typedef const unsigned long long __attribute__((address_space(4))) * tbl_t;
+        const tbl_t q = (tbl_t)(const unsigned long long*)batch + 5 * (size_t)blockIdx.y;
+        cA = (const float*)q[0];
+        cH = (const float*)q[1];
+        cV = (const float*)q[2];
+        cD = (const float*)q[3];
+        out = (float*)q[4];
     }
     using G = InvGeom<HLEN>;
     constexpr int H2 = G::H2, C = G::C, SHIFT = G::SHIFT, NB = G::NB, WIN = G::WIN;
@@ -222,7 +228,7 @@
     const int col0 = strip * VL * 2;
     if (col0 >= Nci) return;
     const int cx = col0 + (lane - NB) * 2;
-    const int cxw = wrapi(cx, Nci);
+    const int cxw = wrap_col(cx, Nci, cm.one_wrap);
     const bool valid = (lane >= NB) && (lane < NB + VL) && (cx < Nci);
     const int Nco = 2 * Nci;
     const int y0 = cy * RQ;
@@ -391,10 +397,11 @@
     const int VL = idiv_up(nc / NIN, strips);
     const int R = std::min(pick_rows((long long)(nr / 2) * nimg, strips, HLEN / 2), std::max(2, nr / 2));
     dim3 grid;
-    const ChunkMap cm = make_map(idiv_up(strips, 4), idiv_up(nr / 2, R), &grid);
+    ChunkMap cm = make_map(idiv_up(strips, 4), idiv_up(nr / 2, R), &grid);
+    cm.one_wrap = NIN * FwdGeom<HLEN, NIN>::NB <= nc && (long long)(strips - 1) * VL * NIN + NIN * 63 < 2LL * nc;
     grid.y = (unsigned)nimg;
     KTimer kt(K_FWD2D_STREAM, true);
-    PDWT_LAUNCH_KT(kt, (k_fwd2d_stream<HLEN, NIN>), grid, dim3(256), 0, in, cA, cH, cV, cD, nr, nc, R, VL, trash, trash_mask, cm, f, batch);
+    PDWT_LAUNCH_KT(kt, (k_fwd2d_stream<HLEN, NIN>), grid, dim3(256), 0, in, cA, cH, cV, cD, nr, nc, R, VL, cm, batch, trash, trash_mask, f);
     PDWT_CHECK_LAUNCH();
     return PDWT_OK;
 }
@@ -420,10 +427,11 @@
     const int VL = idiv_up(nci / 2, strips);
     const int RQ = std::min(pick_rows((long long)nri * nimg, strips, InvGeom<HLEN>::H2), std::max(2, nri));
     dim3 grid;
-    const ChunkMap cm = make_map(idiv_up(strips, 4), idiv_up(nri, RQ), &grid);
+    ChunkMap cm = make_map(idiv_up(strips, 4), idiv_up(nri, RQ), &grid);
+    cm.one_wrap = 2 * InvGeom<HLEN>::NB <= nci && (long long)(strips - 1) * VL * 2 + 2 * 63 < 2LL * nci;
     grid.y = (unsigned)nimg;
     KTimer kt(K_INV2D_STREAM, true);
-    PDWT_LAUNCH_KT(kt, k_inv2d_stream<HLEN>, grid, dim3(256), 0, cA, cH, cV, cD, out, nri, nci, RQ, VL, cm, f, batch);
+    PDWT_LAUNCH_KT(kt, k_inv2d_stream<HLEN>, grid, dim3(256), 0, cA, cH, cV, cD, out, nri, nci, RQ, VL, cm, batch, f);
     PDWT_CHECK_LAUNCH();
     return PDWT_OK;
 }
diff --git a/pdwt_amd/csrc/runtime.hip b/pdwt_amd/csrc/runtime.hip
--- a/pdwt_amd/csrc/runtime.hip
+++ b/pdwt_amd/csrc/runtime.hip
@@ -57,7 +57,7 @@
     {"force_twopass", "PDWT_FORCE_TWOPASS", 0}, {"tiled_cols", "PDWT_TILED_COLS", 0},
     {"casc", "PDWT_CASC", 1}, {"casc_waves", "PDWT_CASC_WAVES", 0}, {"casc_nv", "PDWT_CASC_NV", 0},
     {"casc_min", "PDWT_CASC_MIN", 2048 * 2048}, {"casc_iwaves", "PDWT_CASC_IWAVES", 0}, {"casc_ipfd", "PDWT_CASC_IPFD", 1},
-    {"casc_wg", "PDWT_CASC_WG", 0}, {"casc_iwg", "PDWT_CASC_IWG", 0}, {"casc_l3", "PDWT_CASC_L3", 1}, {"casc_spec", "PDWT_CASC_SPEC", 7}, {"casc_xcdw", "PDWT_CASC_XCDW", 0}, {"dwt1d_lds_kb", "PDWT_DWT1D_LDS_KB", 80},
+    {"casc_wg", "PDWT_CASC_WG", 0}, {"casc_iwg", "PDWT_CASC_IWG", 0}, {"casc_l3", "PDWT_CASC_L3", 1}, {"casc_spec", "PDWT_CASC_SPEC", 7}, {"casc_recip", "PDWT_CASC_RECIP", 1}, {"dwt1d_lds_kb", "PDWT_DWT1D_LDS_KB", 80},
     {"stream", "PDWT_STREAM", 1}, {"stream_r", "PDWT_STREAM_R", 0}, {"stream_waves", "PDWT_STREAM_WAVES", 8192},
     {"stream_narrow", "PDWT_STREAM_NARROW", 2048 * 2048}, {"small", "PDWT_SMALL", 1},
     {"rows_tr", "PDWT_ROWS_TR", 1}, {"ring_r", "PDWT_RING_R", 0}, {"ring_waves", "PDWT_RING_WAVES", 4096},
diff --git a/pdwt_amd/csrc/stream_dev.hpp b/pdwt_amd/csrc/stream_dev.hpp
--- a/pdwt_amd/csrc/stream_dev.hpp
+++ b/pdwt_amd/csrc/stream_dev.hpp
@@ -26,6 +26,28 @@
     return s < 0 ? s + n : s;
 }
 __device__ __forceinline__ int wrap1(int s, int n) { return s < 0 ? s + n : (s >= n ? s - n : s); }
+__device__ __forceinline__ int wrap_col(int s, int n, int one_wrap)
+{
+    if (__builtin_amdgcn_readfirstlane(one_wrap)) return wrap1(s, n);
+    return wrapi(s, n);
+}
+__device__ __forceinline__ int wrap2(int s, int n)
+{
+    s = wrap1(s, n);
+    return s >= n ? s - n : s;
+}
+
+#define PDWT_FETCH_NOW(...) pdwt_fetch_now(__VA_ARGS__)
+template <typename T>
+__device__ __forceinline__ void pdwt_fetch_one(T v)
+{
+    asm volatile("" ::"s"(v));
+}
+template <typename... T>
+__device__ __forceinline__ void pdwt_fetch_now(T... v)
+{
+    (pdwt_fetch_one(v), ...);
+}
 
 template <int I, int N, typename F>
 __device__ __forceinline__ void static_for_impl(F&& fn)
@@ -83,13 +105,16 @@
     int gx;
     int nchunks;
     int rpx;
+    unsigned mgx;
+    int one_wrap;
 };
 __device__ __forceinline__ bool chunk_of_block(const ChunkMap& m, int& cy, int& bx)
 {
     const int b = blockIdx.x;
     const int xcd = b & 7, slot = b >> 3;
-    cy = xcd * m.rpx + slot / m.gx;
-    bx = slot % m.gx;
+    const int q = m.mgx ? div_recip31((unsigned)slot, m.mgx) : slot / m.gx;
+    cy = xcd * m.rpx + q;
+    bx = slot - q * m.gx;
     return cy < min(m.nchunks, (xcd + 1) * m.rpx);
 }
 
@@ -200,6 +225,15 @@
     m.gx = gx;
     m.nchunks = nchunks;
     m.rpx = idiv_up(nchunks, 8);
+    static thread_local struct { int gx, rpx; unsigned mgx; } last = {0, 0, 0u};
+    if (last.gx != gx || last.rpx != m.rpx) {
+        unsigned mgx = recip31(gx);
+        for (long long slot = 0; slot < (long long)m.rpx * gx && mgx; slot++)
+            if (slot >= (1LL << 31) || div_recip31((unsigned)slot, mgx) != (int)(slot / gx)) mgx = 0;
+        last = {gx, m.rpx, mgx};
+    }
+    m.mgx = last.mgx;
+    m.one_wrap = 0;
     *grid = dim3((unsigned)(8 * m.rpx * gx));
     return m;
 }
```

Result: faster. 353,300 Mpixels/s (median of 6 runs) (+3.4%).
